# succinctlabs/snark-bn254-verifier

Hardware: AMD Instinct MI355X
Metric: Groth16 verifies/sec (2 pub-inputs) at batch=2^20, 1/2/4/8 MI355X (higher is better)
Workload: dtype int64

## Files before the change

### snark-bn254-verifier_amd/csrc/bn254_coop12.hip

```cpp
#include <hip/hip_runtime.h>
#include <mutex>
#include "bn254_vm.h"
#include "bn254_kernels.h"

namespace bn254 {

static_assert(COOP_T_ELEM == VE_S2, "COOP_T_ELEM must name a workspace slot that neither VE_T nor the result slot VE_S0 overlays");
#define C12_STRIDE 12
#define C12_SLOT(e) (((e) - VE_F) / 12)
#define C12_X 10
#define C12_I 11
#define C12_B 7
#define C12_R1 7
#define C12_R2 11
#define C12_R3 12
#define C12_SLOTS 13
#define C12_WAVE_DWORDS (C12_SLOTS * 64 * C12_STRIDE)
#define C12_PER_WAVE 5

typedef __attribute__((address_space(3))) int32_t c12_lds_i32;
typedef int c12_v4i __attribute__((ext_vector_type(4)));
typedef __attribute__((address_space(3))) c12_v4i c12_lds_i4;
struct Coop12 {
  c12_lds_i32* img;
  uint32_t lane, g0, c, h;
  __device__ __forceinline__ void put(int slot, const Fp& a) const {
    c12_lds_i4* q = (c12_lds_i4*)(img + ((size_t)slot * 64 + lane) * C12_STRIDE);
    q[0] = (c12_v4i){a.v[0], a.v[1], a.v[2], a.v[3]}; q[1] = (c12_v4i){a.v[4], a.v[5], a.v[6], a.v[7]}; q[2] = (c12_v4i){a.v[8], 0, 0, 0};
  }
  __device__ __forceinline__ Fp at(int slot, uint32_t ln) const {
    const c12_lds_i4* q = (const c12_lds_i4*)(img + ((size_t)slot * 64 + ln) * C12_STRIDE);
    const c12_v4i v0 = q[0], v1 = q[1], v2 = q[2];
    Fp a;
    a.v[0] = v0.x; a.v[1] = v0.y; a.v[2] = v0.z; a.v[3] = v0.w; a.v[4] = v1.x; a.v[5] = v1.y; a.v[6] = v1.z; a.v[7] = v1.w; a.v[8] = v2.x;
    return a;
  }
  __device__ __forceinline__ Fp own(int slot) const { return at(slot, lane); }
  __device__ __forceinline__ Fp half(int slot, uint32_t i) const { return at(slot, g0 + 2 * i + h); }
  __device__ __forceinline__ Fp2 coef(int slot, uint32_t i) const { Fp2 r; r.c0 = at(slot, g0 + 2 * i); r.c1 = at(slot, g0 + 2 * i + 1); return r; }
};

__device__ __forceinline__ Fp2 c12_scale(const Fp2& a, int32_t w) {
  Fp2 r;
#pragma unroll
  for (int i = 0; i < BN_NL; i++) { r.c0.v[i] = a.c0.v[i] * w; r.c1.v[i] = a.c1.v[i] * w; }
  return r;
}
struct C12H { Fp p, q; };
__device__ __forceinline__ C12H c12_halves(const Fp2& b, uint32_t h) { C12H r; r.p = fp_select(h != 0, b.c1, b.c0); r.q = fp_select(h != 0, b.c0, fp_neg(b.c1)); return r; }
__device__ __forceinline__ void c12_publish_xi(const Coop12& co, int slot) {
  const Fp o = co.own(slot), pt = co.at(slot, co.lane ^ 1);
  co.put(C12_X, fp_lincomb_reduce(9, o, co.h ? 1 : -1, pt));
}
__device__ __forceinline__ void c12_publish_i(const Coop12& co, int slot) {
  const Fp pt = co.at(slot, co.lane ^ 1);
  co.put(C12_I, fp_select(co.h != 0, pt, fp_neg(pt)));
}

__constant__ int8_t C12_SQ_Q[6][4] = {{0, 1, 2, 3}, {0, 2, 3, 0}, {0, 1, 3, 4}, {0, 1, 4, 0}, {0, 1, 2, 5}, {0, 1, 2, 0}};
__constant__ int8_t C12_SQ_P[6][4] = {{0, 5, 4, 3}, {1, 5, 4, 0}, {2, 1, 5, 4}, {3, 2, 5, 0}, {4, 3, 2, 5}, {5, 4, 3, 0}};
__constant__ int8_t C12_SQ_X[6][4] = {{0, 1, 1, 1}, {0, 1, 1, 0}, {0, 0, 1, 1}, {0, 0, 1, 0}, {0, 0, 0, 1}, {0, 0, 0, 0}};
__constant__ int8_t C12_SQ_W[6][4] = {{1, 2, 2, 1}, {2, 2, 2, 0}, {2, 1, 2, 1}, {2, 2, 2, 0}, {2, 2, 1, 1}, {2, 2, 2, 0}};
__device__ __forceinline__ void c12_sqr(const Coop12& co, int s) {
  c12_publish_xi(co, s);
  c12_publish_i(co, s);
  const uint32_t c = co.c;
  const Fp2 p0 = c12_scale(co.coef(s, C12_SQ_P[c][0]), C12_SQ_W[c][0]);
  const Fp2 p1 = c12_scale(co.coef(C12_SQ_X[c][1] ? C12_X : s, C12_SQ_P[c][1]), C12_SQ_W[c][1]);
  const Fp2 p2 = c12_scale(co.coef(C12_SQ_X[c][2] ? C12_X : s, C12_SQ_P[c][2]), C12_SQ_W[c][2]);
  const Fp2 p3 = c12_scale(co.coef(C12_SQ_X[c][3] ? C12_X : s, C12_SQ_P[c][3]), C12_SQ_W[c][3]);
  const Fp q0 = co.half(s, C12_SQ_Q[c][0]), q1 = co.half(s, C12_SQ_Q[c][1]), q2 = co.half(s, C12_SQ_Q[c][2]), q3 = co.half(s, C12_SQ_Q[c][3]);
  const Fp j0 = co.half(C12_I, C12_SQ_Q[c][0]), j1 = co.half(C12_I, C12_SQ_Q[c][1]), j2 = co.half(C12_I, C12_SQ_Q[c][2]), j3 = co.half(C12_I, C12_SQ_Q[c][3]);
  co.put(s, fp_dot(dplus(p0.c0, q0), dplus(p0.c1, j0), dplus(p1.c0, q1), dplus(p1.c1, j1), dplus(p2.c0, q2), dplus(p2.c1, j2), dplus(p3.c0, q3), dplus(p3.c1, j3)));
}
__device__ __forceinline__ void c12_mul_line_fp(const Coop12& co, int s, const Fp& d0, const C12H& d3, const C12H& d4, bool keep) {
  c12_publish_xi(co, s);
  const uint32_t c = co.c;
  const Fp k = co.own(s);
  const Fp2 k1 = co.coef(c >= 1 ? s : C12_X, (c + 5) % 6), k3 = co.coef(c >= 3 ? s : C12_X, (c + 3) % 6);
  const Fp r = fp_dot(dplus(k, d0), dplus(k1.c0, d3.p), dplus(k1.c1, d3.q), dplus(k3.c0, d4.p), dplus(k3.c1, d4.q));
  co.put(s, fp_select(keep, k, r));
}
__device__ __forceinline__ void c12_mul_line_fp2(const Coop12& co, int s, const C12H& d0, const C12H& d3, const C12H& d4) {
  c12_publish_xi(co, s);
  const uint32_t c = co.c;
  const Fp2 k0 = co.coef(s, c);
  const Fp2 k1 = co.coef(c >= 1 ? s : C12_X, (c + 5) % 6), k3 = co.coef(c >= 3 ? s : C12_X, (c + 3) % 6);
  co.put(s, fp_dot(dplus(k0.c0, d0.p), dplus(k0.c1, d0.q), dplus(k1.c0, d3.p), dplus(k1.c1, d3.q), dplus(k3.c0, d4.p), dplus(k3.c1, d4.q)));
}
__device__ __noinline__ void c12_mul(const Coop12 co, int d, int a, int b, bool conj_b) {
  const uint32_t c = co.c;
  c12_publish_xi(co, a);
  int bp = b;
  if (conj_b) {
    const Fp o = co.own(b);
    co.put(C12_B, (c & 1) ? fp_neg(o) : o);
    bp = C12_B;
  }
  c12_publish_i(co, bp);
  Fp acc;
  {
    const Fp2 a0 = co.coef(0 <= (int)c ? a : C12_X, 0), a1 = co.coef(1 <= c ? a : C12_X, 1), a2 = co.coef(2 <= c ? a : C12_X, 2);
    const uint32_t i0 = (c + 6 - 0) % 6, i1 = (c + 6 - 1) % 6, i2 = (c + 6 - 2) % 6;
    const Fp q0 = co.half(bp, i0), q1 = co.half(bp, i1), q2 = co.half(bp, i2), j0 = co.half(C12_I, i0), j1 = co.half(C12_I, i1), j2 = co.half(C12_I, i2);
    acc = fp_dot(dplus(a0.c0, q0), dplus(a0.c1, j0), dplus(a1.c0, q1), dplus(a1.c1, j1), dplus(a2.c0, q2), dplus(a2.c1, j2));
  }
  {
    const Fp2 a3 = co.coef(3 <= c ? a : C12_X, 3), a4 = co.coef(4 <= c ? a : C12_X, 4), a5 = co.coef(5 <= c ? a : C12_X, 5);
    const uint32_t i3 = (c + 6 - 3) % 6, i4 = (c + 6 - 4) % 6, i5 = (c + 6 - 5) % 6;
    const Fp q3 = co.half(bp, i3), q4 = co.half(bp, i4), q5 = co.half(bp, i5), j3 = co.half(C12_I, i3), j4 = co.half(C12_I, i4), j5 = co.half(C12_I, i5);
    acc = fp_add(acc, fp_dot(dplus(a3.c0, q3), dplus(a3.c1, j3), dplus(a4.c0, q4), dplus(a4.c1, j4), dplus(a5.c0, q5), dplus(a5.c1, j5)));
  }
  co.put(d, acc);
}
__constant__ int8_t C12_CY_A[6] = {0, 2, 1, 0, 2, 1};
__constant__ int8_t C12_CY_B[6] = {3, 5, 4, 3, 5, 4};
__device__ __noinline__ void c12_cyclo_sqr_n(const Coop12 co, int d, int s, int count) {
  const uint32_t c = co.c, h = co.h;
  const bool is_s = (c == 0) | (c == 2) | (c == 4);
  const int32_t lin = is_s ? -2 : 2;
  Fp k = co.own(s);
  for (int it = 0; it < count; it++) {
    const int src = it == 0 ? s : d;
    const Fp2 a = co.coef(src, C12_CY_A[c]), b = co.coef(src, C12_CY_B[c]);
    const Fp2 xb = fp2_mul_xi(b);
    const Fp2 u1 = fp2_select(is_s, xb, c12_scale(a, 2));
    const Fp2 v1 = fp2_select(is_s | (c == 1), is_s ? b : xb, b);
    const Fp2 u2 = c12_scale(a, is_s ? 1 : 0);
    const C12H h1 = c12_halves(v1, h), h2 = c12_halves(a, h);
    const Fp X = fp_dot(dplus(u1.c0, h1.p), dplus(u1.c1, h1.q), dplus(u2.c0, h2.p), dplus(u2.c1, h2.q));
    const Fp z = fp_lincomb_reduce(3, X, lin, k);
    co.put(d, z);
    k = z;
  }
}
__device__ __noinline__ void c12_conj(const Coop12 co, int d, int s) {
  const Fp k = co.own(s);
  co.put(d, (co.c & 1) ? fp_neg(k) : k);
}
__device__ __noinline__ void c12_frob(const Coop12 co, int d, int s, int j) {
  Fp2 k = co.coef(s, co.c);
  if (j & 1) k = fp2_conj(k);
  const int32_t(*t)[2][BN_NL] = j == 1 ? BN_FROB_G1 : j == 2 ? BN_FROB_G2 : BN_FROB_G3;
  Fp2 g;
#pragma unroll
  for (int l = 0; l < BN_NL; l++) { g.c0.v[l] = t[co.c][0][l]; g.c1.v[l] = t[co.c][1][l]; }
  const C12H gh = c12_halves(g, co.h);
  co.put(d, fp_dot(dplus(k.c0, gh.p), dplus(k.c1, gh.q)));
}
__device__ __noinline__ void c12_inv(const Coop12 co, int d, int s) {
  Fp12 f;
  K0(f) = co.coef(s, 0); K1(f) = co.coef(s, 1); K2(f) = co.coef(s, 2); K3(f) = co.coef(s, 3); K4(f) = co.coef(s, 4); K5(f) = co.coef(s, 5);
  Fp12 r = fp12_inv(f);
  const uint32_t c = co.c;
  const Fp2 o = fp2_select(c == 0, K0(r), fp2_select(c == 1, K1(r), fp2_select(c == 2, K2(r), fp2_select(c == 3, K3(r), fp2_select(c == 4, K4(r), K5(r))))));
  co.put(d, fp_select(co.h != 0, o.c1, o.c0));
}
struct Coop12Ops {
  const Coop12& co;
  __device__ __forceinline__ void f12_inv(int d, int a) { c12_inv(co, C12_SLOT(d), C12_SLOT(a)); }
  __device__ __forceinline__ void f12_conj(int d, int a) { c12_conj(co, C12_SLOT(d), C12_SLOT(a)); }
  __device__ __forceinline__ void f12_mul(int d, int a, int b, bool conj_b = false) { c12_mul(co, C12_SLOT(d), C12_SLOT(a), C12_SLOT(b), conj_b); }
  __device__ __forceinline__ void f12_frob(int d, int a, int j) { c12_frob(co, C12_SLOT(d), C12_SLOT(a), j); }
  __device__ __forceinline__ void f12_cyclo_sqr(int d, int a) { c12_cyclo_sqr_n(co, C12_SLOT(d), C12_SLOT(a), 1); }
  __device__ __forceinline__ void f12_cyclo_sqr_n(int d, int a, int count) { c12_cyclo_sqr_n(co, C12_SLOT(d), C12_SLOT(a), count); }
};

__device__ __forceinline__ Fp c12_ws_ld(const int32_t* ws, uint32_t n, uint32_t p, int e) {
  Fp r;
#pragma unroll
  for (int l = 0; l < BN_NL; l++) r.v[l] = ws[((size_t)e * BN_NL + l) * n + p];
  return r;
}
__device__ __forceinline__ void c12_ws_st(int32_t* ws, uint32_t n, uint32_t p, int e, const Fp& a) {
#pragma unroll
  for (int l = 0; l < BN_NL; l++) ws[((size_t)e * BN_NL + l) * n + p] = a.v[l];
}
__device__ __forceinline__ Fp2 c12_ws_ld2(const int32_t* ws, uint32_t n, uint32_t p, int e) { Fp2 r; r.c0 = c12_ws_ld(ws, n, p, e); r.c1 = c12_ws_ld(ws, n, p, e + 1); return r; }
__device__ __forceinline__ FixedLine c12_line_entry(const int32_t* entry) {
  FixedLine l;
#pragma unroll
  for (int i = 0; i < BN_NL; i++) {
    l.m.c0.v[i] = entry[i]; l.m.c1.v[i] = entry[BN_NL + i]; l.c.c0.v[i] = entry[2 * BN_NL + i]; l.c.c1.v[i] = entry[3 * BN_NL + i];
    l.xc.c0.v[i] = entry[4 * BN_NL + i]; l.xc.c1.v[i] = entry[5 * BN_NL + i];
  }
  return l;
}
__device__ __forceinline__ void c12_store_f12(const Coop12& co, int32_t* ws, uint32_t n, uint32_t p, int slot, int e, bool pending) {
  const Fp r = co.own(slot);
  if (pending) c12_ws_st(ws, n, p, e + 2 * (int)co.c + (int)co.h, r);
}

__device__ __forceinline__ bool c12_eq_const(const Coop12& co, int slot, const int32_t* __restrict__ target, uint32_t pl) {
  Fp t;
#pragma unroll
  for (int l = 0; l < BN_NL; l++) t.v[l] = target[(2 * (int)co.c + (int)co.h) * BN_NL + l];
  BN_SETB(t, 1.0, 0.5);
  const uint64_t m = __builtin_amdgcn_ballot_w64(fp_eq(co.own(slot), t));
  return ((m >> (pl * 12u)) & 0xfffull) == 0xfffull;
}

#define C12_PROLOGUE()                                                                                        \
  extern __shared__ __attribute__((aligned(16))) int32_t c12_lds[];                                           \
  const uint32_t lane = threadIdx.x & 63;                                                                     \
  const bool act = lane < 12 * C12_PER_WAVE;                                                                  \
  const uint32_t la = act ? lane : lane - 12;                          \
  const uint32_t pl = la / 12, c = (la - pl * 12) >> 1, h = la & 1;                                           \
  const uint32_t p = blockIdx.x * (uint32_t)C12_PER_WAVE + pl;                                                \
  const bool live = act && p < n;                                                                             \
  const uint32_t pc = p < n ? p : n - 1;                                                                      \
  const uint8_t st = status[pc];                                                                              \
  const bool pending = live && (st & BN254_ST_PENDING) != 0;                                                  \
  if (__builtin_amdgcn_ballot_w64(pending) == 0) return;                                                      \
  Coop12 co{(c12_lds_i32*)c12_lds, lane, pl * 12, c, h}

__global__ void __launch_bounds__(64) k_coop12_final_exp(int32_t* ws, uint32_t n, const uint8_t* __restrict__ status) {
  C12_PROLOGUE();
  co.put(C12_SLOT(VE_F), c12_ws_ld(ws, n, pc, VE_F + 2 * (int)c + (int)h));
  Coop12Ops ops{co};
  vm_final_exp_program(ops);
  c12_store_f12(co, ws, n, p, C12_SLOT(VE_S0), VE_S0, pending);
}

__global__ void __launch_bounds__(64)
k_coop12_miller_fixed(int32_t* ws, uint32_t n, uint8_t* status, const uint8_t* __restrict__ kinds, int n_pairs,
                      const int32_t* __restrict__ tab0, const int32_t* __restrict__ tab1, const int32_t* __restrict__ tab2,
                      int e_p0, int e_p1, int e_p2, int inf0, int inf1, int inf2, int fuse_final_exp, const int32_t* __restrict__ target, int reject_code) {
  C12_PROLOGUE();
  const int F = C12_SLOT(VE_F);
  co.put(F, (c == 0 && h == 0) ? fp_one() : fp_zero());
  const int np = __builtin_amdgcn_readfirstlane(n_pairs);
  const Fp px0 = c12_ws_ld(ws, n, pc, e_p0), py0 = c12_ws_ld(ws, n, pc, e_p0 + 1), px1 = c12_ws_ld(ws, n, pc, e_p1), py1 = c12_ws_ld(ws, n, pc, e_p1 + 1);
  const Fp px2 = c12_ws_ld(ws, n, pc, e_p2), py2 = c12_ws_ld(ws, n, pc, e_p2 + 1);
  const bool i0 = (st & inf0) != 0, i1 = (st & inf1) != 0, i2 = (st & inf2) != 0;
  for (int s = 0; s < BN_ATE_STEPS; s++) {
    const int kind = __builtin_amdgcn_readfirstlane((int)kinds[s]);
    if (kind == 0 && s != 0) c12_sqr(co, F);
    { const FixedLine l = c12_line_entry(tab0 + (size_t)s * FIXED_LINE_DWORDS); const C12H m = c12_halves(l.m, h);
      C12H d3; d3.p = fp_mul(m.p, px0); d3.q = fp_mul(m.q, px0); c12_mul_line_fp(co, F, py0, d3, c12_halves(l.c, h), i0); }
    if (np > 1) { const FixedLine l = c12_line_entry(tab1 + (size_t)s * FIXED_LINE_DWORDS); const C12H m = c12_halves(l.m, h);
      C12H d3; d3.p = fp_mul(m.p, px1); d3.q = fp_mul(m.q, px1); c12_mul_line_fp(co, F, py1, d3, c12_halves(l.c, h), i1); }
    if (np > 2) { const FixedLine l = c12_line_entry(tab2 + (size_t)s * FIXED_LINE_DWORDS); const C12H m = c12_halves(l.m, h);
      C12H d3; d3.p = fp_mul(m.p, px2); d3.q = fp_mul(m.q, px2); c12_mul_line_fp(co, F, py2, d3, c12_halves(l.c, h), i2); }
  }
  if (fuse_final_exp) {
    Coop12Ops ops{co};
    vm_final_exp_program(ops);
    if (target) {
      const bool acc = c12_eq_const(co, C12_SLOT(VE_S0), target, pl);
      if (pending && c == 0 && h == 0) status[p] = acc ? BN254_ST_ACCEPT : (uint8_t)reject_code;
    } else c12_store_f12(co, ws, n, p, C12_SLOT(VE_S0), VE_S0, pending);
  } else c12_store_f12(co, ws, n, p, F, VE_F, pending);
}

__device__ __forceinline__ Fp2 c12_sel6(uint32_t c, const Fp2& v0, const Fp2& v1, const Fp2& v2, const Fp2& v3, const Fp2& v4, const Fp2& v5) {
  return fp2_select(c == 0, v0, fp2_select(c == 1, v1, fp2_select(c == 2, v2, fp2_select(c == 3, v3, fp2_select(c == 4, v4, v5)))));
}
__device__ __forceinline__ Fp2 c12_fp_as_fp2(const Fp& a) { Fp2 r; r.c0 = a; r.c1 = fp_zero(); return r; }
__device__ __forceinline__ Fp c12_prod(const Coop12& co, const Fp2& u, const Fp2& v) {
  const C12H vh = c12_halves(v, co.h);
  return fp_dot(dplus(u.c0, vh.p), dplus(u.c1, vh.q));
}
struct C12Line { Fp2 d0, d3, d4, s1, s2, cz; };
__device__ __forceinline__ void c12_g2_double(const Coop12& co, G2Proj& t, const Fp& xa, const Fp& ya, const Fp2& m1, const Fp& xl, const Fp2& m2, const Fp& xc, const Fp2& c1,
                                              const Fp& zl, C12Line& out) {
  const uint32_t c = co.c;
  const Fp2 yz = fp2_add(t.y, t.z);
  co.put(C12_R1, c12_prod(co, c12_sel6(c, t.x, t.y, t.z, t.x, yz, m1), c12_sel6(c, t.y, t.y, t.z, t.x, yz, c12_fp_as_fp2(xl))));
  const Fp2 A = co.coef(C12_R1, 0), B = co.coef(C12_R1, 1), C = co.coef(C12_R1, 2), J = co.coef(C12_R1, 3), S = co.coef(C12_R1, 4);
  out.s1 = co.coef(C12_R1, 5);
  const Fp2 H = fp2_sub2(S, B, C);
  const Fp2 b3 = fp2_from_limbs(BN_TWIST_3B0, BN_TWIST_3B1);
  co.put(C12_R2, c12_prod(co, c12_sel6(c, B, B, b3, H, J, m2), c12_sel6(c, H, B, C, c12_fp_as_fp2(ya), c12_fp_as_fp2(xa), c12_fp_as_fp2(xc))));
  const Fp2 BH = co.coef(C12_R2, 0), E = co.coef(C12_R2, 2), Hy = co.coef(C12_R2, 3), Jx = co.coef(C12_R2, 4);
  out.s2 = co.coef(C12_R2, 5);
  const Fp2 F = fp2_mul_small(E, 3);
  const Fp2 BmF = fp2_sub(B, F), BF = fp2_add(B, F);
  co.put(C12_R3, c12_prod(co, c12_sel6(c, E, A, BF, c1, E, E), c12_sel6(c, E, BmF, BF, c12_fp_as_fp2(zl), E, E)));
  const Fp2 E2 = co.coef(C12_R3, 0), AX = co.coef(C12_R3, 1), BF2 = co.coef(C12_R3, 2);
  out.cz = co.coef(C12_R3, 3);
  t.x = fp2_dbl(AX);
  t.y = fp2_sub(BF2, fp2_mul_small(E2, 12));
  t.z = fp2_mul_small(BH, 4);
  out.d0 = fp2_neg(Hy);
  out.d3 = fp2_mul_small(Jx, 3);
  out.d4 = fp2_sub(E, B);
}
__device__ __forceinline__ void c12_g2_add(const Coop12& co, G2Proj& t, const Fp2& qx, const Fp2& qy, const Fp& xa, const Fp& ya, const Fp2& m1, const Fp& xl, const Fp2& m2,
                                           const Fp& xc, const Fp2& c1, const Fp& zl, C12Line& out) {
  const uint32_t c = co.c;
  co.put(C12_R1, c12_prod(co, c12_sel6(c, qy, qx, qx, qx, qx, m1), c12_sel6(c, t.z, t.z, t.z, t.z, t.z, c12_fp_as_fp2(xl))));
  const Fp2 O = fp2_sub(t.y, co.coef(C12_R1, 0)), L = fp2_sub(t.x, co.coef(C12_R1, 1));
  out.s1 = co.coef(C12_R1, 5);
  co.put(C12_R2, c12_prod(co, c12_sel6(c, O, L, qx, L, L, m2), c12_sel6(c, O, L, O, qy, c12_fp_as_fp2(ya), c12_fp_as_fp2(xc))));
  const Fp2 Cc = co.coef(C12_R2, 0), D = co.coef(C12_R2, 1), xqO = co.coef(C12_R2, 2), Lyq = co.coef(C12_R2, 3);
  out.d0 = co.coef(C12_R2, 4);
  out.s2 = co.coef(C12_R2, 5);
  co.put(C12_R3, c12_prod(co, c12_sel6(c, L, t.z, t.x, O, c1, O), c12_sel6(c, D, Cc, D, c12_fp_as_fp2(xa), c12_fp_as_fp2(zl), O)));
  const Fp2 E = co.coef(C12_R3, 0), Fz = co.coef(C12_R3, 1), G = co.coef(C12_R3, 2), Ox = co.coef(C12_R3, 3);
  out.cz = co.coef(C12_R3, 4);
  const Fp2 H = fp2_sub(fp2_add(E, Fz), fp2_dbl(G));
  const Fp2 GmH = fp2_sub(G, H);
  co.put(C12_R1, c12_prod(co, c12_sel6(c, L, GmH, t.y, E, E, E), c12_sel6(c, H, O, E, t.z, E, E)));
  t.x = co.coef(C12_R1, 0);
  t.y = fp2_sub(co.coef(C12_R1, 1), co.coef(C12_R1, 2));
  t.z = co.coef(C12_R1, 3);
  out.d3 = fp2_neg(Ox);
  out.d4 = fp2_sub(xqO, Lyq);
}
__device__ __forceinline__ G1Aff c12_msm_entry(const int32_t* __restrict__ msm_tab, size_t idx) {
  const int4* e = (const int4*)(msm_tab + idx * MSM_ENTRY_DWORDS);
  int4 v0 = e[0], v1 = e[1], v2 = e[2], v3 = e[3], v4 = e[4];
  G1Aff q;
  q.x.v[0] = v0.x; q.x.v[1] = v0.y; q.x.v[2] = v0.z; q.x.v[3] = v0.w; q.x.v[4] = v1.x; q.x.v[5] = v1.y; q.x.v[6] = v1.z; q.x.v[7] = v1.w;
  q.x.v[8] = v2.x; q.y.v[0] = v2.y; q.y.v[1] = v2.z; q.y.v[2] = v2.w; q.y.v[3] = v3.x; q.y.v[4] = v3.y; q.y.v[5] = v3.z; q.y.v[6] = v3.w;
  q.y.v[7] = v4.x; q.y.v[8] = v4.y;
  return q;
}
// ... 133 lines not shown
```

### snark-bn254-verifier_amd/csrc/bn254_devws.h

```cpp
#pragma once
#include <hip/hip_runtime.h>
#include "bn254_vm.h"
#include "bn254_kernels.h"

namespace bn254 {

struct DevWs {
  __amdgpu_buffer_rsrc_t rsrc;
  uint32_t row_bytes;
  uint32_t voff;
  int32_t* lds = nullptr;
  __device__ __forceinline__ void park(int slot, const Fp2& a) const {
#pragma unroll
    for (int l = 0; l < BN_NL; l++) { lds[(slot * 18 + l) * 256 + threadIdx.x] = a.c0.v[l]; lds[(slot * 18 + BN_NL + l) * 256 + threadIdx.x] = a.c1.v[l]; }
  }
  __device__ __forceinline__ Fp2 unpark(int slot) const {
    Fp2 r;
#pragma unroll
    for (int l = 0; l < BN_NL; l++) { r.c0.v[l] = lds[(slot * 18 + l) * 256 + threadIdx.x]; r.c1.v[l] = lds[(slot * 18 + BN_NL + l) * 256 + threadIdx.x]; }
    BN_SETB(r.c0, 3.0, 0.5); BN_SETB(r.c1, 3.0, 0.5);
    return r;
  }
  __device__ __forceinline__ DevWs(int32_t* base, uint32_t n, uint32_t lane) {
    uint64_t b = (uint64_t)base;
    uint32_t lo = __builtin_amdgcn_readfirstlane((uint32_t)b), hi = __builtin_amdgcn_readfirstlane((uint32_t)(b >> 32));
    uint32_t nn = __builtin_amdgcn_readfirstlane(n);
    rsrc = __builtin_amdgcn_make_buffer_rsrc((void*)(((uint64_t)hi << 32) | lo), 0, nn * (uint32_t)(G16_WS_ELEMS * 36), 0x00020000);
    row_bytes = nn * 4u;
    voff = lane * 4u;
  }
  __device__ __forceinline__ Fp ld(int e) const {
    Fp r;
    uint32_t eu = __builtin_amdgcn_readfirstlane((uint32_t)e);
#pragma unroll
    for (int l = 0; l < BN_NL; l++) r.v[l] = __builtin_amdgcn_raw_buffer_load_b32(rsrc, voff, (eu * (uint32_t)BN_NL + (uint32_t)l) * row_bytes, 0);
    return r;
  }
  __device__ __forceinline__ void st(int e, const Fp& a) const {
    uint32_t eu = __builtin_amdgcn_readfirstlane((uint32_t)e);
#pragma unroll
    for (int l = 0; l < BN_NL; l++) __builtin_amdgcn_raw_buffer_store_b32(a.v[l], rsrc, voff, (eu * (uint32_t)BN_NL + (uint32_t)l) * row_bytes, 0);
  }
};

#define DEAD_LANE (0xffffffffu / 4u)

__device__ __forceinline__ const int32_t* uni_ptr(const int32_t* p) {
  uint64_t b = (uint64_t)p;
  uint32_t lo = __builtin_amdgcn_readfirstlane((uint32_t)b), hi = __builtin_amdgcn_readfirstlane((uint32_t)(b >> 32));
  return (const int32_t*)(((uint64_t)hi << 32) | lo);
}
__device__ __forceinline__ Fp uni_ld(const int32_t* p) {
  Fp r;
#pragma unroll
  for (int l = 0; l < BN_NL; l++) r.v[l] = p[l];
  return r;
}
__device__ __forceinline__ Fp2 uni_ld2(const int32_t* p) { Fp2 r; r.c0 = uni_ld(p); r.c1 = uni_ld(p + BN_NL); return r; }

__device__ __forceinline__ G1Aff msm_entry(const int32_t* __restrict__ msm_tab, size_t idx) {
  const int4* e = (const int4*)(msm_tab + idx * MSM_ENTRY_DWORDS);
  int4 v0 = e[0], v1 = e[1], v2 = e[2], v3 = e[3], v4 = e[4];
  G1Aff q;
  q.x.v[0] = v0.x; q.x.v[1] = v0.y; q.x.v[2] = v0.z; q.x.v[3] = v0.w; q.x.v[4] = v1.x; q.x.v[5] = v1.y; q.x.v[6] = v1.z; q.x.v[7] = v1.w;
  q.x.v[8] = v2.x; q.y.v[0] = v2.y; q.y.v[1] = v2.z; q.y.v[2] = v2.w; q.y.v[3] = v3.x; q.y.v[4] = v3.y; q.y.v[5] = v3.z; q.y.v[6] = v3.w;
  q.y.v[7] = v4.x; q.y.v[8] = v4.y;
  BN_SETB(q.x, 1.0, 0.5); BN_SETB(q.y, 1.0, 0.5);
  return q;
}

struct KeyView { const int32_t *msm_tab, *k0, *gtab, *dtab, *target; int n_public, inputs_match; };
__device__ __forceinline__ const int32_t* keys_const_ptr(uint64_t bits) {
  const uint32_t lo = __builtin_amdgcn_readfirstlane((uint32_t)bits), hi = __builtin_amdgcn_readfirstlane((uint32_t)(bits >> 32));
  return (const int32_t*)(const __attribute__((address_space(4))) int32_t*)(((uint64_t)hi << 32) | lo);
}
__device__ __forceinline__ KeyView keys_view(const G16KeyDesc* __restrict__ desc, const uint32_t* __restrict__ granule_key, uint32_t wave_first, uint32_t n_keys) {
  static_assert(sizeof(G16KeyDesc) == 48, "five pointers and two words");
  uint32_t k = (uint32_t)__builtin_amdgcn_readfirstlane((int)granule_key[wave_first / G16_KEYS_GRANULE]);
  k = k < n_keys ? k : 0u;
  const uint64_t b = (uint64_t)(desc + k);
  const uint32_t lo = __builtin_amdgcn_readfirstlane((uint32_t)b), hi = __builtin_amdgcn_readfirstlane((uint32_t)(b >> 32));
  const __attribute__((address_space(4))) uint64_t* f = (const __attribute__((address_space(4))) uint64_t*)(((uint64_t)hi << 32) | lo);
  KeyView v;
  const uint64_t tab = f[0];
  v.msm_tab = (const int32_t*)(const __attribute__((address_space(1))) int32_t*)tab;
  v.k0 = keys_const_ptr(f[1]); v.gtab = keys_const_ptr(f[2]); v.dtab = keys_const_ptr(f[3]); v.target = keys_const_ptr(f[4]);
  const uint64_t w = f[5];
  v.n_public = __builtin_amdgcn_readfirstlane((int)(uint32_t)w); v.inputs_match = __builtin_amdgcn_readfirstlane((int)(uint32_t)(w >> 32));
  return v;
}

__device__ __forceinline__ void be_field_to_words(uint32_t w[8], const uint32_t* d) {
#pragma unroll
  for (int i = 0; i < 8; i++) w[i] = __builtin_bswap32(d[7 - i]);
}
__device__ __forceinline__ bool words_lt_p(const uint32_t w[8]) { return !words_ge(w, BN_P_WORDS); }

#define VM_KERNEL_PROLOGUE()                                                                     \
  const uint32_t i = blockIdx.x * 256u + threadIdx.x;                                           \
  const uint8_t st = status[i < n ? i : n - 1];                                                 \
  if (__builtin_amdgcn_ballot_w64((st & BN254_ST_PENDING) != 0) == 0) return;                   \
  DevWs w(ws, n, i < n ? i : DEAD_LANE)


}
```

### snark-bn254-verifier_amd/csrc/bn254_k_keys.hip

```cpp
#include <hip/hip_runtime.h>
#include "bn254_devws.h"
#include "bn254_keys.h"

namespace bn254 {

#define KEYS_LDS_COUNTERS 8192
__global__ void __launch_bounds__(256) k_keys_count(const uint32_t* __restrict__ key_index, uint32_t n, uint32_t n_keys, uint32_t* __restrict__ count) {
  __shared__ uint32_t lc[KEYS_LDS_COUNTERS];
  const bool priv = n_keys <= KEYS_LDS_COUNTERS;
  if (priv) { for (uint32_t k = threadIdx.x; k < n_keys; k += 256) lc[k] = 0; __syncthreads(); }
  for (uint32_t i = blockIdx.x * 256u + threadIdx.x; i < n; i += gridDim.x * 256u) {
    const uint32_t k = key_index[i];
    if (k >= n_keys) continue;
    if (priv) atomicAdd(&lc[k], 1u); else atomicAdd(&count[k], 1u);
  }
  if (priv) {
    __syncthreads();
    for (uint32_t k = threadIdx.x; k < n_keys; k += 256) { const uint32_t c = lc[k]; if (c) atomicAdd(&count[k], c); }
  }
}
__global__ void __launch_bounds__(1024) k_keys_scan(const uint32_t* __restrict__ count, uint32_t n_keys, uint32_t* __restrict__ base, uint32_t* __restrict__ cursor, uint32_t* __restrict__ n_slots) {
  __shared__ uint32_t tot[1024];
  const uint32_t t = threadIdx.x, per = (n_keys + 1023u) / 1024u;
  const uint32_t lo = t * per < n_keys ? t * per : n_keys, hi = lo + per < n_keys ? lo + per : n_keys;
// ... 25 lines not shown
    const uint32_t lead = (uint32_t)__builtin_ctzll(left);
    const uint32_t kk = (uint32_t)__builtin_amdgcn_readlane((int)k, (int)lead);
    const uint64_t same = __builtin_amdgcn_ballot_w64(todo && k == kk);
    uint32_t first = 0;
    if (lane == lead) first = atomicAdd(&cursor[kk], (uint32_t)__builtin_popcountll(same));
    first = (uint32_t)__builtin_amdgcn_readlane((int)first, (int)lead);
    if (todo && k == kk) {
      keys_place(slot_to_proof, granule_key, first + (uint32_t)__builtin_popcountll(same & ((1ull << lane) - 1ull)), i, k);
      todo = false;
    }
  }
}

#define PREPK_LDS_ROW 65
__global__ void __launch_bounds__(256, 2)
k_g16_prepare_keys(const uint8_t* __restrict__ proofs, size_t stride, const uint8_t* __restrict__ inputs, size_t input_stride, uint32_t n_proofs, uint32_t m, uint32_t slot0,
                   const uint32_t* __restrict__ n_slots, const uint32_t* __restrict__ slot_to_proof, const uint32_t* __restrict__ granule_key,
                   const G16KeyDesc* __restrict__ desc, uint32_t n_keys, int32_t* ws, uint8_t* __restrict__ slot_status) {
  __shared__ uint32_t lds[4 * 64 * PREPK_LDS_ROW];
  const int wave = threadIdx.x >> 6, lane = threadIdx.x & 63;
  const uint32_t first = blockIdx.x * 256u + (uint32_t)wave * 64u;
  const uint32_t total = (uint32_t)__builtin_amdgcn_readfirstlane((int)n_slots[0]);
  const uint32_t live_slots = total > slot0 ? (total - slot0 < m ? total - slot0 : m) : 0u;
  const bool wave_live = first < live_slots;
  const uint32_t i = first + lane;
  uint32_t pi = wave_live ? slot_to_proof[i] : G16_KEYS_NO_PROOF;
  const bool live = pi < n_proofs;
  uint32_t* wl = lds + wave * 64 * PREPK_LDS_ROW;
  const bool aligned = ((((uintptr_t)proofs) | stride) & 3) == 0;
  if (wave_live) {
    if (aligned) {
      for (int j0 = 0; j0 < 64; j0 += 16) {
        uint32_t v[16];
#pragma unroll
        for (int u = 0; u < 16; u++) { const uint32_t rec = (uint32_t)__builtin_amdgcn_readlane((int)pi, j0 + u); v[u] = rec < n_proofs ? *(const uint32_t*)(proofs + (size_t)rec * stride + (size_t)lane * 4) : 0u; }
#pragma unroll
        for (int u = 0; u < 16; u++) wl[(j0 + u) * PREPK_LDS_ROW + lane] = v[u];
      }
    } else {
      for (int j = 0; j < 64; j++) {
        const uint32_t rec = (uint32_t)__builtin_amdgcn_readlane((int)pi, j);
        uint32_t v = 0;
        if (rec < n_proofs) {
          const uint8_t* p = proofs + (size_t)rec * stride + (size_t)lane * 4;
          v = (uint32_t)p[0] | (uint32_t)p[1] << 8 | (uint32_t)p[2] << 16 | (uint32_t)p[3] << 24;
        }
        wl[j * PREPK_LDS_ROW + lane] = v;
      }
    }
  }
  __syncthreads();
  if (!wave_live) { if (i < m) slot_status[i] = 0; return; }
  const KeyView kv = keys_view(desc, granule_key, first, n_keys);
  DevWs w(ws, m, live ? i : DEAD_LANE);
  const uint32_t* my = wl + lane * PREPK_LDS_ROW;
  uint32_t d[8], wx[8], wy[8];
  int err = 0;
  int err_c = 0;

#pragma unroll
  for (int k = 0; k < 8; k++) d[k] = my[k];
  be_field_to_words(wx, d);
#pragma unroll
  for (int k = 0; k < 8; k++) d[k] = my[8 + k];
  be_field_to_words(wy, d);
  bool memb = words_lt_p(wx) & words_lt_p(wy);
  G1Aff A; A.x = fp_from_words(wx); A.y = fp_from_words(wy);
  if (!memb) err = BN254_ST_NOT_MEMBER; else if (!g1_on_curve(A)) err = BN254_ST_NOT_ON_CURVE;
  w.st(VE_AX, A.x); w.st(VE_AY, A.y);

  G2Aff B;
  bool membb = true;
#pragma unroll
  for (int k = 0; k < 8; k++) d[k] = my[16 + k];
  be_field_to_words(wx, d); membb &= words_lt_p(wx); B.x.c1 = fp_from_words(wx);
#pragma unroll
  for (int k = 0; k < 8; k++) d[k] = my[24 + k];
  be_field_to_words(wx, d); membb &= words_lt_p(wx); B.x.c0 = fp_from_words(wx);
#pragma unroll
  for (int k = 0; k < 8; k++) d[k] = my[32 + k];
  be_field_to_words(wx, d); membb &= words_lt_p(wx); B.y.c1 = fp_from_words(wx);
#pragma unroll
  for (int k = 0; k < 8; k++) d[k] = my[40 + k];
  be_field_to_words(wx, d); membb &= words_lt_p(wx); B.y.c0 = fp_from_words(wx);
  if (err == 0) { if (!membb) err = BN254_ST_NOT_MEMBER; else if (!g2_on_curve(B)) err = BN254_ST_NOT_ON_CURVE; }
  vst2(w, VE_B, B.x); vst2(w, VE_B + 2, B.y);

#pragma unroll
  for (int k = 0; k < 8; k++) d[k] = my[48 + k];
  be_field_to_words(wx, d);
#pragma unroll
  for (int k = 0; k < 8; k++) d[k] = my[56 + k];
  be_field_to_words(wy, d);
  memb = words_lt_p(wx) & words_lt_p(wy);
  G1Aff C; C.x = fp_from_words(wx); C.y = fp_from_words(wy);
  if (!memb) err_c = BN254_ST_NOT_MEMBER; else if (!g1_on_curve(C)) err_c = BN254_ST_NOT_ON_CURVE;
  w.st(VE_CX, C.x); w.st(VE_CY, C.y);

  const int32_t* k0 = kv.k0;
  const int32_t* msm_tab = kv.msm_tab;
  const int n_public = kv.inputs_match ? kv.n_public : 0;
  G1Aff K0; K0.x = uni_ld(k0); K0.y = uni_ld(k0 + BN_NL);
  G1Proj L = g1_from_affine(K0);
  for (int s = 0; s < n_public; s++) {
    uint32_t sw[8];
#pragma unroll
    for (int k = 0; k < 8; k++) sw[k] = 0u;
    if (live) {
      const uint8_t* sp = inputs + (size_t)pi * input_stride + (size_t)s * 32;
      if (((((uintptr_t)inputs) | input_stride) & 3) == 0) {
#pragma unroll
        for (int k = 0; k < 8; k++) sw[k] = ((const uint32_t*)sp)[k];
      } else {
#pragma unroll
        for (int k = 0; k < 8; k++) sw[k] = (uint32_t)sp[4 * k] | (uint32_t)sp[4 * k + 1] << 8 | (uint32_t)sp[4 * k + 2] << 16 | (uint32_t)sp[4 * k + 3] << 24;
      }
    }
    for (int j = 0; j < 32; j++) {
      const int wi = 31 - j;
      const uint32_t dig = sw[0] & 0xff;
#pragma unroll
      for (int k = 0; k < 7; k++) sw[k] = (sw[k] >> 8) | (sw[k + 1] << 24);
      sw[7] >>= 8;
      if (dig != 0) L = g1_add_mixed(L, msm_entry(msm_tab, (size_t)(s * 32 + wi) * 255 + (dig - 1)));
    }
  }
  bool l_inf = g1_is_identity(L);
  G1Aff La = g1_to_affine(L);
  La.y = fp_select(l_inf, fp_one(), La.y);
  w.st(VE_LX, La.x); w.st(VE_LY, La.y);
  slot_status[i] = !live ? (uint8_t)0 : err ? (uint8_t)err : (uint8_t)(BN254_ST_PENDING | (l_inf ? BN254_ST_LINF : 0) | err_c);
}

__global__ void __launch_bounds__(256, 2)
k_g16_check_scalars_keys(const uint8_t* __restrict__ inputs, size_t input_stride, uint32_t n_proofs, uint32_t m, const uint32_t* __restrict__ slot_to_proof,
                         const uint32_t* __restrict__ granule_key, const G16KeyDesc* __restrict__ desc, uint32_t n_keys, uint8_t* __restrict__ slot_status) {
  const uint32_t i = blockIdx.x * 256u + threadIdx.x;
  const uint32_t first = i & ~63u;
  if (first >= m) return;
  const uint8_t st = slot_status[i];
  if (__builtin_amdgcn_ballot_w64(st != 0) == 0) return;
  const int n_public = keys_view(desc, granule_key, first, n_keys).n_public;
  const uint32_t pi = slot_to_proof[i];
  if (st == 0 || pi >= n_proofs) return;
  bool bad = false;
  for (int s = 0; s < n_public; s++) {
    uint32_t w[8];
    words_from_be(w, inputs + (size_t)pi * input_stride + (size_t)s * 32);
    bad |= words_ge(w, BN_R_WORDS);
  }
  if (bad) slot_status[i] = BN254_ST_NOT_MEMBER;
}

#define VM_KEYS_PROLOGUE()                                                                       \
  const uint32_t i = blockIdx.x * 256u + threadIdx.x;                                           \
  if ((i & ~63u) >= n) return;                                                                   \
  const uint8_t st = status[i < n ? i : n - 1];                                                 \
  if (__builtin_amdgcn_ballot_w64((st & BN254_ST_PENDING) != 0) == 0) return;                   \
  DevWs w(ws, n, i < n ? i : DEAD_LANE)

__global__ void __launch_bounds__(256, 2)
k_g16_subgroup_keys(uint32_t n, int32_t* ws, uint8_t* __restrict__ status, const uint32_t* __restrict__ granule_key, const G16KeyDesc* __restrict__ desc, uint32_t n_keys, int e_t) {
  VM_KEYS_PROLOGUE();
  const int inputs_match_key = keys_view(desc, granule_key, i & ~63u, n_keys).inputs_match;
  bool ok = vm_g2_ate_check(w, e_t, VE_B);
  if (i < n && (st & BN254_ST_PENDING)) {
    uint8_t out;
    if (!ok) out = BN254_ST_NOT_IN_SUBGROUP;
    else if (st & 0x3f) out = st & 0x3f;
    else if (!inputs_match_key) out = BN254_ST_INPUT_LEN;
    else out = BN254_ST_PENDING | (st & BN254_ST_LINF);
    status[i] = out;
  }
}

__global__ void __launch_bounds__(256, 2)
k_g16_compare_keys(int32_t* ws, uint32_t n, const uint8_t* __restrict__ status, const uint32_t* __restrict__ slot_to_proof, const uint32_t* __restrict__ granule_key,
                   const G16KeyDesc* __restrict__ desc, uint32_t n_keys, uint32_t n_proofs, uint8_t* __restrict__ out_status) {
  const uint32_t i = blockIdx.x * 256u + threadIdx.x;
  if ((i & ~63u) >= n) return;
  const uint8_t st = status[i < n ? i : n - 1];
  if (__builtin_amdgcn_ballot_w64(st != 0) == 0) return;
  uint8_t out = st;
  if (__builtin_amdgcn_ballot_w64((st & BN254_ST_PENDING) != 0) != 0) {
    DevWs w(ws, n, i < n ? i : DEAD_LANE);
    const int32_t* target = keys_view(desc, granule_key, i & ~63u, n_keys).target;
    const bool acc = vm_f12_eq_const(w, VE_S0, target);
    if (st & BN254_ST_PENDING) out = acc ? BN254_ST_ACCEPT : BN254_ST_REJECT;
  }
  if (i < n && st != 0) { const uint32_t pi = slot_to_proof[i]; if (pi < n_proofs) out_status[pi] = out; }
}

}

using namespace bn254;
hipError_t bn254_launch_keys_group(const uint32_t* key_index, uint32_t n, uint32_t n_keys, uint32_t slot_cap, uint32_t* count, uint32_t* base, uint32_t* cursor,
                                   uint32_t* n_slots, uint32_t* slot_to_proof, uint32_t* granule_key, uint8_t* status, hipStream_t s) {
  hipError_t e;
  if ((e = hipMemsetAsync(count, 0, (size_t)n_keys * 4, s)) != hipSuccess) return e;
  if ((e = hipMemsetAsync(slot_to_proof, 0xff, (size_t)slot_cap * 4, s)) != hipSuccess) return e;
  if ((e = hipMemsetAsync(granule_key, 0, (size_t)(slot_cap / G16_KEYS_GRANULE + 1) * 4, s)) != hipSuccess) return e;
  const unsigned blocks = (n + 255) / 256;
  hipLaunchKernelGGL(k_keys_count, dim3(blocks < 1024 ? blocks : 1024), dim3(256), 0, s, key_index, n, n_keys, count);
  hipLaunchKernelGGL(k_keys_scan, dim3(1), dim3(1024), 0, s, (const uint32_t*)count, n_keys, base, cursor, n_slots);
  hipLaunchKernelGGL(k_keys_place, dim3(blocks), dim3(256), 0, s, key_index, n, n_keys, cursor, slot_to_proof, granule_key, status);
  return hipGetLastError();
}
void bn254_launch_g16_prepare_keys(const G16KeysLaunchArgs& a, unsigned grid, hipStream_t s) {
  hipLaunchKernelGGL(k_g16_prepare_keys, dim3(grid), dim3(256), 0, s, a.proofs, a.stride, a.inputs, a.input_stride, a.n_proofs, (uint32_t)a.m, a.slot0, a.n_slots, a.slot_to_proof,
                     a.granule_key, a.desc, a.n_keys, a.ws, a.slot_status);
  if (a.strict_scalars)
    hipLaunchKernelGGL(k_g16_check_scalars_keys, dim3(grid), dim3(256), 0, s, a.inputs, a.input_stride, a.n_proofs, (uint32_t)a.m, a.slot_to_proof, a.granule_key, a.desc, a.n_keys,
                       a.slot_status);
}
void bn254_launch_g16_subgroup_keys(const G16KeysLaunchArgs& a, unsigned grid, hipStream_t s, int e_t) {
  hipLaunchKernelGGL(k_g16_subgroup_keys, dim3(grid), dim3(256), 0, s, (uint32_t)a.m, a.ws, a.slot_status, a.granule_key, a.desc, a.n_keys, e_t);
}
void bn254_launch_g16_compare_keys(const G16KeysLaunchArgs& a, unsigned grid, hipStream_t s) {
  hipLaunchKernelGGL(k_g16_compare_keys, dim3(grid), dim3(256), 0, s, a.ws, (uint32_t)a.m, (const uint8_t*)a.slot_status, a.slot_to_proof, a.granule_key, a.desc, a.n_keys, a.n_proofs,
                     a.status);
}
```

### snark-bn254-verifier_amd/csrc/bn254_k_miller.hip

```cpp
#include <cstdlib>
#include "bn254_devws.h"

namespace bn254 {

template <bool DO_SQR>
__global__ void __launch_bounds__(256, 2) k_miller_step_dbl(int32_t* ws, uint32_t n, const uint8_t* __restrict__ status, int e_t, int e, int e_pa,
                                                            const int32_t* __restrict__ entry0, int e_p0, int inf_mask0,
                                                            const int32_t* __restrict__ entry1, int e_p1, int inf_mask1) {
  __shared__ int32_t park_lds[72 * 256];
  VM_KERNEL_PROLOGUE();
  w.lds = park_lds;
  FixedLine l0, l1;
  l0.m = uni_ld2(entry0); l0.c = uni_ld2(entry0 + 2 * BN_NL); l0.xc = uni_ld2(entry0 + 4 * BN_NL);
  l1.m = uni_ld2(entry1); l1.c = uni_ld2(entry1 + 2 * BN_NL); l1.xc = uni_ld2(entry1 + 4 * BN_NL);
  vm_miller_step<DO_SQR>(w, 0, e_t, 0, e, e_pa, l0, e_p0, (st & inf_mask0) != 0, l1, e_p1, (st & inf_mask1) != 0);
}
__global__ void __launch_bounds__(256, 2) k_miller_step_add(int32_t* ws, uint32_t n, const uint8_t* __restrict__ status, int kind, int e_t, int e_b, int e, int e_pa,
                                                            const int32_t* __restrict__ entry0, int e_p0, int inf_mask0,
                                                            const int32_t* __restrict__ entry1, int e_p1, int inf_mask1) {
  __shared__ int32_t park_lds[72 * 256];
  VM_KERNEL_PROLOGUE();
  w.lds = park_lds;
  FixedLine l0, l1;
  l0.m = uni_ld2(entry0); l0.c = uni_ld2(entry0 + 2 * BN_NL); l0.xc = uni_ld2(entry0 + 4 * BN_NL);
  l1.m = uni_ld2(entry1); l1.c = uni_ld2(entry1 + 2 * BN_NL); l1.xc = uni_ld2(entry1 + 4 * BN_NL);
  int k = __builtin_amdgcn_readfirstlane(kind);
  vm_miller_step<false>(w, k < 1 ? 1 : k, e_t, e_b, e, e_pa, l0, e_p0, (st & inf_mask0) != 0, l1, e_p1, (st & inf_mask1) != 0);
}

struct DevLines {
  const int32_t* tab0; const int32_t* tab1;
  __device__ __forceinline__ FixedLine get(int t, int s) const {
    const int32_t* e = (t == 0 ? tab0 : tab1) + (size_t)s * FIXED_LINE_DWORDS;
    FixedLine l; l.m = uni_ld2(e); l.c = uni_ld2(e + 2 * BN_NL); l.xc = uni_ld2(e + 4 * BN_NL);
    return l;
  }
};
struct DevKinds {
  MillerKinds k;
  __device__ __forceinline__ int get(int s) const { return __builtin_amdgcn_readfirstlane((k.nib[s >> 1] >> ((s & 1) * 4)) & 15); }
};
__global__ void __launch_bounds__(256, 2) k_miller_run(int32_t* ws, uint32_t n, const uint8_t* __restrict__ status, MillerKinds kinds, int s_begin, int s_end,
                                                       int e_t, int e_b, int e, int e_pa, const int32_t* __restrict__ tab0, int e_p0, int inf_mask0,
                                                       const int32_t* __restrict__ tab1, int e_p1, int inf_mask1) {
  __shared__ int32_t park_lds[72 * 256];
  VM_KERNEL_PROLOGUE();
  w.lds = park_lds;
  DevLines lines{uni_ptr(tab0), uni_ptr(tab1)};
  DevKinds dk{kinds};
  vm_miller_run(w, lines, dk, __builtin_amdgcn_readfirstlane(s_begin), __builtin_amdgcn_readfirstlane(s_end), e_t, e_b, e, e_pa, e_p0, (st & inf_mask0) != 0,
                e_p1, (st & inf_mask1) != 0);
}

__global__ void __launch_bounds__(256, 2) k_miller_run_keys(int32_t* ws, uint32_t n, const uint8_t* __restrict__ status, MillerKinds kinds, int s_begin, int s_end,
                                                            int e_t, int e_b, int e, int e_pa, const G16KeyDesc* __restrict__ desc, uint32_t n_keys,
                                                            const uint32_t* __restrict__ granule_key, int e_p0, int inf_mask0, int e_p1, int inf_mask1) {
  __shared__ int32_t park_lds[72 * 256];
  if (((blockIdx.x * 256u + threadIdx.x) & ~63u) >= n) return;
  VM_KERNEL_PROLOGUE();
  w.lds = park_lds;
  const KeyView kv = keys_view(desc, granule_key, i & ~63u, n_keys);
  DevLines lines{kv.gtab, kv.dtab};
  DevKinds dk{kinds};
  vm_miller_run(w, lines, dk, __builtin_amdgcn_readfirstlane(s_begin), __builtin_amdgcn_readfirstlane(s_end), e_t, e_b, e, e_pa, e_p0, (st & inf_mask0) != 0,
                e_p1, (st & inf_mask1) != 0);
}

__global__ void __launch_bounds__(256, 2) k_miller_run_fixed2(int32_t* ws, uint32_t n, const uint8_t* __restrict__ status, MillerKinds kinds, int s_begin, int s_end, int e,
                                                              const int32_t* __restrict__ tab0, int e_p0, int inf_mask0, const int32_t* __restrict__ tab1, int e_p1, int inf_mask1) {
  __shared__ int32_t park_lds[72 * 256];
  VM_KERNEL_PROLOGUE();
  w.lds = park_lds;
  DevLines lines{uni_ptr(tab0), uni_ptr(tab1)};
  DevKinds dk{kinds};
  vm_miller_run_fixed2(w, lines, dk, __builtin_amdgcn_readfirstlane(s_begin), __builtin_amdgcn_readfirstlane(s_end), e, e_p0, (st & inf_mask0) != 0, e_p1, (st & inf_mask1) != 0);
}

}

using namespace bn254;
void bn254_launch_miller_run_fixed2(const MillerKinds& kinds, int s_begin, int s_end, int32_t* ws, uint32_t n, const uint8_t* status, unsigned grid, hipStream_t s, int e,
                                    const int32_t* tab0, int ep0, int inf0, const int32_t* tab1, int ep1, int inf1) {
  hipLaunchKernelGGL(k_miller_run_fixed2, dim3(grid), dim3(256), 0, s, ws, n, status, kinds, s_begin, s_end, e, tab0, ep0, inf0, tab1, ep1, inf1);
}
void bn254_launch_miller_run(const MillerKinds& kinds, int s_begin, int s_end, int32_t* ws, uint32_t n, const uint8_t* status, unsigned grid, hipStream_t s, int et, int eb,
                             int e, int epa, const int32_t* tab0, int ep0, int inf0, const int32_t* tab1, int ep1, int inf1) {
  hipLaunchKernelGGL(k_miller_run, dim3(grid), dim3(256), 0, s, ws, n, status, kinds, s_begin, s_end, et, eb, e, epa, tab0, ep0, inf0, tab1, ep1, inf1);
}
void bn254_launch_miller_run_keys(const MillerKinds& kinds, int s_begin, int s_end, int32_t* ws, uint32_t n, const uint8_t* status, unsigned grid, hipStream_t s, int et, int eb,
                                  int e, int epa, const G16KeyDesc* desc, uint32_t n_keys, const uint32_t* granule_key, int ep0, int inf0, int ep1, int inf1) {
  hipLaunchKernelGGL(k_miller_run_keys, dim3(grid), dim3(256), 0, s, ws, n, status, kinds, s_begin, s_end, et, eb, e, epa, desc, n_keys, granule_key, ep0, inf0, ep1, inf1);
}
void bn254_launch_miller_step(bool do_sqr, int kind, int32_t* ws, uint32_t n, const uint8_t* status, unsigned grid, hipStream_t s, int et, int eb, int e, int epa,
                              const int32_t* t0, int ep0, int inf0, const int32_t* t1, int ep1, int inf1) {
  if (kind == 0 && do_sqr) hipLaunchKernelGGL(k_miller_step_dbl<true>, dim3(grid), dim3(256), 0, s, ws, n, status, et, e, epa, t0, ep0, inf0, t1, ep1, inf1);
  else if (kind == 0) hipLaunchKernelGGL(k_miller_step_dbl<false>, dim3(grid), dim3(256), 0, s, ws, n, status, et, e, epa, t0, ep0, inf0, t1, ep1, inf1);
  else hipLaunchKernelGGL(k_miller_step_add, dim3(grid), dim3(256), 0, s, ws, n, status, kind, et, eb, e, epa, t0, ep0, inf0, t1, ep1, inf1);
}
```

### snark-bn254-verifier_amd/csrc/bn254_kernels.h

```cpp
#pragma once
#include <hip/hip_runtime.h>
#include <stddef.h>
#include <stdint.h>

#define BN254_ST_REJECT 0
#define BN254_ST_ACCEPT 1
#define BN254_ST_NOT_MEMBER 2
#define BN254_ST_NOT_ON_CURVE 3
#define BN254_ST_NOT_IN_SUBGROUP 4
#define BN254_ST_INPUT_LEN 5
#define BN254_ST_MALFORMED 6
#define BN254_ST_PENDING 0x80
#define BN254_ST_LINF 0x40
#define BN254_ST_LINF2 0x20
#define BN254_ST_LINF3 0x10

#define MSM_ENTRY_DWORDS 20
#include "bn254_fw.h"
#define FIXED_LINE_DWORDS 54
#define G16_WS_ELEMS 130
#define G16_WS_BYTES_PER_PROOF (G16_WS_ELEMS * 36)
#define G16_MAX_BATCH 1048576
#define G16_MAX_LAUNCH 786432

static_assert((unsigned long long)G16_MAX_LAUNCH * G16_WS_BYTES_PER_PROOF < 0xfffffffcull, "workspace of one launch exceeds 32-bit buffer offsets");
#define VE_LX_ELEM 8
#define VE_CX_ELEM 6
struct G16LaunchArgs {
  const uint8_t* proofs; size_t stride;
  const uint8_t* inputs; int n_public;
  size_t n;
  int32_t* ws;
  uint8_t* status;
  const int32_t* msm_tab;
  const int32_t* k0;
  const int32_t* gtab;
  const int32_t* dtab;
  const int32_t* target;
  int inputs_match_key;
  int strict_scalars = 0;
  int msm_comb = 0;
  uint16_t* msm_digits = nullptr;
  int part_of_larger = 0;
  int32_t* msm_part;
  hipStream_t split_streams[2] = {nullptr, nullptr};
  hipEvent_t split_ev[3] = {nullptr, nullptr, nullptr};
};
#define G16_SPLIT_MAX_PROOFS 16384
#define G16_WIDE_MSM_MIN_INPUTS 16
#define G16_WIDE_MSM_INPUTS_PER_LANE 16
#define G16_COMB_TEETH 13
#define G16_COMB_COLS 20
static inline __host__ __device__ uint32_t g16_comb_digit(const uint32_t w[8], int col) {
  uint32_t idx = 0;
#pragma unroll
  for (int t = 0; t < G16_COMB_TEETH; t++) {
    const int base = G16_COMB_COLS * t;
    const int wi = base >> 5, sh = base & 31;
    const uint64_t two = ((uint64_t)(wi + 1 < 8 ? w[wi + 1 < 8 ? wi + 1 : 7] : 0u) << 32) | w[wi < 8 ? wi : 7];
    const uint32_t bit = wi < 8 ? (uint32_t)((two >> (sh + col)) & 1u) : 0u;
    idx |= bit << t;
  }
  return idx;
}
#define G16_WIDE_MSM_MAX_PROOFS 65536
enum {
  KID_PREPARE, KID_SUBGROUP, KID_VM_INIT, KID_F12_SQR, KID_MUL_LINE_FIXED, KID_F12_MUL,
  KID_CYCLO_SQR, KID_F12_CONJ, KID_F12_FROB, KID_F12_INV, KID_COMPARE, KID_F12_COPY, KID_CYCLO_SQR_N, KID_MILLER_DBL_VAR, KID_MILLER_ADD_VAR, KID_MSM_PARTIAL, KID_MSM_REDUCE, KID_MUL_LINE_FIXED2, KID_MILLER_SQR_DBL_VAR, KID_MILLER_STEP_DBL, KID_MILLER_STEP_ADD, KID_COOP_G16, KID_MILLER_RUN, KID_COUNT
};
extern const char* const bn254_kernel_kind_names[KID_COUNT];
struct G16Prof {
  uint32_t mask;
  hipEvent_t* ev;
  uint8_t* kid;
  int cap, used;
};
hipError_t bn254_launch_g16(const G16LaunchArgs& a, hipStream_t s, hipEvent_t* ev, G16Prof* prof);
void bn254_launch_miller_step(bool do_sqr, int kind, int32_t* ws, uint32_t n, const uint8_t* status, unsigned grid, hipStream_t s, int et, int eb, int e, int epa,
                              const int32_t* t0, int ep0, int inf0, const int32_t* t1, int ep1, int inf1);
struct MillerKinds { uint8_t nib[44]; };
void bn254_launch_miller_run(const MillerKinds& kinds, int s_begin, int s_end, int32_t* ws, uint32_t n, const uint8_t* status, unsigned grid, hipStream_t s, int et, int eb,
                             int e, int epa, const int32_t* tab0, int ep0, int inf0, const int32_t* tab1, int ep1, int inf1);
void bn254_launch_miller_run_fixed2(const MillerKinds& kinds, int s_begin, int s_end, int32_t* ws, uint32_t n, const uint8_t* status, unsigned grid, hipStream_t s, int e,
                                    const int32_t* tab0, int ep0, int inf0, const int32_t* tab1, int ep1, int inf1);
#include "bn254_keys.h"
struct G16KeysLaunchArgs {
  const uint8_t* proofs; size_t stride;
  const uint8_t* inputs; size_t input_stride;
  uint32_t n_proofs;
  size_t m;
  uint32_t slot0;
  const uint32_t* n_slots;
  const uint32_t* slot_to_proof;
  const uint32_t* granule_key;
  const bn254::G16KeyDesc* desc; uint32_t n_keys;
  int32_t* ws;
  uint8_t* slot_status;
  uint8_t* status;
  int strict_scalars = 0;
  int part_of_larger = 0;
};
hipError_t bn254_launch_keys_group(const uint32_t* key_index, uint32_t n, uint32_t n_keys, uint32_t slot_cap, uint32_t* count, uint32_t* base, uint32_t* cursor,
                                   uint32_t* n_slots, uint32_t* slot_to_proof, uint32_t* granule_key, uint8_t* status, hipStream_t s);
void bn254_launch_g16_prepare_keys(const G16KeysLaunchArgs& a, unsigned grid, hipStream_t s);
void bn254_launch_g16_subgroup_keys(const G16KeysLaunchArgs& a, unsigned grid, hipStream_t s, int e_t);
void bn254_launch_g16_compare_keys(const G16KeysLaunchArgs& a, unsigned grid, hipStream_t s);
void bn254_launch_miller_run_keys(const MillerKinds& kinds, int s_begin, int s_end, int32_t* ws, uint32_t n, const uint8_t* status, unsigned grid, hipStream_t s, int et, int eb,
                                  int e, int epa, const bn254::G16KeyDesc* desc, uint32_t n_keys, const uint32_t* granule_key, int ep0, int inf0, int ep1, int inf1);
hipError_t bn254_launch_g16_keys(const G16KeysLaunchArgs& a, hipStream_t s);
size_t bn254_tab_build_teeth(int form);
size_t bn254_tab_build_entries(int form);
size_t bn254_tab_build_out_entries(int form);
hipError_t bn254_launch_tab_build(int form, const int32_t* pts, uint32_t points, int32_t* table, int32_t* teeth_plane, int32_t* teeth_aff, int32_t* plane, hipStream_t s);
#include "bn254_rlc_plan.h"
struct RlcLaunchArgs {
  uint32_t key[11];
  uint32_t counter_base;
  bn254::RlcPlan plan;
  uint8_t* grp_status;
  const int32_t* btab;
  const int32_t* rlc_tab;
  const int32_t* one;
  uint8_t* grp_rows = nullptr;
  uint16_t* grp_digits = nullptr;
  int32_t* grp_part = nullptr;
  int msm_form = 2;
};
hipError_t bn254_launch_g16_rlc(const G16LaunchArgs& a, const RlcLaunchArgs& r, hipStream_t s);
hipError_t bn254_launch_gather_rows(uint8_t* dst, const uint8_t* src, size_t src_stride, uint32_t row_bytes, const uint32_t* idx, uint32_t m, hipStream_t s);
hipError_t bn254_launch_scatter_status(uint8_t* status, const uint8_t* fb_status, const uint32_t* idx, uint32_t m, hipStream_t s);
hipError_t bn254_launch_g16_decompress(const uint8_t* src, size_t stride, uint32_t n, uint8_t* raw, uint8_t* pre, hipStream_t s);
hipError_t bn254_launch_g16_status_merge(uint8_t* status, const uint8_t* pre, uint32_t n, hipStream_t s);
hipError_t bn254_launch_sp1_public_inputs(const uint8_t* vkh, size_t vkh_stride, const uint8_t* pv, uint64_t pv_bytes, uint64_t pv_base, const uint64_t* off, uint32_t n,
                                          uint8_t* rows, uint8_t* pre, hipStream_t s);
#define G1_GLV_TAB_BYTES_PER_LANE (16 * 28 * 4)
namespace bn254 { struct MsmPlan; }
size_t bn254_g1_msm_scratch_lanes(const bn254::MsmPlan& plan, size_t n);
hipError_t bn254_launch_g1_msm_rows(const bn254::MsmPlan& plan, const int32_t* terms, const uint8_t* flags, size_t n, int n_terms, int32_t* part, int32_t* glv_tab,
                                    const int32_t* tabs, hipStream_t s);
hipError_t bn254_launch_g1_sum_rows(const bn254::MsmPlan& plan, const int32_t* part, size_t n, uint32_t* out_words, uint8_t* out_inf, int32_t* ws, uint8_t* status, int e_x, int inf_bit,
                                    int e_x_b, int inf_bit_b, hipStream_t s);
hipError_t bn254_launch_pairing2_fixed(int32_t* ws, uint8_t* status, size_t n, const int32_t* tab0, const int32_t* tab1, const int32_t* target_one,
                                       int reject_code, hipStream_t s, hipStream_t aux, hipEvent_t ev_fork, hipEvent_t ev_join);
#define COOP_T_ELEM 46
#define COOP12_MAX_PROOFS 30720
#define COOP12_MAX_PROOFS_FIXED 40960
hipError_t bn254_coop12_miller_g16(int32_t* ws, uint8_t* status, size_t n, const int32_t* tab0, const int32_t* tab1, const uint8_t* inputs, int n_public,
                                   int inputs_match_key, const int32_t* msm_tab, const int32_t* k0, int l_from_ws, int fuse_final_exp, const int32_t* target, hipStream_t s);
hipError_t bn254_coop12_final_exp(int32_t* ws, uint8_t* status, size_t n, hipStream_t s);
hipError_t bn254_coop12_miller_fixed(int32_t* ws, uint8_t* status, size_t n, int n_pairs, const int32_t* tab0, const int32_t* tab1, const int32_t* tab2,
                                     int e_p0, int e_p1, int e_p2, int inf0, int inf1, int inf2, int fuse_final_exp, const int32_t* target, int reject_code, hipStream_t s);
static inline size_t bn254_coop_max_proofs() { return COOP12_MAX_PROOFS; }
static inline size_t bn254_coop_max_proofs_fixed() { return COOP12_MAX_PROOFS_FIXED; }
double bn254_measure_valu_sustained(double ms_target);
double bn254_measure_valu_peak(int reps);
hipError_t bn254_launch_dbg_fp_mul(const uint8_t* a, const uint8_t* b, uint8_t* o, size_t n, hipStream_t s);
hipError_t bn254_launch_dbg_fp12_op(int op, const uint8_t* a, const uint8_t* b, uint8_t* o, size_t n, int32_t* ws, uint8_t* status, hipStream_t s);
hipError_t bn254_launch_dbg_pairing(const uint8_t* g1, const uint8_t* g2, uint8_t* o, size_t n, int32_t* ws, uint8_t* status, hipStream_t s);
hipError_t bn254_launch_dbg_g2_ate(const uint8_t* g1, const uint8_t* g2, uint8_t* o, size_t n, int32_t* ws, uint8_t* status, hipStream_t s);
hipError_t bn254_launch_dbg_g2_subgroup(const uint8_t* g2, uint8_t* o, size_t n, hipStream_t s);
```

### snark-bn254-verifier_amd/csrc/bn254_kernels.hip

```cpp
#include <hip/hip_runtime.h>
#include <cstdlib>
#include <cstring>
#include "bn254_devws.h"
#include "bn254_rlc.h"
#include "bn254_g16_plan.h"
#include "bn254_codec.h"
#include "bn254_sha256.h"

namespace bn254 {


__global__ void __launch_bounds__(256, 2) k_vm_init(int32_t* ws, uint32_t n, const uint8_t* __restrict__ status) {
  VM_KERNEL_PROLOGUE();
  w.st(VE_F, fp_one());
  for (int e = 1; e < 12; e++) w.st(VE_F + e, fp_zero());
  for (int e = 0; e < 4; e++) w.st(VE_T + e, w.ld(VE_B + e));
  w.st(VE_T + 4, fp_one()); w.st(VE_T + 5, fp_zero());
}
__global__ void __launch_bounds__(256, 2) k_f12_sqr(int32_t* ws, uint32_t n, const uint8_t* __restrict__ status, int e) { VM_KERNEL_PROLOGUE(); vm_f12_sqr(w, e); }
__global__ void __launch_bounds__(256, 2) k_f12_mul_line_fixed(int32_t* ws, uint32_t n, const uint8_t* __restrict__ status, int e, const int32_t* __restrict__ entry, int e_px, int inf_mask) {
  VM_KERNEL_PROLOGUE();
  FixedLine l; l.m = uni_ld2(entry); l.c = uni_ld2(entry + 2 * BN_NL); l.xc = uni_ld2(entry + 4 * BN_NL);
  vm_f12_mul_line_fixed(w, e, l, e_px, (st & inf_mask) != 0);
}
__global__ void __launch_bounds__(256, 2) k_f12_mul_line_fixed2(int32_t* ws, uint32_t n, const uint8_t* __restrict__ status, int e, const int32_t* __restrict__ entry0,
                                                                int e_px0, int inf_mask0, const int32_t* __restrict__ entry1, int e_px1, int inf_mask1) {
  __shared__ int32_t park_lds[72 * 256];
  VM_KERNEL_PROLOGUE();
  w.lds = park_lds;
  FixedLine l0, l1;
  l0.m = uni_ld2(entry0); l0.c = uni_ld2(entry0 + 2 * BN_NL); l0.xc = uni_ld2(entry0 + 4 * BN_NL);
  l1.m = uni_ld2(entry1); l1.c = uni_ld2(entry1 + 2 * BN_NL); l1.xc = uni_ld2(entry1 + 4 * BN_NL);
  vm_f12_mul_line_fixed2(w, e, l0, e_px0, (st & inf_mask0) != 0, l1, e_px1, (st & inf_mask1) != 0);
}
__global__ void __launch_bounds__(256, 2) k_miller_dbl_var(int32_t* ws, uint32_t n, const uint8_t* __restrict__ status, int e_t, int e, int e_px) {
  VM_KERNEL_PROLOGUE(); vm_miller_dbl_var(w, e_t, e, e_px);
}
__global__ void __launch_bounds__(256, 2) k_miller_sqr_dbl_var(int32_t* ws, uint32_t n, const uint8_t* __restrict__ status, int e_t, int e, int e_px) {
  __shared__ int32_t park_lds[72 * 256];
  VM_KERNEL_PROLOGUE();
  w.lds = park_lds;
  vm_miller_sqr_dbl_var(w, e_t, e, e_px);
}
__global__ void __launch_bounds__(256, 2) k_miller_add_var(int32_t* ws, uint32_t n, const uint8_t* __restrict__ status, int e_t, int e_b, int which, int e, int e_px) {
  VM_KERNEL_PROLOGUE(); vm_miller_add_var(w, e_t, e_b, which, e, e_px);
}
__global__ void __launch_bounds__(256, 2) k_f12_mul(int32_t* ws, uint32_t n, const uint8_t* __restrict__ status, int d, int a, int b, int conj_b) {
  __shared__ int32_t park_lds[72 * 256];
  VM_KERNEL_PROLOGUE();
  w.lds = park_lds;
  vm_f12_mul(w, d, a, b, conj_b != 0);
}
__global__ void __launch_bounds__(256, 2) k_f12_copy(int32_t* ws, uint32_t n, const uint8_t* __restrict__ status, int d, int a) { VM_KERNEL_PROLOGUE(); vm_f12_copy(w, d, a); }
__global__ void __launch_bounds__(256, 2) k_f12_cyclo_sqr(int32_t* ws, uint32_t n, const uint8_t* __restrict__ status, int d, int a) { VM_KERNEL_PROLOGUE(); vm_f12_cyclo_sqr(w, d, a); }
__global__ void __launch_bounds__(256, 2) k_f12_cyclo_sqr_n(int32_t* ws, uint32_t n, const uint8_t* __restrict__ status, int d, int a, int count) {
  VM_KERNEL_PROLOGUE(); vm_f12_cyclo_sqr_n(w, d, a, __builtin_amdgcn_readfirstlane(count));
}
__global__ void __launch_bounds__(256, 2) k_f12_conj(int32_t* ws, uint32_t n, const uint8_t* __restrict__ status, int d, int a) { VM_KERNEL_PROLOGUE(); vm_f12_conj(w, d, a); }
__global__ void __launch_bounds__(256, 2) k_f12_frob(int32_t* ws, uint32_t n, const uint8_t* __restrict__ status, int d, int a, int j) { VM_KERNEL_PROLOGUE(); vm_f12_frob(w, d, a, j); }
__global__ void __launch_bounds__(256, 2) k_f12_inv(int32_t* ws, uint32_t n, const uint8_t* __restrict__ status, int d, int a) { VM_KERNEL_PROLOGUE(); vm_f12_inv(w, d, a); }
__global__ void __launch_bounds__(256, 2) k_g16_compare(int32_t* ws, uint32_t n, uint8_t* __restrict__ status, const int32_t* __restrict__ target, int reject_code) {
  VM_KERNEL_PROLOGUE();
  bool acc = vm_f12_eq_const(w, VE_S0, target);
  if (i < n && (st & BN254_ST_PENDING)) status[i] = acc ? BN254_ST_ACCEPT : (uint8_t)reject_code;
}


#define PREP_LDS_ROW 65
__global__ void __launch_bounds__(256, 2)
k_g16_prepare(const uint8_t* __restrict__ proofs, size_t stride, const uint8_t* __restrict__ inputs, int n_public, uint32_t n,
              int32_t* ws, uint8_t* __restrict__ status, const int32_t* __restrict__ msm_tab, const int32_t* __restrict__ k0,
              int inputs_match_key, int wide_msm) {
  __shared__ uint32_t lds[4 * 64 * PREP_LDS_ROW];
  const int wave = threadIdx.x >> 6, lane = threadIdx.x & 63;
  const uint32_t first = blockIdx.x * 256u + (uint32_t)wave * 64u;
  uint32_t* wl = lds + wave * 64 * PREP_LDS_ROW;
  const bool aligned = ((((uintptr_t)proofs) | stride) & 3) == 0;
  if (aligned) {
    for (int j0 = 0; j0 < 64; j0 += 16) {
      uint32_t v[16];
#pragma unroll
      for (int u = 0; u < 16; u++) { const uint32_t rec = first + (uint32_t)(j0 + u); v[u] = rec < n ? *(const uint32_t*)(proofs + (size_t)rec * stride + (size_t)lane * 4) : 0u; }
#pragma unroll
      for (int u = 0; u < 16; u++) wl[(j0 + u) * PREP_LDS_ROW + lane] = v[u];
    }
  } else {
    for (int j = 0; j < 64; j++) {
      uint32_t rec = first + j;
      uint32_t v = 0;
      if (rec < n) {
        const uint8_t* p = proofs + (size_t)rec * stride + (size_t)lane * 4;
        v = (uint32_t)p[0] | (uint32_t)p[1] << 8 | (uint32_t)p[2] << 16 | (uint32_t)p[3] << 24;
      }
      wl[j * PREP_LDS_ROW + lane] = v;
    }
  }
  __syncthreads();
  const uint32_t i = first + lane;
  const bool live = i < n;
  const uint32_t ii = live ? i : n - 1;
  DevWs w(ws, n, live ? i : DEAD_LANE);
  const uint32_t* my = wl + lane * PREP_LDS_ROW;
  uint32_t d[8], wx[8], wy[8];
  int err = 0;
  int err_c = 0;

#pragma unroll
  for (int k = 0; k < 8; k++) d[k] = my[k];
  be_field_to_words(wx, d);
#pragma unroll
  for (int k = 0; k < 8; k++) d[k] = my[8 + k];
  be_field_to_words(wy, d);
  bool memb = words_lt_p(wx) & words_lt_p(wy);
  G1Aff A; A.x = fp_from_words(wx); A.y = fp_from_words(wy);
  if (!memb) err = BN254_ST_NOT_MEMBER; else if (!g1_on_curve(A)) err = BN254_ST_NOT_ON_CURVE;
  w.st(VE_AX, A.x); w.st(VE_AY, A.y);

  G2Aff B;
  bool membb = true;
#pragma unroll
  for (int k = 0; k < 8; k++) d[k] = my[16 + k];
  be_field_to_words(wx, d); membb &= words_lt_p(wx); B.x.c1 = fp_from_words(wx);
#pragma unroll
  for (int k = 0; k < 8; k++) d[k] = my[24 + k];
  be_field_to_words(wx, d); membb &= words_lt_p(wx); B.x.c0 = fp_from_words(wx);
#pragma unroll
  for (int k = 0; k < 8; k++) d[k] = my[32 + k];
  be_field_to_words(wx, d); membb &= words_lt_p(wx); B.y.c1 = fp_from_words(wx);
#pragma unroll
  for (int k = 0; k < 8; k++) d[k] = my[40 + k];
  be_field_to_words(wx, d); membb &= words_lt_p(wx); B.y.c0 = fp_from_words(wx);
  if (err == 0) { if (!membb) err = BN254_ST_NOT_MEMBER; else if (!g2_on_curve(B)) err = BN254_ST_NOT_ON_CURVE; }
  vst2(w, VE_B, B.x); vst2(w, VE_B + 2, B.y);

#pragma unroll
  for (int k = 0; k < 8; k++) d[k] = my[48 + k];
  be_field_to_words(wx, d);
#pragma unroll
  for (int k = 0; k < 8; k++) d[k] = my[56 + k];
  be_field_to_words(wy, d);
  memb = words_lt_p(wx) & words_lt_p(wy);
  G1Aff C; C.x = fp_from_words(wx); C.y = fp_from_words(wy);
  if (!memb) err_c = BN254_ST_NOT_MEMBER; else if (!g1_on_curve(C)) err_c = BN254_ST_NOT_ON_CURVE;
  w.st(VE_CX, C.x); w.st(VE_CY, C.y);

  if (wide_msm) {
    if (live) status[i] = err ? (uint8_t)err : (uint8_t)(BN254_ST_PENDING | err_c);
    return;
  }
  G1Aff K0; K0.x = uni_ld(k0); K0.y = uni_ld(k0 + BN_NL);
  G1Proj L = g1_from_affine(K0);
  if (inputs_match_key) {
    for (int s = 0; s < n_public; s++) {
      const uint8_t* sp = inputs + ((size_t)ii * (size_t)n_public + s) * 32;
      uint32_t sw[8];
      if ((((uintptr_t)inputs) & 3) == 0) {
#pragma unroll
        for (int k = 0; k < 8; k++) sw[k] = ((const uint32_t*)sp)[k];
      } else {
#pragma unroll
        for (int k = 0; k < 8; k++) sw[k] = (uint32_t)sp[4 * k] | (uint32_t)sp[4 * k + 1] << 8 | (uint32_t)sp[4 * k + 2] << 16 | (uint32_t)sp[4 * k + 3] << 24;
      }
      uint32_t kw[8];
#pragma unroll
      for (int k = 0; k < 8; k++) kw[k] = __builtin_bswap32(sw[7 - k]);
      auto next_digit = [&]() -> uint32_t {
        const uint32_t dg = kw[0] & MSM_FW_ENTRIES;
#pragma unroll
        for (int k = 0; k < 7; k++) kw[k] = (kw[k] >> MSM_FW_BITS) | (kw[k + 1] << (32 - MSM_FW_BITS));
        kw[7] >>= MSM_FW_BITS;
        return dg;
      };
      uint32_t dig = next_digit();
      G1Aff q = msm_entry(msm_tab, (size_t)(s * MSM_FW_WINDOWS) * MSM_FW_ENTRIES + (dig ? dig - 1 : 0));
      for (int j = 0; j < MSM_FW_WINDOWS; j++) {
        uint32_t dn = 0; G1Aff qn = q;
        if (j + 1 < MSM_FW_WINDOWS) { dn = next_digit(); qn = msm_entry(msm_tab, (size_t)(s * MSM_FW_WINDOWS + j + 1) * MSM_FW_ENTRIES + (dn ? dn - 1 : 0)); }
        if (dig != 0) L = g1_add_mixed(L, q);
        dig = dn; q = qn;
      }
    }
  }
  bool l_inf = g1_is_identity(L);
  G1Aff La = g1_to_affine(L);
  La.y = fp_select(l_inf, fp_one(), La.y);
  w.st(VE_LX, La.x); w.st(VE_LY, La.y);
  if (live) status[i] = err ? (uint8_t)err : (uint8_t)(BN254_ST_PENDING | (l_inf ? BN254_ST_LINF : 0) | err_c);
}

__global__ void __launch_bounds__(256, 2)
k_g16_check_scalars(const uint8_t* __restrict__ inputs, int n_public, uint32_t n, uint8_t* __restrict__ status) {
  const uint32_t i = blockIdx.x * 256u + threadIdx.x;
  if (i >= n) return;
  bool bad = false;
  for (int s = 0; s < n_public; s++) {
    const uint8_t* sp = inputs + ((size_t)i * (size_t)n_public + s) * 32;
    uint32_t w[8];
    words_from_be(w, sp);
    bad |= words_ge(w, BN_R_WORDS);
  }
  if (bad) status[i] = BN254_ST_NOT_MEMBER;
}

__global__ void __launch_bounds__(256, 2)
k_g16_msm_partial(const uint8_t* __restrict__ inputs, int n_public, uint32_t n, int per, int chunks, const uint8_t* __restrict__ status,
                  const int32_t* __restrict__ msm_tab, int32_t* __restrict__ part) {
  const uint32_t g = blockIdx.x * 256u + threadIdx.x;
  if (g >= n * (uint32_t)chunks) return;
  const uint32_t c = g / n, i = g - c * n;
  G1Proj acc = g1_identity();
  if (status[i] & BN254_ST_PENDING) {
    const int s_end = (int)min((uint32_t)n_public, (c + 1) * (uint32_t)per);
    for (int s = (int)(c * per); s < s_end; s++) {
      const uint8_t* sp = inputs + ((size_t)i * (size_t)n_public + s) * 32;
      uint32_t sw[8];
      if ((((uintptr_t)inputs) & 3) == 0) {
#pragma unroll
        for (int k = 0; k < 8; k++) sw[k] = ((const uint32_t*)sp)[k];
      } else {
#pragma unroll
        for (int k = 0; k < 8; k++) sw[k] = (uint32_t)sp[4 * k] | (uint32_t)sp[4 * k + 1] << 8 | (uint32_t)sp[4 * k + 2] << 16 | (uint32_t)sp[4 * k + 3] << 24;
      }
      for (int j = 0; j < 32; j++) {
        const int wi = 31 - j;
        uint32_t dig = sw[0] & 0xff;
#pragma unroll
        for (int k = 0; k < 7; k++) sw[k] = (sw[k] >> 8) | (sw[k + 1] << 24);
        sw[7] >>= 8;
        if (dig != 0) acc = g1_add_mixed(acc, msm_entry(msm_tab, (size_t)(s * 32 + wi) * 255 + (dig - 1)));
      }
    }
  }
  int32_t* o = part + (size_t)c * 27 * n + i;
#pragma unroll
  for (int l = 0; l < BN_NL; l++) { o[(size_t)l * n] = acc.x.v[l]; o[(size_t)(9 + l) * n] = acc.y.v[l]; o[(size_t)(18 + l) * n] = acc.z.v[l]; }
}
__global__ void __launch_bounds__(256)
k_g16_comb_digits(const uint8_t* __restrict__ inputs, int n_public, uint32_t n, uint16_t* __restrict__ digits) {
  const size_t g = (size_t)blockIdx.x * 256u + threadIdx.x;
  if (g >= (size_t)n * (size_t)n_public) return;
  const uint32_t s = (uint32_t)(g / n), i = (uint32_t)(g - (size_t)s * n);
  const uint8_t* sp = inputs + ((size_t)i * (size_t)n_public + s) * 32;
  uint32_t w[8];
#pragma unroll
  for (int k = 0; k < 8; k++) { const uint8_t* q = sp + 28 - 4 * k; w[k] = (uint32_t)q[0] << 24 | (uint32_t)q[1] << 16 | (uint32_t)q[2] << 8 | (uint32_t)q[3]; }
  for (int col = 0; col < G16_COMB_COLS; col++) {
    const uint32_t idx = g16_comb_digit(w, col);
    digits[((size_t)col * (size_t)n_public + s) * n + i] = (uint16_t)idx;
  }
}
__global__ void __launch_bounds__(256, 2)
k_g16_msm_partial_comb(const uint16_t* __restrict__ digits, int n_public, uint32_t n, int per, int chunks, const uint8_t* __restrict__ status,
                       const int32_t* __restrict__ msm_tab, int32_t* __restrict__ part) {
  const uint32_t g = blockIdx.x * 256u + threadIdx.x;
  if (g >= n * (uint32_t)chunks) return;
  const uint32_t c = g / n, i = g - c * n;
  G1Proj acc = g1_identity();
  if (status[i] & BN254_ST_PENDING) {
    const int s_begin = (int)(c * per), s_end = (int)min((uint32_t)n_public, (c + 1) * (uint32_t)per);
    auto digit_at = [&](int col, int s) -> uint32_t { return digits[((size_t)col * (size_t)n_public + (size_t)s) * n + i]; };
    auto entry_at = [&](int s, uint32_t idx) -> G1Aff { return msm_entry(msm_tab, ((size_t)s << G16_COMB_TEETH) + idx); };
    auto advance = [&](int& col, int& s) { if (++s == s_end) { s = s_begin; col--; } };
    if (s_begin < s_end) {
      int col1 = G16_COMB_COLS - 1, s1 = s_begin;
      uint32_t d_cur = digit_at(col1, s1);
      G1Aff e_cur = entry_at(s1, d_cur);
      int col0 = col1, s0 = s1;
      advance(col1, s1);
      uint32_t d_nxt = col1 >= 0 ? digit_at(col1, s1) : 0u;
      int col2 = col1, s2 = s1;
      if (col2 >= 0) advance(col2, s2);
      while (col0 >= 0) {
        G1Aff e_nxt = e_cur;
        uint32_t d_nn = 0u;
        if (col1 >= 0) e_nxt = entry_at(s1, d_nxt);
        if (col2 >= 0) d_nn = digit_at(col2, s2);
        if (s0 == s_begin && col0 != G16_COMB_COLS - 1) acc = g1_dbl(acc);
        if (d_cur != 0) acc = g1_add_mixed(acc, e_cur);
        col0 = col1; s0 = s1; d_cur = d_nxt; e_cur = e_nxt;
        col1 = col2; s1 = s2; d_nxt = d_nn;
        if (col2 >= 0) advance(col2, s2);
      }
    }
  }
  int32_t* o = part + (size_t)c * 27 * n + i;
#pragma unroll
  for (int l = 0; l < BN_NL; l++) { o[(size_t)l * n] = acc.x.v[l]; o[(size_t)(9 + l) * n] = acc.y.v[l]; o[(size_t)(18 + l) * n] = acc.z.v[l]; }
}
__global__ void __launch_bounds__(256, 2)
k_g16_msm_reduce(const int32_t* __restrict__ part, int chunks, uint32_t n, int32_t* ws, uint8_t* __restrict__ status, const int32_t* __restrict__ k0) {
  VM_KERNEL_PROLOGUE();
  const uint32_t ii = i < n ? i : n - 1;
  G1Aff K0; K0.x = uni_ld(k0); K0.y = uni_ld(k0 + BN_NL);
  G1Proj L = g1_from_affine(K0);
  for (int c = 0; c < chunks; c++) {
    const int32_t* o = part + (size_t)c * 27 * n + ii;
    G1Proj q;
#pragma unroll
    for (int l = 0; l < BN_NL; l++) { q.x.v[l] = o[(size_t)l * n]; q.y.v[l] = o[(size_t)(9 + l) * n]; q.z.v[l] = o[(size_t)(18 + l) * n]; }
    BN_SETB(q.x, 3.0, 0.5); BN_SETB(q.y, 3.0, 0.5); BN_SETB(q.z, 3.0, 0.5);
    L = g1_add(L, q);
  }
  bool l_inf = g1_is_identity(L);
  G1Aff La = g1_to_affine(L);
  La.y = fp_select(l_inf, fp_one(), La.y);
  w.st(VE_LX, La.x); w.st(VE_LY, La.y);
  if (i < n && (st & BN254_ST_PENDING) && l_inf) status[i] = st | BN254_ST_LINF;
}

__global__ void __launch_bounds__(256, 2)
k_g16_msm_reduce8(const int32_t* __restrict__ part, int chunks, uint32_t n, int32_t* ws, uint8_t* __restrict__ status, const int32_t* __restrict__ k0) {
  __shared__ int32_t sums[32 * 8 * 27];
  const uint32_t p = blockIdx.x * 32u + (threadIdx.x >> 3), sub = threadIdx.x & 7u;
  const uint32_t pp = p < n ? p : n - 1;
  G1Proj L = g1_identity();
  for (int c = (int)sub; c < chunks; c += 8) {
    const int32_t* o = part + (size_t)c * 27 * n + pp;
    G1Proj q;
#pragma unroll
    for (int l = 0; l < BN_NL; l++) { q.x.v[l] = o[(size_t)l * n]; q.y.v[l] = o[(size_t)(9 + l) * n]; q.z.v[l] = o[(size_t)(18 + l) * n]; }
    BN_SETB(q.x, 3.0, 0.5); BN_SETB(q.y, 3.0, 0.5); BN_SETB(q.z, 3.0, 0.5);
    L = g1_add(L, q);
  }
  {
    int32_t* o = sums + threadIdx.x * 27;
    const Fp x = fp_reduce(L.x), y = fp_reduce(L.y), z = fp_reduce(L.z);
#pragma unroll
    for (int l = 0; l < BN_NL; l++) { o[l] = x.v[l]; o[9 + l] = y.v[l]; o[18 + l] = z.v[l]; }
  }
  __syncthreads();
  const bool lead = sub == 0 && p < n;
  const uint8_t st = status[pp];
  G1Aff K0; K0.x = uni_ld(k0); K0.y = uni_ld(k0 + BN_NL);
  G1Proj T = g1_from_affine(K0);
  for (int j = 0; j < 8; j++) {
    const int32_t* o = sums + ((threadIdx.x & ~7u) + j) * 27;
    G1Proj q;
#pragma unroll
    for (int l = 0; l < BN_NL; l++) { q.x.v[l] = o[l]; q.y.v[l] = o[9 + l]; q.z.v[l] = o[18 + l]; }
    BN_SETB(q.x, 1.01, 0.5); BN_SETB(q.y, 1.01, 0.5); BN_SETB(q.z, 1.01, 0.5);
    T = g1_add(T, q);
  }
  const bool l_inf = g1_is_identity(T);
  G1Aff La = g1_to_affine(T);
  La.y = fp_select(l_inf, fp_one(), La.y);
  DevWs w(ws, n, lead ? p : DEAD_LANE);
  w.st(VE_LX, La.x); w.st(VE_LY, La.y);
  if (lead && (st & BN254_ST_PENDING) && l_inf) status[p] = st | BN254_ST_LINF;
}

__global__ void __launch_bounds__(256, 2)
k_g16_subgroup(uint32_t n, int32_t* ws, uint8_t* __restrict__ status, int inputs_match_key, int e_t) {
  VM_KERNEL_PROLOGUE();
  bool ok = vm_g2_ate_check(w, e_t, VE_B);
  if (i < n && (st & BN254_ST_PENDING)) {
    uint8_t out;
    if (!ok) out = BN254_ST_NOT_IN_SUBGROUP;
    else if (st & 0x3f) out = st & 0x3f;
    else if (!inputs_match_key) out = BN254_ST_INPUT_LEN;
    else out = BN254_ST_PENDING | (st & BN254_ST_LINF);
    status[i] = out;
  }
}
__global__ void __launch_bounds__(256, 2) k_dbg_g2_ate(int32_t* ws, uint32_t n, const uint8_t* __restrict__ status, uint8_t* o) {
  VM_KERNEL_PROLOGUE();
  bool ok = vm_g2_ate_check(w, VE_T, VE_B);
  if (i < n) o[i] = ok ? 1 : 0;
}

struct DevWs2 {
  __amdgpu_buffer_rsrc_t rsrc;
  uint32_t row_bytes, voff_lo, voff_hi;
  int32_t* lds;
  __device__ __forceinline__ DevWs2(int32_t* base, uint32_t n, uint32_t lane_lo, uint32_t lane_hi, int32_t* lds_) : lds(lds_) {
    DevWs t(base, n, lane_lo);
    rsrc = t.rsrc; row_bytes = t.row_bytes; voff_lo = lane_lo * 4u; voff_hi = lane_hi * 4u;
  }
  __device__ __forceinline__ void park(int slot, const Fp2& a) const {
#pragma unroll
    for (int l = 0; l < BN_NL; l++) { lds[(slot * 18 + l) * 256 + threadIdx.x] = a.c0.v[l]; lds[(slot * 18 + BN_NL + l) * 256 + threadIdx.x] = a.c1.v[l]; }
  }
  __device__ __forceinline__ Fp2 unpark(int slot) const {
    Fp2 r;
#pragma unroll
    for (int l = 0; l < BN_NL; l++) { r.c0.v[l] = lds[(slot * 18 + l) * 256 + threadIdx.x]; r.c1.v[l] = lds[(slot * 18 + BN_NL + l) * 256 + threadIdx.x]; }
    return r;
  }
  __device__ __forceinline__ Fp ld(int e) const {
    Fp r;
    uint32_t eu = __builtin_amdgcn_readfirstlane((uint32_t)e);
    const bool hi = eu >= (uint32_t)RLC_HI;
    if (hi) eu -= (uint32_t)RLC_HI;
    const uint32_t vo = hi ? voff_hi : voff_lo;
#pragma unroll
    for (int l = 0; l < BN_NL; l++) r.v[l] = __builtin_amdgcn_raw_buffer_load_b32(rsrc, vo, (eu * (uint32_t)BN_NL + (uint32_t)l) * row_bytes, 0);
    return r;
  }
  __device__ __forceinline__ void st(int e, const Fp& a) const {
    uint32_t eu = __builtin_amdgcn_readfirstlane((uint32_t)e);
#pragma unroll
    for (int l = 0; l < BN_NL; l++) __builtin_amdgcn_raw_buffer_store_b32(a.v[l], rsrc, voff_lo, (eu * (uint32_t)BN_NL + (uint32_t)l) * row_bytes, 0);
  }
};
struct DevWsM {
  __amdgpu_buffer_rsrc_t rsrc;
  uint32_t row_bytes, voff0, lane, m, n, voff;
  int32_t* lds;
  __device__ __forceinline__ DevWsM(int32_t* base, uint32_t n_, uint32_t lane_, uint32_t m_, int32_t* lds_) : lane(lane_), m(m_), n(n_), lds(lds_) {
    DevWs t(base, n_, lane_);
    rsrc = t.rsrc; row_bytes = t.row_bytes; voff0 = lane_ < n_ ? lane_ * 4u : 0xfffffffcu; voff = voff0;
  }
  __device__ __forceinline__ void sel(int q) { const uint32_t i = lane + (uint32_t)q * m; voff = (lane < m && i < n) ? i * 4u : 0xfffffffcu; }
  __device__ __forceinline__ void park(int slot, const Fp2& a) const {
#pragma unroll
    for (int l = 0; l < BN_NL; l++) { lds[(slot * 18 + l) * 256 + threadIdx.x] = a.c0.v[l]; lds[(slot * 18 + BN_NL + l) * 256 + threadIdx.x] = a.c1.v[l]; }
  }
  __device__ __forceinline__ Fp2 unpark(int slot) const {
    Fp2 r;
#pragma unroll
    for (int l = 0; l < BN_NL; l++) { r.c0.v[l] = lds[(slot * 18 + l) * 256 + threadIdx.x]; r.c1.v[l] = lds[(slot * 18 + BN_NL + l) * 256 + threadIdx.x]; }
    return r;
  }
  __device__ __forceinline__ Fp ldv(int e, uint32_t vo) const {
    Fp r;
    uint32_t eu = __builtin_amdgcn_readfirstlane((uint32_t)e);
#pragma unroll
    for (int l = 0; l < BN_NL; l++) r.v[l] = __builtin_amdgcn_raw_buffer_load_b32(rsrc, vo, (eu * (uint32_t)BN_NL + (uint32_t)l) * row_bytes, 0);
    return r;
  }
  __device__ __forceinline__ void stv(int e, const Fp& a, uint32_t vo) const {
    uint32_t eu = __builtin_amdgcn_readfirstlane((uint32_t)e);
#pragma unroll
    for (int l = 0; l < BN_NL; l++) __builtin_amdgcn_raw_buffer_store_b32(a.v[l], rsrc, vo, (eu * (uint32_t)BN_NL + (uint32_t)l) * row_bytes, 0);
  }
  __device__ __forceinline__ Fp ld(int e) const { return ldv(e, voff); }
  __device__ __forceinline__ void st(int e, const Fp& a) const { stv(e, a, voff); }
  __device__ __forceinline__ Fp ld0(int e) const { return ldv(e, voff0); }
  __device__ __forceinline__ void st0(int e, const Fp& a) const { stv(e, a, voff0); }
};
template <bool DO_SQR>
__global__ void __launch_bounds__(256, 2)
k_rlc_miller_multi(int32_t* ws, uint32_t n, const uint8_t* __restrict__ status, int kind, int G, uint32_t m) {
  __shared__ int32_t park_lds[72 * 256];
  const uint32_t j = blockIdx.x * 256u + threadIdx.x;
  uint32_t deadmask = 0;
  const int g = __builtin_amdgcn_readfirstlane(G);
  for (int q = 0; q < g; q++) {
    const uint32_t i = j + (uint32_t)q * m;
    const bool live = j < m && i < n && (status[i < n ? i : n - 1] & BN254_ST_PENDING) != 0;
    if (!live) deadmask |= 1u << q;
  }
  if (__builtin_amdgcn_ballot_w64(j < m) == 0) return;
  DevWsM w(ws, n, j < m ? j : 0xffffffffu, m, park_lds);
  vm_miller_var_multi<DO_SQR>(w, __builtin_amdgcn_readfirstlane(kind), g, deadmask);
}
__global__ void __launch_bounds__(256, 2) k_rlc_init_f(int32_t* ws, uint32_t n, uint32_t m) {
  const uint32_t j = blockIdx.x * 256u + threadIdx.x;
  DevWs w(ws, n, j < m ? j : DEAD_LANE);
  w.st(VE_F, fp_one());
  for (int e = 1; e < 12; e++) w.st(VE_F + e, fp_zero());
}
__global__ void __launch_bounds__(256, 2)
k_rlc_scale(int32_t* ws, uint32_t n, const uint8_t* __restrict__ status, const uint8_t* __restrict__ inputs, int n_public, ChaChaKey key, uint32_t counter_base) {
  VM_KERNEL_PROLOGUE();
  const uint32_t ii = i < n ? i : n - 1;
  uint32_t r[4];
  chacha20_block4(r, key, counter_base + ii);
  const uint8_t* in = inputs + (size_t)ii * (size_t)n_public * 32;
  vm_rlc_scale(w, r, n_public, [&](int j, uint32_t* o) { words_from_be(o, in + 32 * j); });
}
__global__ void __launch_bounds__(256, 2)
k_rlc_neutral(int32_t* ws, uint32_t n, const uint8_t* __restrict__ status, int n_public, int with_f) {
  const uint32_t i = blockIdx.x * 256u + threadIdx.x;
  const bool dead = i < n && (status[i] & BN254_ST_PENDING) == 0;
  if (__builtin_amdgcn_ballot_w64(dead) == 0) return;
  DevWs w(ws, n, dead ? i : DEAD_LANE);
  vm_rlc_neutral(w, n_public, __builtin_amdgcn_readfirstlane(with_f) != 0);
}
__global__ void __launch_bounds__(256, 2)
k_rlc_fold(int32_t* ws, uint32_t n, uint32_t cur, uint32_t half, int n_public, int with_f) {
  __shared__ int32_t park_lds[72 * 256];
  const uint32_t j = blockIdx.x * 256u + threadIdx.x;
  const bool act = j + half < cur;
  if (__builtin_amdgcn_ballot_w64(act) == 0) return;
  DevWs2 w(ws, n, act ? j : DEAD_LANE, act ? j + half : DEAD_LANE, park_lds);
  vm_rlc_fold(w, n_public, __builtin_amdgcn_readfirstlane(with_f) != 0);
}
__global__ void __launch_bounds__(256, 2)
k_rlc_group_points(int32_t* ws, uint32_t n, uint8_t* __restrict__ grp_status, uint32_t groups, int n_public, const int32_t* __restrict__ rlc_tab,
                   const int32_t* __restrict__ msm_tab) {
  const uint32_t g = blockIdx.x * 256u + threadIdx.x;
  if (__builtin_amdgcn_ballot_w64(g < groups) == 0) return;
  DevWs w(ws, n, g < groups ? g : DEAD_LANE);
  const int fl = vm_rlc_group_points(w, n_public, [&](int b, int wi, int d) {
    return b < 2 ? msm_entry(rlc_tab, (size_t)(b * MSM_FW_WINDOWS + wi) * MSM_FW_ENTRIES + d) : msm_entry(msm_tab, (size_t)((b - 2) * MSM_FW_WINDOWS + wi) * MSM_FW_ENTRIES + d);
  });
  if (g < groups) grp_status[g] = (uint8_t)(BN254_ST_PENDING | ((fl & 1) ? BN254_ST_LINF : 0) | ((fl & 2) ? BN254_ST_LINF2 : 0) | ((fl & 4) ? BN254_ST_LINF3 : 0));
}
template <bool DO_SQR>
__global__ void __launch_bounds__(256, 2)
k_rlc_group_step(int32_t* ws, uint32_t n, const uint8_t* __restrict__ status, int e, const int32_t* __restrict__ entry0, const int32_t* __restrict__ entry1,
                 const int32_t* __restrict__ entry2) {
  __shared__ int32_t park_lds[72 * 256];
  VM_KERNEL_PROLOGUE();
  w.lds = park_lds;
  FixedLine l0, l1, l2;
  l0.m = uni_ld2(entry0); l0.c = uni_ld2(entry0 + 2 * BN_NL); l0.xc = uni_ld2(entry0 + 4 * BN_NL);
  l1.m = uni_ld2(entry1); l1.c = uni_ld2(entry1 + 2 * BN_NL); l1.xc = uni_ld2(entry1 + 4 * BN_NL);
  l2.m = uni_ld2(entry2); l2.c = uni_ld2(entry2 + 2 * BN_NL); l2.xc = uni_ld2(entry2 + 4 * BN_NL);
  vm_miller_step_fixed3<DO_SQR>(w, e, l0, VE_LX, (st & BN254_ST_LINF) != 0, l1, VE_CX, (st & BN254_ST_LINF2) != 0, l2, VE_AX, (st & BN254_ST_LINF3) != 0);
}
__global__ void __launch_bounds__(256, 2)
k_rlc_scale_wide(int32_t* ws, uint32_t n, const uint8_t* __restrict__ status, ChaChaKey key, uint32_t counter_base) {
  VM_KERNEL_PROLOGUE();
  const uint32_t ii = i < n ? i : n - 1;
// ... 62 lines not shown
__global__ void __launch_bounds__(256, 2)
k_rlc_scatter(uint8_t* __restrict__ status, uint32_t n, const uint8_t* __restrict__ grp_status, RlcPlan plan) {
  const uint32_t i = blockIdx.x * 256u + threadIdx.x;
  if (i >= n) return;
  const uint8_t st = status[i];
  if (!(st & BN254_ST_PENDING)) return;
  status[i] = grp_status[rlc_group_of(i, plan)] == BN254_ST_ACCEPT ? (uint8_t)BN254_ST_ACCEPT : (uint8_t)BN254_ST_PENDING;
}
__global__ void k_gather_rows(uint8_t* __restrict__ dst, const uint8_t* __restrict__ src, size_t src_stride, uint32_t row_bytes, const uint32_t* __restrict__ idx, uint32_t m) {
  const size_t t = (size_t)blockIdx.x * 256 + threadIdx.x;
  const uint32_t per = row_bytes / 4;
  if (t >= (size_t)m * per) return;
  const uint32_t k = (uint32_t)(t / per), c = (uint32_t)(t % per);
  const uint8_t* p = src + (size_t)idx[k] * src_stride + 4 * (size_t)c;
  uint32_t v;
  if ((((uintptr_t)src) | src_stride) & 3) v = (uint32_t)p[0] | (uint32_t)p[1] << 8 | (uint32_t)p[2] << 16 | (uint32_t)p[3] << 24;
  else v = *(const uint32_t*)p;
  ((uint32_t*)dst)[t] = v;
}
__global__ void k_scatter_status(uint8_t* __restrict__ status, const uint8_t* __restrict__ fb_status, const uint32_t* __restrict__ idx, uint32_t m) {
  const uint32_t k = blockIdx.x * 256u + threadIdx.x;
  if (k < m) status[idx[k]] = fb_status[k];
}
__global__ void __launch_bounds__(256, 2) k_g16_decompress(const uint8_t* __restrict__ src, size_t stride, uint32_t n, uint8_t* __restrict__ raw, uint8_t* __restrict__ pre) {
  const uint32_t i = blockIdx.x * 256u + threadIdx.x;
  if (i >= n) return;
  const uint8_t* p = src + (size_t)i * stride;
  uint32_t in[32], out[64];
  if (((((uintptr_t)src) | stride) & 15) == 0) {
#pragma unroll
    for (int k = 0; k < 8; k++) { const uint4 v = ((const uint4*)p)[k]; in[4 * k] = v.x; in[4 * k + 1] = v.y; in[4 * k + 2] = v.z; in[4 * k + 3] = v.w; }
  } else {
#pragma unroll
    for (int k = 0; k < 32; k++) in[k] = (uint32_t)p[4 * k] | (uint32_t)p[4 * k + 1] << 8 | (uint32_t)p[4 * k + 2] << 16 | (uint32_t)p[4 * k + 3] << 24;
  }
  const bool ok = g16_decompress_record(in, out);
  uint4* q = (uint4*)(raw + (size_t)i * 256);
#pragma unroll
  for (int k = 0; k < 16; k++) q[k] = make_uint4(out[4 * k], out[4 * k + 1], out[4 * k + 2], out[4 * k + 3]);
  pre[i] = ok ? 0 : 1;
}
__global__ void __launch_bounds__(256) k_g16_status_merge(uint8_t* __restrict__ status, const uint8_t* __restrict__ pre, uint32_t n) {
  const uint32_t i = blockIdx.x * 256u + threadIdx.x;
  if (i < n && pre[i]) status[i] = BN254_ST_MALFORMED;
}
__global__ void __launch_bounds__(256) k_sp1_public_inputs(const uint8_t* __restrict__ vkh, size_t vkh_stride, const uint8_t* __restrict__ pv, uint64_t pv_bytes,
                                                           uint64_t pv_base, const uint64_t* __restrict__ off, uint32_t n, uint8_t* __restrict__ rows,
                                                           uint8_t* __restrict__ pre) {
  const uint32_t i = blockIdx.x * 256u + threadIdx.x;
  const bool lane = i < n;
  uint64_t start = 0, len = 0;
  bool ok = false;
  if (lane) ok = sp1_range(off[i], off[i + 1], pv_base, pv_bytes, &start, &len);
  const uint64_t nb = lane ? sha256_blocks(len) : 0;
  uint32_t h[8];
  sha256_init(h);
  for (uint64_t b = 0; __ballot(b < nb) != 0; b++) sp1_sha256_block(h, pv, pv_bytes, start, len, b);
  if (!lane) return;
  uint32_t v[8], dg[8];
  sp1_load_vkey_hash(vkh + (size_t)i * vkh_stride, v);
  sp1_digest_words(h, dg);
  uint4* q = (uint4*)(rows + (size_t)i * 64);
  q[0] = make_uint4(v[0], v[1], v[2], v[3]); q[1] = make_uint4(v[4], v[5], v[6], v[7]);
  q[2] = make_uint4(dg[0], dg[1], dg[2], dg[3]); q[3] = make_uint4(dg[4], dg[5], dg[6], dg[7]);
  pre[i] = ok ? 0 : 1;
}

#define VALU_PEAK_ITERS 16384
__global__ void __launch_bounds__(256) k_valu_peak(uint32_t* out, uint32_t seed, int iters) {
  const uint32_t tid = threadIdx.x + blockIdx.x * blockDim.x;
  const uint32_t a = seed * 2654435761u + tid, b = (seed ^ 0x9e3779b9u) + tid * 7u;
  uint64_t acc[16];
#pragma unroll
  for (int i = 0; i < 16; i++) acc[i] = (uint64_t)(a + i) << 7 | (uint32_t)i;
  for (int it = 0; it < iters; it++) {
#pragma unroll
    for (int i = 0; i < 16; i++) asm volatile("v_mad_u64_u32 %0, vcc, %1, %2, %0" : "+v"(acc[i]) : "v"(a), "v"(b) : "vcc");
  }
  uint32_t x = 0;
#pragma unroll
  for (int i = 0; i < 16; i++) x ^= (uint32_t)acc[i] ^ (uint32_t)(acc[i] >> 32);
  out[tid] = x;
}

__device__ __forceinline__ Fp probe_ld_fp(const uint8_t* p) {
  uint32_t w[8];
  words_from_be(w, p);
  return fp_from_words(w);
}
__device__ __forceinline__ void probe_st_fp(uint8_t* p, const Fp& a) {
  uint32_t w[8];
  fp_to_words(w, a);
  words_to_be(p, w);
}
__global__ void __launch_bounds__(256, 2) k_dbg_fp_mul(const uint8_t* a, const uint8_t* b, uint8_t* o, size_t n) {
  size_t i = (size_t)blockIdx.x * 256 + threadIdx.x;
  if (i >= n) return;
  probe_st_fp(o + 32 * i, fp_mul(probe_ld_fp(a + 32 * i), probe_ld_fp(b + 32 * i)));
}
__global__ void __launch_bounds__(256, 2) k_dbg_load(int32_t* ws, uint32_t n, uint8_t* status, int e, const uint8_t* src, int kind) {
  const uint32_t i = blockIdx.x * 256u + threadIdx.x;
  if (i >= n) return;
  DevWs w(ws, n, i);
  if (kind == 0) {
    const int korder[6] = {0, 2, 4, 1, 3, 5};
    const uint8_t* p = src + 384 * (size_t)i;
    for (int t = 0; t < 6; t++) { w.st(e + 2 * korder[t], probe_ld_fp(p + 64 * t)); w.st(e + 2 * korder[t] + 1, probe_ld_fp(p + 64 * t + 32)); }
  } else if (kind == 1) {
    w.st(VE_AX, probe_ld_fp(src + 64 * (size_t)i)); w.st(VE_AY, probe_ld_fp(src + 64 * (size_t)i + 32));
  } else {
    const uint8_t* q = src + 128 * (size_t)i;
    w.st(VE_B + 1, probe_ld_fp(q)); w.st(VE_B, probe_ld_fp(q + 32)); w.st(VE_B + 3, probe_ld_fp(q + 64)); w.st(VE_B + 2, probe_ld_fp(q + 96));
  }
  status[i] = BN254_ST_PENDING;
}
__global__ void __launch_bounds__(256, 2) k_dbg_store(int32_t* ws, uint32_t n, int e, uint8_t* dst) {
  const uint32_t i = blockIdx.x * 256u + threadIdx.x;
  if (i >= n) return;
  DevWs w(ws, n, i);
  const int korder[6] = {0, 2, 4, 1, 3, 5};
  uint8_t* p = dst + 384 * (size_t)i;
  for (int t = 0; t < 6; t++) { probe_st_fp(p + 64 * t, w.ld(e + 2 * korder[t])); probe_st_fp(p + 64 * t + 32, w.ld(e + 2 * korder[t] + 1)); }
}
__global__ void __launch_bounds__(256, 2) k_dbg_g2_subgroup(const uint8_t* g2, uint8_t* o, size_t n) {
  size_t i = (size_t)blockIdx.x * 256 + threadIdx.x;
  if (i >= n) return;
  G2Aff q; q.x.c1 = probe_ld_fp(g2 + 128 * i); q.x.c0 = probe_ld_fp(g2 + 128 * i + 32);
  q.y.c1 = probe_ld_fp(g2 + 128 * i + 64); q.y.c0 = probe_ld_fp(g2 + 128 * i + 96);
  o[i] = (g2_on_curve(q) && g2_in_subgroup(q)) ? 1 : 0;
}

}

using namespace bn254;
static inline unsigned grid_for(size_t n) { return (unsigned)((n + 255) / 256); }

const char* const bn254_kernel_kind_names[KID_COUNT] = {
  "k_g16_prepare", "k_g16_subgroup", "k_vm_init", "k_f12_sqr", "k_f12_mul_line_fixed",
  "k_f12_mul", "k_f12_cyclo_sqr", "k_f12_conj", "k_f12_frob", "k_f12_inv", "k_g16_compare", "k_f12_copy", "k_f12_cyclo_sqr_n", "k_miller_dbl_var", "k_miller_add_var", "k_g16_msm_partial", "k_g16_msm_reduce", "k_f12_mul_line_fixed2", "k_miller_sqr_dbl_var", "k_miller_step_dbl", "k_miller_step_add", "k_coop12_miller_g16", "k_miller_run"};
struct ProfScope {
  G16Prof* p; hipStream_t s; int slot;
  ProfScope(G16Prof* p_, int kid, hipStream_t s_) : p(p_), s(s_), slot(-1) {
    if (p && ((p->mask >> kid) & 1u) && p->used < p->cap) { slot = p->used++; p->kid[slot] = (uint8_t)kid; (void)hipEventRecord(p->ev[2 * slot], s); }
  }
  ~ProfScope() { if (slot >= 0) (void)hipEventRecord(p->ev[2 * slot + 1], s); }
};
#define BN_LAUNCH(KID, KERNEL, ...) do { ProfScope ps_(prof, KID, s); hipLaunchKernelGGL(KERNEL, dim3(grid), dim3(256), 0, s, __VA_ARGS__); } while (0)
struct LaunchOps {
  int32_t* ws; uint32_t n; const uint8_t* status; unsigned grid; hipStream_t s;
  const int32_t* tab[3];
  G16Prof* prof;
  int inf_mask[3] = {BN254_ST_LINF, 0, 0};
  const G16KeyDesc* key_desc = nullptr; uint32_t n_keys = 0; const uint32_t* granule_key = nullptr;
  int uni(int x) { return x; }
  void f12_sqr(int e) { BN_LAUNCH(KID_F12_SQR, k_f12_sqr, ws, n, status, e); }
  void miller_dbl_var(int et, int e, int ep) { BN_LAUNCH(KID_MILLER_DBL_VAR, k_miller_dbl_var, ws, n, status, et, e, ep); }
  void miller_step(bool do_sqr, int kind, int st_, int et, int eb, int e, int epa, int ep0, int ep1) {
    const int32_t *t0 = tab[0] + (size_t)st_ * FIXED_LINE_DWORDS, *t1 = tab[1] + (size_t)st_ * FIXED_LINE_DWORDS;
    ProfScope ps_(prof, kind == 0 ? KID_MILLER_STEP_DBL : KID_MILLER_STEP_ADD, s);
    bn254_launch_miller_step(do_sqr, kind, ws, n, status, grid, s, et, eb, e, epa, t0, ep0, inf_mask[0], t1, ep1, inf_mask[1]);
  }
  void miller_run(int s_begin, int s_end, int et, int eb, int e, int epa, int ep0, int ep1) {
    static const MillerKinds kinds = [] { MillerKinds k; memset(&k, 0, sizeof k); for (int st_ = 0; st_ < BN_ATE_STEPS; st_++) k.nib[st_ >> 1] |= (uint8_t)(miller_step_kind(st_) << ((st_ & 1) * 4)); return k; }();
    ProfScope ps_(prof, KID_MILLER_RUN, s);
    if (key_desc) { bn254_launch_miller_run_keys(kinds, s_begin, s_end, ws, n, status, grid, s, et, eb, e, epa, key_desc, n_keys, granule_key, ep0, inf_mask[0], ep1, inf_mask[1]); return; }
    bn254_launch_miller_run(kinds, s_begin, s_end, ws, n, status, grid, s, et, eb, e, epa, tab[0], ep0, inf_mask[0], tab[1], ep1, inf_mask[1]);
  }
  void miller_run_fixed2(int s_begin, int s_end, int e, int ep0, int ep1) {
    static const MillerKinds kinds = [] { MillerKinds k; memset(&k, 0, sizeof k); for (int st_ = 0; st_ < BN_ATE_STEPS; st_++) k.nib[st_ >> 1] |= (uint8_t)(miller_step_kind(st_) << ((st_ & 1) * 4)); return k; }();
    ProfScope ps_(prof, KID_MILLER_RUN, s);
    bn254_launch_miller_run_fixed2(kinds, s_begin, s_end, ws, n, status, grid, s, e, tab[0], ep0, inf_mask[0], tab[1], ep1, inf_mask[1]);
  }
  void miller_sqr_dbl_var(int et, int e, int ep) { BN_LAUNCH(KID_MILLER_SQR_DBL_VAR, k_miller_sqr_dbl_var, ws, n, status, et, e, ep); }
  void miller_add_var(int et, int eb, int which, int e, int ep) { BN_LAUNCH(KID_MILLER_ADD_VAR, k_miller_add_var, ws, n, status, et, eb, which, e, ep); }
  void f12_mul_line_fixed(int e, int t, int st_, int ep) {
    BN_LAUNCH(KID_MUL_LINE_FIXED, k_f12_mul_line_fixed, ws, n, status, e, tab[t] + (size_t)st_ * FIXED_LINE_DWORDS, ep, inf_mask[t]);
  }
  void f12_mul_line_fixed2(int e, int st_, int ep0, int ep1) {
    BN_LAUNCH(KID_MUL_LINE_FIXED2, k_f12_mul_line_fixed2, ws, n, status, e, tab[0] + (size_t)st_ * FIXED_LINE_DWORDS, ep0, inf_mask[0],
              tab[1] + (size_t)st_ * FIXED_LINE_DWORDS, ep1, inf_mask[1]);
  }
  void f12_mul(int d, int a, int b, bool conj_b = false) { BN_LAUNCH(KID_F12_MUL, k_f12_mul, ws, n, status, d, a, b, conj_b ? 1 : 0); }
  void f12_copy(int d, int a) { BN_LAUNCH(KID_F12_COPY, k_f12_copy, ws, n, status, d, a); }
  void f12_cyclo_sqr(int d, int a) { BN_LAUNCH(KID_CYCLO_SQR, k_f12_cyclo_sqr, ws, n, status, d, a); }
  void f12_cyclo_sqr_n(int d, int a, int count) { BN_LAUNCH(KID_CYCLO_SQR_N, k_f12_cyclo_sqr_n, ws, n, status, d, a, count); }
  void f12_conj(int d, int a) { BN_LAUNCH(KID_F12_CONJ, k_f12_conj, ws, n, status, d, a); }
  void f12_frob(int d, int a, int j) { BN_LAUNCH(KID_F12_FROB, k_f12_frob, ws, n, status, d, a, j); }
  void f12_inv(int d, int a) { BN_LAUNCH(KID_F12_INV, k_f12_inv, ws, n, status, d, a); }
};
static uint8_t g_step_kinds[BN_ATE_STEPS];
static const uint8_t* step_kinds_host() {
  static bool init = false;
  if (!init) { for (int s_ = 0; s_ < BN_ATE_STEPS; s_++) g_step_kinds[s_] = (uint8_t)miller_step_kind(s_); init = true; }
  return g_step_kinds;
}

hipError_t bn254_launch_g16(const G16LaunchArgs& a, hipStream_t s, hipEvent_t* ev , G16Prof* prof) {
  unsigned grid = grid_for(a.n);
  uint32_t n = (uint32_t)a.n;
  if (ev) (void)hipEventRecord(ev[0], s);
  static const bool coop_on = [] { const char* e = getenv("BN254_COOP"); return !e || atoi(e) != 0; }();
  static const int run_steps_env = [] { const char* e = getenv("BN254_MILLER_RUN_STEPS"); int v = e ? atoi(e) : -1; return v < -1 ? -1 : v; }();
  const G16Form form = g16_launch_form(a.n, (size_t)a.n_public, a.inputs_match_key != 0, a.msm_part != nullptr, a.part_of_larger != 0,
                                       a.split_streams[0] && a.split_streams[1], coop_on, run_steps_env);
  const bool wide = form.wide, coop = form.form == G16_FORM_COOP;
  BN_LAUNCH(KID_PREPARE, k_g16_prepare, a.proofs, a.stride, a.inputs, a.n_public, n, a.ws, a.status, a.msm_tab, a.k0, a.inputs_match_key, (wide || coop) ? 1 : 0);
  if (a.strict_scalars && a.n_public > 0) hipLaunchKernelGGL(k_g16_check_scalars, dim3(grid), dim3(256), 0, s, a.inputs, a.n_public, n, a.status);
  if (wide) {
    static const int per_env = [] { const char* e = getenv("BN254_WIDE_PER"); int v = e ? atoi(e) : 0; return v >= G16_WIDE_MSM_INPUTS_PER_LANE && v <= 256 ? v : 0; }();
    const int per = per_env ? per_env : G16_WIDE_MSM_INPUTS_PER_LANE, chunks = (a.n_public + per - 1) / per;
    unsigned pg = (unsigned)(((size_t)n * chunks + 255) / 256);
    {
      ProfScope ps_(prof, KID_MSM_PARTIAL, s);
      if (a.msm_comb) {
        const size_t scalars = (size_t)n * (size_t)a.n_public;
        hipLaunchKernelGGL(k_g16_comb_digits, dim3((unsigned)((scalars + 255) / 256)), dim3(256), 0, s, a.inputs, a.n_public, n, a.msm_digits);
        hipLaunchKernelGGL(k_g16_msm_partial_comb, dim3(pg), dim3(256), 0, s, (const uint16_t*)a.msm_digits, a.n_public, n, per, chunks, (const uint8_t*)a.status, a.msm_tab, a.msm_part);
      }
      else hipLaunchKernelGGL(k_g16_msm_partial, dim3(pg), dim3(256), 0, s, a.inputs, a.n_public, n, per, chunks, (const uint8_t*)a.status, a.msm_tab, a.msm_part);
    }
    if (chunks >= 16 && a.n <= 65536) {
      ProfScope ps_(prof, KID_MSM_REDUCE, s);
      hipLaunchKernelGGL(k_g16_msm_reduce8, dim3((unsigned)((a.n + 31) / 32)), dim3(256), 0, s, (const int32_t*)a.msm_part, chunks, n, a.ws, a.status, a.k0);
    } else {
      BN_LAUNCH(KID_MSM_REDUCE, k_g16_msm_reduce, (const int32_t*)a.msm_part, chunks, n, a.ws, a.status, a.k0);
    }
  }
  if (ev) (void)hipEventRecord(ev[1], s);
  if (coop) {
    hipError_t e;
    { ProfScope ps_(prof, KID_COOP_G16, s); e = bn254_coop12_miller_g16(a.ws, a.status, a.n, a.gtab, a.dtab, a.inputs, a.n_public, a.inputs_match_key, a.msm_tab, a.k0, wide ? 1 : 0, 1, a.target, s); }
    if (e != hipSuccess) return e;
    if (ev) { (void)hipEventRecord(ev[2], s); (void)hipEventRecord(ev[3], s); (void)hipEventRecord(ev[4], s); }
    return hipGetLastError();
  }
  LaunchOps ops{a.ws, n, a.status, grid, s, {a.gtab, a.dtab, nullptr}, prof};
  BN_LAUNCH(KID_VM_INIT, k_vm_init, a.ws, n, (const uint8_t*)a.status);
  if (form.form == G16_FORM_LATENCY) {
    ops.f12_copy(VE_S1, VE_F); ops.f12_copy(VE_S2, VE_F);
    (void)hipEventRecord(a.split_ev[0], s);
    LaunchOps ob{a.ws, n, a.status, grid, a.split_streams[0], {a.gtab, a.dtab, nullptr}, nullptr};
    LaunchOps oc{a.ws, n, a.status, grid, a.split_streams[1], {a.gtab, a.dtab, nullptr}, nullptr};
    (void)hipStreamWaitEvent(ob.s, a.split_ev[0], 0); (void)hipStreamWaitEvent(oc.s, a.split_ev[0], 0);
    const uint8_t* kinds = step_kinds_host();
    for (int st_ = 0; st_ < BN_ATE_STEPS; st_++) {
      const int kind = kinds[st_];
      if (kind == 0) { if (st_ != 0) ops.miller_sqr_dbl_var(VE_T, VE_F, VE_AX); else ops.miller_dbl_var(VE_T, VE_F, VE_AX); }
      else ops.miller_add_var(VE_T, VE_B, kind - 1, VE_F, VE_AX);
      if (kind == 0 && st_ != 0) { ob.f12_sqr(VE_S1); oc.f12_sqr(VE_S2); }
      ob.f12_mul_line_fixed(VE_S1, 0, st_, VE_LX);
      oc.f12_mul_line_fixed(VE_S2, 1, st_, VE_CX);
    }
    (void)hipEventRecord(a.split_ev[1], ob.s); (void)hipEventRecord(a.split_ev[2], oc.s);
    (void)hipStreamWaitEvent(s, a.split_ev[1], 0); (void)hipStreamWaitEvent(s, a.split_ev[2], 0);
    ops.f12_mul(VE_F, VE_F, VE_S1); ops.f12_mul(VE_F, VE_F, VE_S2);
  } else {
    const int run_steps = form.run_steps;
    if (run_steps) vm_miller_program_runs(ops, run_steps);
    else vm_miller_program(ops, step_kinds_host(), true);
  }
  if (ev) (void)hipEventRecord(ev[2], s);
  BN_LAUNCH(KID_SUBGROUP, k_g16_subgroup, n, a.ws, a.status, a.inputs_match_key, (int)VE_T);
  if (ev) (void)hipEventRecord(ev[3], s);
  vm_final_exp_program(ops);
  BN_LAUNCH(KID_COMPARE, k_g16_compare, a.ws, n, a.status, a.target, BN254_ST_REJECT);
  if (ev) (void)hipEventRecord(ev[4], s);
  return hipGetLastError();
}

hipError_t bn254_launch_g16_keys(const G16KeysLaunchArgs& a, hipStream_t s) {
  unsigned grid = grid_for(a.m);
  const uint32_t n = (uint32_t)a.m;
  G16Prof* prof = nullptr;
  static const int run_steps_env = [] { const char* e = getenv("BN254_MILLER_RUN_STEPS"); int v = e ? atoi(e) : -1; return v < 1 ? -1 : v; }();
  bn254_launch_g16_prepare_keys(a, grid, s);
  LaunchOps ops{a.ws, n, a.slot_status, grid, s, {nullptr, nullptr, nullptr}, prof};
  ops.key_desc = a.desc; ops.n_keys = a.n_keys; ops.granule_key = a.granule_key;
  BN_LAUNCH(KID_VM_INIT, k_vm_init, a.ws, n, (const uint8_t*)a.slot_status);
  vm_miller_program_runs(ops, g16_launch_form(a.m, 0, true, false, a.part_of_larger != 0, false, false, run_steps_env).run_steps);
  bn254_launch_g16_subgroup_keys(a, grid, s, (int)VE_T);
  vm_final_exp_program(ops);
  bn254_launch_g16_compare_keys(a, grid, s);
  return hipGetLastError();
}

hipError_t bn254_launch_g16_rlc(const G16LaunchArgs& a, const RlcLaunchArgs& r, hipStream_t s) {
  unsigned grid = grid_for(a.n);
  uint32_t n = (uint32_t)a.n;
  G16Prof* prof = nullptr;
  ChaChaKey key;
  for (int i = 0; i < 8; i++) key.k[i] = r.key[i];
  for (int i = 0; i < 3; i++) key.nonce[i] = r.key[8 + i];
  BN_LAUNCH(KID_PREPARE, k_g16_prepare, a.proofs, a.stride, a.inputs, a.n_public, n, a.ws, a.status, a.msm_tab, a.k0, a.inputs_match_key, 1);
  if (a.strict_scalars && a.n_public > 0) hipLaunchKernelGGL(k_g16_check_scalars, dim3(grid), dim3(256), 0, s, a.inputs, a.n_public, n, a.status);
  LaunchOps ops{a.ws, n, a.status, grid, s, {nullptr, nullptr, nullptr}, nullptr};
  BN_LAUNCH(KID_VM_INIT, k_vm_init, a.ws, n, (const uint8_t*)a.status);
  const bool wide = r.grp_rows != nullptr;
  const int slots = wide ? 0 : a.n_public;
  if (wide) hipLaunchKernelGGL(k_rlc_scale_wide, dim3(grid), dim3(256), 0, s, a.ws, n, (const uint8_t*)a.status, key, r.counter_base);
  else hipLaunchKernelGGL(k_rlc_scale, dim3(grid), dim3(256), 0, s, a.ws, n, (const uint8_t*)a.status, a.inputs, a.n_public, key, r.counter_base);
  const uint8_t* kinds = step_kinds_host();
  const int share = 1 << r.plan.pre;
  if (share == 1) {
    vm_miller_program(ops, kinds, false);
  } else {
    const uint32_t m = r.plan.lanes;
    const unsigned mgrid = grid_for(m);
    hipLaunchKernelGGL(k_rlc_init_f, dim3(mgrid), dim3(256), 0, s, a.ws, n, m);
    for (int st_ = 0; st_ < BN_ATE_STEPS; st_++) {
      const int kind = kinds[st_];
      if (kind == 0 && st_ != 0) hipLaunchKernelGGL(k_rlc_miller_multi<true>, dim3(mgrid), dim3(256), 0, s, a.ws, n, (const uint8_t*)a.status, kind, share, m);
      else hipLaunchKernelGGL(k_rlc_miller_multi<false>, dim3(mgrid), dim3(256), 0, s, a.ws, n, (const uint8_t*)a.status, kind, share, m);
    }
  }
  BN_LAUNCH(KID_SUBGROUP, k_g16_subgroup, n, a.ws, a.status, a.inputs_match_key, (int)VE_T);
  hipLaunchKernelGGL(k_rlc_neutral, dim3(grid), dim3(256), 0, s, a.ws, n, (const uint8_t*)a.status, slots, share == 1 ? 1 : 0);
  uint32_t cur = n;
  for (int k = 0; k < r.plan.rounds; k++) {
    const uint32_t half = r.plan.half[k];
    hipLaunchKernelGGL(k_rlc_fold, dim3(grid_for(cur - half)), dim3(256), 0, s, a.ws, n, cur, half, slots, k >= r.plan.pre ? 1 : 0);
    cur = half;
  }
  const uint32_t groups = r.plan.groups;
  const unsigned ggrid = grid_for(groups);
  if (wide) {
    const size_t lanes = (size_t)groups * (size_t)a.n_public;
    hipLaunchKernelGGL(k_rlc_group_scalars, dim3((unsigned)((lanes + 255) / 256)), dim3(256), 0, s, (const int32_t*)a.ws, n, (const uint8_t*)a.status, a.inputs, a.n_public, r.plan, r.grp_rows);
    (void)hipMemsetAsync(r.grp_status, BN254_ST_PENDING, ((size_t)groups + 255) / 256 * 256, s);
    const int per = G16_WIDE_MSM_INPUTS_PER_LANE, chunks = r.msm_form == 2 ? 0 : (a.n_public + per - 1) / per;
    const unsigned pg = (unsigned)(((size_t)groups * chunks + 255) / 256);
    if (r.msm_form == 0) {
      hipLaunchKernelGGL(k_g16_comb_digits, dim3((unsigned)((lanes + 255) / 256)), dim3(256), 0, s, (const uint8_t*)r.grp_rows, a.n_public, groups, r.grp_digits);
      hipLaunchKernelGGL(k_g16_msm_partial_comb, dim3(pg), dim3(256), 0, s, (const uint16_t*)r.grp_digits, a.n_public, groups, per, chunks, (const uint8_t*)r.grp_status, a.msm_tab, r.grp_part);
    } else if (r.msm_form == 1) {
      hipLaunchKernelGGL(k_g16_msm_partial, dim3(pg), dim3(256), 0, s, (const uint8_t*)r.grp_rows, a.n_public, groups, per, chunks, (const uint8_t*)r.grp_status, a.msm_tab, r.grp_part);
    }
    hipLaunchKernelGGL(k_rlc_group_points_wide, dim3(ggrid), dim3(256), 0, s, a.ws, n, r.grp_status, groups, a.n_public, r.rlc_tab, a.msm_tab, (const uint8_t*)r.grp_rows,
                       (const int32_t*)r.grp_part, chunks, r.msm_form);
  } else {
    (void)hipMemsetAsync(r.grp_status, 0, ((size_t)groups + 255) / 256 * 256, s);
    hipLaunchKernelGGL(k_rlc_group_points, dim3(ggrid), dim3(256), 0, s, a.ws, n, r.grp_status, groups, a.n_public, r.rlc_tab, a.msm_tab);
  }
  LaunchOps gops{a.ws, n, r.grp_status, ggrid, s, {a.gtab, a.dtab, r.btab}, nullptr};
  gops.inf_mask[0] = BN254_ST_LINF; gops.inf_mask[1] = BN254_ST_LINF2; gops.inf_mask[2] = BN254_ST_LINF3;
  for (int st_ = 0; st_ < BN_ATE_STEPS; st_++) {
    const int32_t *t0 = a.gtab + (size_t)st_ * FIXED_LINE_DWORDS, *t1 = a.dtab + (size_t)st_ * FIXED_LINE_DWORDS, *t2 = r.btab + (size_t)st_ * FIXED_LINE_DWORDS;
    if (kinds[st_] == 0 && st_ != 0) hipLaunchKernelGGL(k_rlc_group_step<true>, dim3(ggrid), dim3(256), 0, s, a.ws, n, (const uint8_t*)r.grp_status, (int)RLC_ACC, t0, t1, t2);
    else hipLaunchKernelGGL(k_rlc_group_step<false>, dim3(ggrid), dim3(256), 0, s, a.ws, n, (const uint8_t*)r.grp_status, (int)RLC_ACC, t0, t1, t2);
  }
  gops.f12_mul(VE_F, VE_F, RLC_ACC);
  vm_final_exp_program(gops);
  { unsigned grid = ggrid; BN_LAUNCH(KID_COMPARE, k_g16_compare, a.ws, n, r.grp_status, r.one, BN254_ST_REJECT); }
  hipLaunchKernelGGL(k_rlc_scatter, dim3(grid), dim3(256), 0, s, a.status, n, (const uint8_t*)r.grp_status, r.plan);
  return hipGetLastError();
}
hipError_t bn254_launch_gather_rows(uint8_t* dst, const uint8_t* src, size_t src_stride, uint32_t row_bytes, const uint32_t* idx, uint32_t m, hipStream_t s) {
  const size_t threads = (size_t)m * (row_bytes / 4);
  if (threads) hipLaunchKernelGGL(k_gather_rows, dim3((unsigned)((threads + 255) / 256)), dim3(256), 0, s, dst, src, src_stride, row_bytes, idx, m);
  return hipGetLastError();
}
hipError_t bn254_launch_scatter_status(uint8_t* status, const uint8_t* fb_status, const uint32_t* idx, uint32_t m, hipStream_t s) {
  if (m) hipLaunchKernelGGL(k_scatter_status, dim3(grid_for(m)), dim3(256), 0, s, status, fb_status, idx, m);
  return hipGetLastError();
}
hipError_t bn254_launch_g16_decompress(const uint8_t* src, size_t stride, uint32_t n, uint8_t* raw, uint8_t* pre, hipStream_t s) {
  if (n) hipLaunchKernelGGL(k_g16_decompress, dim3(grid_for(n)), dim3(256), 0, s, src, stride, n, raw, pre);
  return hipGetLastError();
}
hipError_t bn254_launch_g16_status_merge(uint8_t* status, const uint8_t* pre, uint32_t n, hipStream_t s) {
  if (n) hipLaunchKernelGGL(k_g16_status_merge, dim3(grid_for(n)), dim3(256), 0, s, status, pre, n);
  return hipGetLastError();
}
hipError_t bn254_launch_sp1_public_inputs(const uint8_t* vkh, size_t vkh_stride, const uint8_t* pv, uint64_t pv_bytes, uint64_t pv_base, const uint64_t* off, uint32_t n,
                                          uint8_t* rows, uint8_t* pre, hipStream_t s) {
  if (n) hipLaunchKernelGGL(k_sp1_public_inputs, dim3(grid_for(n)), dim3(256), 0, s, vkh, vkh_stride, pv, pv_bytes, pv_base, off, n, rows, pre);
  return hipGetLastError();
}
double bn254_measure_valu_peak(int reps) {
  hipDeviceProp_t p;
  int dev = 0;
  if (hipGetDevice(&dev) != hipSuccess || hipGetDeviceProperties(&p, dev) != hipSuccess) return 0.0;
  const int grid = p.multiProcessorCount * 4;
  uint32_t* out = nullptr;
  if (hipMalloc((void**)&out, (size_t)grid * 256 * 4) != hipSuccess) return 0.0;
  hipEvent_t e0, e1;
  (void)hipEventCreate(&e0); (void)hipEventCreate(&e1);
  hipLaunchKernelGGL(k_valu_peak, dim3(grid), dim3(256), 0, nullptr, out, 1u, VALU_PEAK_ITERS);
  float best = 1e30f;
  int since_best = 0;
  for (int r = 0; r < 200 && since_best < reps; r++) {
    (void)hipEventRecord(e0, nullptr);
    hipLaunchKernelGGL(k_valu_peak, dim3(grid), dim3(256), 0, nullptr, out, (uint32_t)(r + 2), VALU_PEAK_ITERS);
    (void)hipEventRecord(e1, nullptr);
    if (hipEventSynchronize(e1) != hipSuccess) { best = 1e30f; break; }
    float ms = 0.f;
    since_best++;
    if (hipEventElapsedTime(&ms, e0, e1) == hipSuccess && ms > 0.f && ms < best * 0.998f) { best = ms; since_best = 0; }
  }
  (void)hipEventDestroy(e0); (void)hipEventDestroy(e1); (void)hipFree(out);
  if (best > 1e29f) return 0.0;
  return (double)grid * 256.0 * (double)VALU_PEAK_ITERS * 16.0 / ((double)best * 1e-3);
}
double bn254_measure_valu_sustained(double ms_target) {
  hipDeviceProp_t p;
  int dev = 0;
  if (hipGetDevice(&dev) != hipSuccess || hipGetDeviceProperties(&p, dev) != hipSuccess) return 0.0;
  const int grid = p.multiProcessorCount * 4;
  uint32_t* out = nullptr;
  if (hipMalloc((void**)&out, (size_t)grid * 256 * 4) != hipSuccess) return 0.0;
  int launches = (int)(ms_target / 2.0);
  if (launches < 4) launches = 4;
  if (launches > 1000) launches = 1000;
  hipEvent_t e0, e1;
  (void)hipEventCreate(&e0); (void)hipEventCreate(&e1);
  (void)hipEventRecord(e0, nullptr);
  for (int r = 0; r < launches; r++) hipLaunchKernelGGL(k_valu_peak, dim3(grid), dim3(256), 0, nullptr, out, (uint32_t)(r + 1), VALU_PEAK_ITERS);
  (void)hipEventRecord(e1, nullptr);
  float ms = 0.f;
  const bool ok = hipEventSynchronize(e1) == hipSuccess && hipEventElapsedTime(&ms, e0, e1) == hipSuccess && ms > 0.f;
  (void)hipEventDestroy(e0); (void)hipEventDestroy(e1); (void)hipFree(out);
  return ok ? (double)launches * grid * 256.0 * (double)VALU_PEAK_ITERS * 16.0 / ((double)ms * 1e-3) : 0.0;
}
hipError_t bn254_launch_dbg_fp_mul(const uint8_t* a, const uint8_t* b, uint8_t* o, size_t n, hipStream_t s) {
  hipLaunchKernelGGL(k_dbg_fp_mul, dim3(grid_for(n)), dim3(256), 0, s, a, b, o, n);
  return hipGetLastError();
}
hipError_t bn254_launch_dbg_fp12_op(int op, const uint8_t* a, const uint8_t* b, uint8_t* o, size_t n, int32_t* ws, uint8_t* status, hipStream_t s) {
  unsigned g = grid_for(n);
  uint32_t nn = (uint32_t)n;
  LaunchOps ops{ws, nn, status, g, s, {nullptr, nullptr, nullptr}, nullptr};
  hipLaunchKernelGGL(k_dbg_load, dim3(g), dim3(256), 0, s, ws, nn, status, (int)VE_F, a, 0);
  if (op == 0) { hipLaunchKernelGGL(k_dbg_load, dim3(g), dim3(256), 0, s, ws, nn, status, (int)VE_S1, b, 0); ops.f12_mul(VE_S0, VE_F, VE_S1); }
  else if (op == 1) { ops.f12_sqr(VE_F); ops.f12_conj(VE_S0, VE_F); ops.f12_conj(VE_S0, VE_S0); }
  else if (op == 2) ops.f12_inv(VE_S0, VE_F);
  else if (op == 3) {
// ... 77 lines not shown
```

### snark-bn254-verifier_amd/csrc/bn254_vm.h

```cpp
#pragma once
#include "bn254_pairing.h"

namespace bn254 {

enum {
  VE_AX = 0, VE_AY = 1, VE_B = 2 , VE_CX = 6, VE_CY = 7, VE_LX = 8, VE_LY = 9,
  VE_F = 10,
  VE_T = 22,
  VE_S0 = 22, VE_S1 = 34, VE_S2 = 46, VE_S3 = 58, VE_S4 = 70,
  VE_P3 = 82,
  VE_TMPA = 94, VE_TMPB = 100,
  VE_P5 = 106, VE_P7 = 118,
  VE_COUNT = 130
};

template <class W> BN_HD Fp2 vld2(W& w, int e) { Fp2 r; r.c0 = w.ld(e); r.c1 = w.ld(e + 1); return r; }
template <class W> BN_HD void vst2(W& w, int e, const Fp2& a) { w.st(e, a.c0); w.st(e + 1, a.c1); }
template <class W> BN_HD Fp6 vld6(W& w, int e) { Fp6 r; r.c0 = vld2(w, e); r.c1 = vld2(w, e + 2); r.c2 = vld2(w, e + 4); return r; }
template <class W> BN_HD void vst6(W& w, int e, const Fp6& a) { vst2(w, e, a.c0); vst2(w, e + 2, a.c1); vst2(w, e + 4, a.c2); }

template <class W>
BN_HD void vm_f12_sqr(W& w, int e) {
  Fp2 k0 = vld2(w, e), k1 = vld2(w, e + 2), k2 = vld2(w, e + 4), k3 = vld2(w, e + 6), k4 = vld2(w, e + 8), k5 = vld2(w, e + 10);
  Fp2 x3 = fp2_mul_xi(k3), x4 = fp2_mul_xi(k4), x5 = fp2_mul_xi(k5);
  vst2(w, e, fp2_dotp(pp(k0, k0), pp2(k1, x5), pp2(k2, x4), pp(k3, x3)));
  vst2(w, e + 2, fp2_dotp(pp2(k0, k1), pp2(k2, x5), pp2(k3, x4)));
  vst2(w, e + 4, fp2_dotp(pp2(k0, k2), pp(k1, k1), pp2(k3, x5), pp(k4, x4)));
  vst2(w, e + 6, fp2_dotp(pp2(k0, k3), pp2(k1, k2), pp2(k4, x5)));
  vst2(w, e + 8, fp2_dotp(pp2(k0, k4), pp2(k1, k3), pp(k2, k2), pp(k5, x5)));
  vst2(w, e + 10, fp2_dotp(pp2(k0, k5), pp2(k1, k4), pp2(k2, k3)));
}
template <class W>
BN_HD void vm_f12_mul_line_fixed(W& w, int e, const FixedLine& l, int e_px, bool inf) {
  Fp px = w.ld(e_px), d0 = w.ld(e_px + 1);
  Fp2 d3 = fp2_mul_fp(l.m, px);
  Fp2 x3 = fp2_mul_xi(d3);
  const Fp2 &d4 = l.c, &x4 = l.xc;
  Fp2 k0 = vld2(w, e), k1 = vld2(w, e + 2), k2 = vld2(w, e + 4), k3 = vld2(w, e + 6), k4 = vld2(w, e + 8), k5 = vld2(w, e + 10);
  vst2(w, e, fp2_select(inf, k0, fp2_dotk(kfp(k0, d0), kp(x3, k5), kp(x4, k3))));
  vst2(w, e + 2, fp2_select(inf, k1, fp2_dotk(kfp(k1, d0), kp(d3, k0), kp(x4, k4))));
  vst2(w, e + 4, fp2_select(inf, k2, fp2_dotk(kfp(k2, d0), kp(d3, k1), kp(x4, k5))));
  vst2(w, e + 6, fp2_select(inf, k3, fp2_dotk(kfp(k3, d0), kp(d3, k2), kp(d4, k0))));
  vst2(w, e + 8, fp2_select(inf, k4, fp2_dotk(kfp(k4, d0), kp(d3, k3), kp(d4, k1))));
  vst2(w, e + 10, fp2_select(inf, k5, fp2_dotk(kfp(k5, d0), kp(d3, k4), kp(d4, k2))));
}
template <class W>
BN_HD void vm_f12_mul_line_fixed2(W& w, int e, const FixedLine& l1, int e_px1, bool inf1, const FixedLine& l2, int e_px2, bool inf2) {
  Fp2 r4, r5;
  {
    Fp px = w.ld(e_px1), d0 = w.ld(e_px1 + 1);
    Fp2 d3 = fp2_mul_fp(l1.m, px);
    Fp2 x3 = fp2_mul_xi(d3);
    const Fp2 &d4 = l1.c, &x4 = l1.xc;
    Fp2 k0 = vld2(w, e), k1 = vld2(w, e + 2), k2 = vld2(w, e + 4), k3 = vld2(w, e + 6), k4 = vld2(w, e + 8), k5 = vld2(w, e + 10);
    w.park(0, fp2_select(inf1, k0, fp2_dot_line(d0, k0, x3, k5, x4, k3)));
    w.park(1, fp2_select(inf1, k1, fp2_dot_line(d0, k1, d3, k0, x4, k4)));
    w.park(2, fp2_select(inf1, k2, fp2_dot_line(d0, k2, d3, k1, x4, k5)));
    w.park(3, fp2_select(inf1, k3, fp2_dot_line(d0, k3, d3, k2, d4, k0)));
    r4 = fp2_select(inf1, k4, fp2_dot_line(d0, k4, d3, k3, d4, k1));
    r5 = fp2_select(inf1, k5, fp2_dot_line(d0, k5, d3, k4, d4, k2));
  }
  {
    Fp px = w.ld(e_px2), d0 = w.ld(e_px2 + 1);
    Fp2 d3 = fp2_mul_fp(l2.m, px);
    Fp2 x3 = fp2_mul_xi(d3);
    const Fp2 &d4 = l2.c, &x4 = l2.xc;
    Fp2 k0 = w.unpark(0), k1 = w.unpark(1), k2 = w.unpark(2), k3 = w.unpark(3);
    const Fp2 &k4 = r4, &k5 = r5;
    vst2(w, e, fp2_select(inf2, k0, fp2_dotk(kfp(k0, d0), kp(x3, k5), kp(x4, k3))));
    vst2(w, e + 2, fp2_select(inf2, k1, fp2_dotk(kfp(k1, d0), kp(d3, k0), kp(x4, k4))));
    vst2(w, e + 4, fp2_select(inf2, k2, fp2_dotk(kfp(k2, d0), kp(d3, k1), kp(x4, k5))));
    vst2(w, e + 6, fp2_select(inf2, k3, fp2_dotk(kfp(k3, d0), kp(d3, k2), kp(d4, k0))));
    vst2(w, e + 8, fp2_select(inf2, k4, fp2_dotk(kfp(k4, d0), kp(d3, k3), kp(d4, k1))));
    vst2(w, e + 10, fp2_select(inf2, k5, fp2_dotk(kfp(k5, d0), kp(d3, k4), kp(d4, k2))));
  }
}
template <class W>
BN_HD void vm_f12_mul_line_regs(W& w, int e, const G2Line& l, int e_px) {
  Fp px = w.ld(e_px), py = w.ld(e_px + 1);
  Fp2 d0 = fp2_mul_fp(l.r0, py), d3 = fp2_mul_fp(l.r1, px), d4 = l.r2;
  Fp2 x3 = fp2_mul_xi(d3), x4 = fp2_mul_xi(d4);
  Fp2 k0 = vld2(w, e), k1 = vld2(w, e + 2), k2 = vld2(w, e + 4), k3 = vld2(w, e + 6), k4 = vld2(w, e + 8), k5 = vld2(w, e + 10);
  vst2(w, e, fp2_dotp(pp(d0, k0), pp(x3, k5), pp(x4, k3)));
  vst2(w, e + 2, fp2_dotp(pp(d0, k1), pp(d3, k0), pp(x4, k4)));
  vst2(w, e + 4, fp2_dotp(pp(d0, k2), pp(d3, k1), pp(x4, k5)));
  vst2(w, e + 6, fp2_dotp(pp(d0, k3), pp(d3, k2), pp(d4, k0)));
  vst2(w, e + 8, fp2_dotp(pp(d0, k4), pp(d3, k3), pp(d4, k1)));
  vst2(w, e + 10, fp2_dotp(pp(d0, k5), pp(d3, k4), pp(d4, k2)));
}
template <class W>
BN_HD void vm_miller_dbl_var(W& w, int e_t, int e, int e_px) {
  G2Proj t; t.x = vld2(w, e_t); t.y = vld2(w, e_t + 2); t.z = vld2(w, e_t + 4);
  G2Line l = g2_double_step(t);
  vst2(w, e_t, t.x); vst2(w, e_t + 2, t.y); vst2(w, e_t + 4, t.z);
  vm_f12_mul_line_regs(w, e, l, e_px);
}
template <class W>
BN_HD void vm_miller_add_var(W& w, int e_t, int e_b, int which, int e, int e_px) {
  G2Aff q; q.x = vld2(w, e_b); q.y = vld2(w, e_b + 2);
  if (which == 1) q = g2_neg(q);
  else if (which == 2) q = g2_psi_affine(q);
  else if (which == 3) q = g2_neg(g2_psi2_affine(q));
  G2Proj t; t.x = vld2(w, e_t); t.y = vld2(w, e_t + 2); t.z = vld2(w, e_t + 4);
  G2Line l = g2_add_step(t, q);
  vst2(w, e_t, t.x); vst2(w, e_t + 2, t.y); vst2(w, e_t + 4, t.z);
  vm_f12_mul_line_regs(w, e, l, e_px);
}

template <class W>
BN_HD void vm_miller_sqr_dbl_var(W& w, int e_t, int e, int e_px) {
  Fp2 r4, r5;
  {
    Fp2 k0 = vld2(w, e), k1 = vld2(w, e + 2), k2 = vld2(w, e + 4), k3 = vld2(w, e + 6), k4 = vld2(w, e + 8), k5 = vld2(w, e + 10);
    Fp2 x3 = fp2_mul_xi(k3), x4 = fp2_mul_xi(k4), x5 = fp2_mul_xi(k5);
    w.park(0, fp2_dotp(pp(k0, k0), pp2(k1, x5), pp2(k2, x4), pp(k3, x3)));
    w.park(1, fp2_dotp(pp2(k0, k1), pp2(k2, x5), pp2(k3, x4)));
    w.park(2, fp2_dotp(pp2(k0, k2), pp(k1, k1), pp2(k3, x5), pp(k4, x4)));
    w.park(3, fp2_dotp(pp2(k0, k3), pp2(k1, k2), pp2(k4, x5)));
    r4 = fp2_dotp(pp2(k0, k4), pp2(k1, k3), pp(k2, k2), pp(k5, x5));
    r5 = fp2_dotp(pp2(k0, k5), pp2(k1, k4), pp2(k2, k3));
  }
  G2Line l;
  {
    G2Proj t; t.x = vld2(w, e_t); t.y = vld2(w, e_t + 2); t.z = vld2(w, e_t + 4);
    l = g2_double_step(t);
    vst2(w, e_t, t.x); vst2(w, e_t + 2, t.y); vst2(w, e_t + 4, t.z);
  }
  BN_SCHED_FENCE();
  Fp px = w.ld(e_px), py = w.ld(e_px + 1);
  Fp2 d0 = fp2_mul_fp(l.r0, py), d3 = fp2_mul_fp(l.r1, px), d4 = l.r2;
  Fp2 x3 = fp2_mul_xi(d3), x4 = fp2_mul_xi(d4);
  BN_SCHED_FENCE();
  Fp2 k0 = w.unpark(0), k1 = w.unpark(1), k2 = w.unpark(2), k3 = w.unpark(3);
  const Fp2 &k4 = r4, &k5 = r5;
  vst2(w, e, fp2_dotp(pp(d0, k0), pp(x3, k5), pp(x4, k3)));
  vst2(w, e + 2, fp2_dotp(pp(d0, k1), pp(d3, k0), pp(x4, k4)));
  vst2(w, e + 4, fp2_dotp(pp(d0, k2), pp(d3, k1), pp(x4, k5)));
  vst2(w, e + 6, fp2_dotp(pp(d0, k3), pp(d3, k2), pp(d4, k0)));
  vst2(w, e + 8, fp2_dotp(pp(d0, k4), pp(d3, k3), pp(d4, k1)));
  vst2(w, e + 10, fp2_dotp(pp(d0, k5), pp(d3, k4), pp(d4, k2)));
}

template <bool DO_SQR, class W>
BN_HD void vm_miller_step(W& w, int kind, int e_t, int e_b, int e, int e_pa, const FixedLine& l0, int e_p0, bool inf0,
                          const FixedLine& l1, int e_p1, bool inf1) {
  Fp2 f4, f5;
  if constexpr (DO_SQR) {
    Fp2 k0 = vld2(w, e), k1 = vld2(w, e + 2), k2 = vld2(w, e + 4), k3 = vld2(w, e + 6), k4 = vld2(w, e + 8), k5 = vld2(w, e + 10);
    Fp2 x3 = fp2_mul_xi(k3), x4 = fp2_mul_xi(k4), x5 = fp2_mul_xi(k5);
    w.park(0, fp2_dotp(pp(k0, k0), pp2(k1, x5), pp2(k2, x4), pp(k3, x3)));
    w.park(1, fp2_dotp(pp2(k0, k1), pp2(k2, x5), pp2(k3, x4)));
    w.park(2, fp2_dotp(pp2(k0, k2), pp(k1, k1), pp2(k3, x5), pp(k4, x4)));
    w.park(3, fp2_dotp(pp2(k0, k3), pp2(k1, k2), pp2(k4, x5)));
    f4 = fp2_dotp(pp2(k0, k4), pp2(k1, k3), pp(k2, k2), pp(k5, x5));
    f5 = fp2_dotp(pp2(k0, k5), pp2(k1, k4), pp2(k2, k3));
  }
  G2Line l;
  {
    G2Proj t; t.x = vld2(w, e_t); t.y = vld2(w, e_t + 2); t.z = vld2(w, e_t + 4);
    if (kind == 0) {
      l = g2_double_step(t);
    } else {
      G2Aff q; q.x = vld2(w, e_b); q.y = vld2(w, e_b + 2);
      if (kind == 2) q = g2_neg(q);
      else if (kind == 3) q = g2_psi_affine(q);
      else if (kind == 4) q = g2_neg(g2_psi2_affine(q));
      l = g2_add_step(t, q);
    }
    vst2(w, e_t, t.x); vst2(w, e_t + 2, t.y); vst2(w, e_t + 4, t.z);
  }
  {
    Fp px = w.ld(e_pa), py = w.ld(e_pa + 1);
    Fp2 d0 = fp2_mul_fp(l.r0, py), d3 = fp2_mul_fp(l.r1, px), d4 = l.r2;
    Fp2 x3 = fp2_mul_xi(d3), x4 = fp2_mul_xi(d4);
    Fp2 k0, k1, k2, k3, k4, k5;
    if constexpr (DO_SQR) { k0 = w.unpark(0); k1 = w.unpark(1); k2 = w.unpark(2); k3 = w.unpark(3); k4 = f4; k5 = f5; }
    else { k0 = vld2(w, e); k1 = vld2(w, e + 2); k2 = vld2(w, e + 4); k3 = vld2(w, e + 6); k4 = vld2(w, e + 8); k5 = vld2(w, e + 10); }
    w.park(0, fp2_dotp(pp(d0, k0), pp(x3, k5), pp(x4, k3)));
    w.park(1, fp2_dotp(pp(d0, k1), pp(d3, k0), pp(x4, k4)));
    w.park(2, fp2_dotp(pp(d0, k2), pp(d3, k1), pp(x4, k5)));
    w.park(3, fp2_dotp(pp(d0, k3), pp(d3, k2), pp(d4, k0)));
    Fp2 n4 = fp2_dotp(pp(d0, k4), pp(d3, k3), pp(d4, k1));
    f5 = fp2_dotp(pp(d0, k5), pp(d3, k4), pp(d4, k2));
    f4 = n4;
  }
  {
    Fp px = w.ld(e_p0), d0 = w.ld(e_p0 + 1);
    Fp2 d3 = fp2_mul_fp(l0.m, px);
    Fp2 x3 = fp2_mul_xi(d3);
    const Fp2 &d4 = l0.c, &x4 = l0.xc;
    Fp2 k0 = w.unpark(0), k1 = w.unpark(1), k2 = w.unpark(2), k3 = w.unpark(3), k4 = f4, k5 = f5;
    w.park(0, fp2_select(inf0, k0, fp2_dot_line(d0, k0, x3, k5, x4, k3)));
    w.park(1, fp2_select(inf0, k1, fp2_dot_line(d0, k1, d3, k0, x4, k4)));
    w.park(2, fp2_select(inf0, k2, fp2_dot_line(d0, k2, d3, k1, x4, k5)));
    w.park(3, fp2_select(inf0, k3, fp2_dot_line(d0, k3, d3, k2, d4, k0)));
    f4 = fp2_select(inf0, k4, fp2_dot_line(d0, k4, d3, k3, d4, k1));
    f5 = fp2_select(inf0, k5, fp2_dot_line(d0, k5, d3, k4, d4, k2));
  }
  {
    Fp px = w.ld(e_p1), d0 = w.ld(e_p1 + 1);
    Fp2 d3 = fp2_mul_fp(l1.m, px);
    Fp2 x3 = fp2_mul_xi(d3);
    const Fp2 &d4 = l1.c, &x4 = l1.xc;
    Fp2 k0 = w.unpark(0), k1 = w.unpark(1), k2 = w.unpark(2), k3 = w.unpark(3);
    const Fp2 &k4 = f4, &k5 = f5;
    vst2(w, e, fp2_select(inf1, k0, fp2_dotk(kfp(k0, d0), kp(x3, k5), kp(x4, k3))));
    vst2(w, e + 2, fp2_select(inf1, k1, fp2_dotk(kfp(k1, d0), kp(d3, k0), kp(x4, k4))));
    vst2(w, e + 4, fp2_select(inf1, k2, fp2_dotk(kfp(k2, d0), kp(d3, k1), kp(x4, k5))));
    vst2(w, e + 6, fp2_select(inf1, k3, fp2_dotk(kfp(k3, d0), kp(d3, k2), kp(d4, k0))));
    vst2(w, e + 8, fp2_select(inf1, k4, fp2_dotk(kfp(k4, d0), kp(d3, k3), kp(d4, k1))));
    vst2(w, e + 10, fp2_select(inf1, k5, fp2_dotk(kfp(k5, d0), kp(d3, k4), kp(d4, k2))));
  }
}

template <class W> BN_HD void mf_load(W& w, int e, Fp2& f4, Fp2& f5) {
  w.park(0, vld2(w, e)); w.park(1, vld2(w, e + 2)); w.park(2, vld2(w, e + 4)); w.park(3, vld2(w, e + 6));
  f4 = vld2(w, e + 8); f5 = vld2(w, e + 10);
}
template <class W> BN_HD void mf_store(W& w, int e, const Fp2& f4, const Fp2& f5) {
  vst2(w, e, w.unpark(0)); vst2(w, e + 2, w.unpark(1)); vst2(w, e + 4, w.unpark(2)); vst2(w, e + 6, w.unpark(3));
  vst2(w, e + 8, f4); vst2(w, e + 10, f5);
}
template <class W> BN_HD void mf_sqr(W& w, Fp2& f4, Fp2& f5) {
  Fp2 k0 = w.unpark(0), k1 = w.unpark(1), k2 = w.unpark(2), k3 = w.unpark(3), k4 = f4, k5 = f5;
  Fp2 x3 = fp2_mul_xi(k3), x4 = fp2_mul_xi(k4), x5 = fp2_mul_xi(k5);
  w.park(0, fp2_dotp(pp(k0, k0), pp2(k1, x5), pp2(k2, x4), pp(k3, x3)));
  w.park(1, fp2_dotp(pp2(k0, k1), pp2(k2, x5), pp2(k3, x4)));
  w.park(2, fp2_dotp(pp2(k0, k2), pp(k1, k1), pp2(k3, x5), pp(k4, x4)));
  w.park(3, fp2_dotp(pp2(k0, k3), pp2(k1, k2), pp2(k4, x5)));
  Fp2 n4 = fp2_dotp(pp2(k0, k4), pp2(k1, k3), pp(k2, k2), pp(k5, x5));
  f5 = fp2_dotp(pp2(k0, k5), pp2(k1, k4), pp2(k2, k3));
  f4 = n4;
}
template <class W> BN_HD G2Line mf_g2(W& w, int kind, int e_t, int e_b) {
  G2Line l;
  G2Proj t; t.x = vld2(w, e_t); t.y = vld2(w, e_t + 2); t.z = vld2(w, e_t + 4);
  if (kind == 0) {
    l = g2_double_step(t);
  } else {
    G2Aff q; q.x = vld2(w, e_b); q.y = vld2(w, e_b + 2);
    if (kind == 2) q = g2_neg(q);
    else if (kind == 3) q = g2_psi_affine(q);
    else if (kind == 4) q = g2_neg(g2_psi2_affine(q));
    l = g2_add_step(t, q);
  }
  vst2(w, e_t, t.x); vst2(w, e_t + 2, t.y); vst2(w, e_t + 4, t.z);
  return l;
}
template <class W> BN_HD void mf_line_var(W& w, const G2Line& l, int e_pa, Fp2& f4, Fp2& f5) {
  Fp px = w.ld(e_pa), py = w.ld(e_pa + 1);
  Fp2 d0 = fp2_mul_fp(l.r0, py), d3 = fp2_mul_fp(l.r1, px), d4 = l.r2;
  Fp2 x3 = fp2_mul_xi(d3), x4 = fp2_mul_xi(d4);
  Fp2 k0 = w.unpark(0), k1 = w.unpark(1), k2 = w.unpark(2), k3 = w.unpark(3), k4 = f4, k5 = f5;
  w.park(0, fp2_dotp(pp(d0, k0), pp(x3, k5), pp(x4, k3)));
  w.park(1, fp2_dotp(pp(d0, k1), pp(d3, k0), pp(x4, k4)));
  w.park(2, fp2_dotp(pp(d0, k2), pp(d3, k1), pp(x4, k5)));
  w.park(3, fp2_dotp(pp(d0, k3), pp(d3, k2), pp(d4, k0)));
  Fp2 n4 = fp2_dotp(pp(d0, k4), pp(d3, k3), pp(d4, k1));
  f5 = fp2_dotp(pp(d0, k5), pp(d3, k4), pp(d4, k2));
  f4 = n4;
}
template <class W> BN_HD void mf_line_fixed(W& w, const FixedLine& l0, int e_p0, bool inf0, Fp2& f4, Fp2& f5) {
  Fp px = w.ld(e_p0), d0 = w.ld(e_p0 + 1);
  Fp2 d3 = fp2_mul_fp(l0.m, px);
  Fp2 x3 = fp2_mul_xi(d3);
  const Fp2 &d4 = l0.c, &x4 = l0.xc;
  Fp2 k0 = w.unpark(0), k1 = w.unpark(1), k2 = w.unpark(2), k3 = w.unpark(3), k4 = f4, k5 = f5;
  w.park(0, fp2_select(inf0, k0, fp2_dot_line(d0, k0, x3, k5, x4, k3)));
  w.park(1, fp2_select(inf0, k1, fp2_dot_line(d0, k1, d3, k0, x4, k4)));
  w.park(2, fp2_select(inf0, k2, fp2_dot_line(d0, k2, d3, k1, x4, k5)));
  w.park(3, fp2_select(inf0, k3, fp2_dot_line(d0, k3, d3, k2, d4, k0)));
  f4 = fp2_select(inf0, k4, fp2_dot_line(d0, k4, d3, k3, d4, k1));
  f5 = fp2_select(inf0, k5, fp2_dot_line(d0, k5, d3, k4, d4, k2));
}
template <class W> BN_HD void mf_line_fixed_k(W& w, const FixedLine& l1, int e_p1, bool inf1, Fp2& f4, Fp2& f5) {
  Fp px = w.ld(e_p1), d0 = w.ld(e_p1 + 1);
  Fp2 d3 = fp2_mul_fp(l1.m, px);
  Fp2 x3 = fp2_mul_xi(d3);
  const Fp2 &d4 = l1.c, &x4 = l1.xc;
  Fp2 k0 = w.unpark(0), k1 = w.unpark(1), k2 = w.unpark(2), k3 = w.unpark(3);
  const Fp2 k4 = f4, k5 = f5;
  w.park(0, fp2_select(inf1, k0, fp2_dotk(kfp(k0, d0), kp(x3, k5), kp(x4, k3))));
  w.park(1, fp2_select(inf1, k1, fp2_dotk(kfp(k1, d0), kp(d3, k0), kp(x4, k4))));
  w.park(2, fp2_select(inf1, k2, fp2_dotk(kfp(k2, d0), kp(d3, k1), kp(x4, k5))));
  w.park(3, fp2_select(inf1, k3, fp2_dotk(kfp(k3, d0), kp(d3, k2), kp(d4, k0))));
  f4 = fp2_select(inf1, k4, fp2_dotk(kfp(k4, d0), kp(d3, k3), kp(d4, k1)));
  f5 = fp2_select(inf1, k5, fp2_dotk(kfp(k5, d0), kp(d3, k4), kp(d4, k2)));
}
template <class W, class LINES, class KINDS>
BN_HD void vm_miller_run(W& w, const LINES& lines, const KINDS& kinds, int s_begin, int s_end, int e_t, int e_b, int e, int e_pa, int e_p0, bool inf0, int e_p1, bool inf1) {
  Fp2 f4, f5;
  mf_load(w, e, f4, f5);
  for (int s = s_begin; s < s_end; s++) {
    const int kind = kinds.get(s);
    if (kind == 0) {
      if (s != 0) mf_sqr(w, f4, f5);
      BN_SCHED_FENCE();
      G2Line l = mf_g2(w, 0, e_t, e_b);
      mf_line_var(w, l, e_pa, f4, f5);
    } else {
      G2Line l = mf_g2(w, kind, e_t, e_b);
      mf_line_var(w, l, e_pa, f4, f5);
    }
    BN_SCHED_FENCE();
    mf_line_fixed(w, lines.get(0, s), e_p0, inf0, f4, f5);
    mf_line_fixed_k(w, lines.get(1, s), e_p1, inf1, f4, f5);
  }
  mf_store(w, e, f4, f5);
}

template <class W, class LINES, class KINDS>
BN_HD void vm_miller_run_fixed2(W& w, const LINES& lines, const KINDS& kinds, int s_begin, int s_end, int e, int e_p0, bool inf0, int e_p1, bool inf1) {
  Fp2 f4, f5;
  mf_load(w, e, f4, f5);
  for (int s = s_begin; s < s_end; s++) {
    if (kinds.get(s) == 0 && s != 0) mf_sqr(w, f4, f5);
    BN_SCHED_FENCE();
    mf_line_fixed(w, lines.get(0, s), e_p0, inf0, f4, f5);
    mf_line_fixed_k(w, lines.get(1, s), e_p1, inf1, f4, f5);
  }
  mf_store(w, e, f4, f5);
}

template <class W>
BN_HD bool vm_g2_ate_check(W& w, int e_t, int e_b) {
  G2Aff b; b.x = vld2(w, e_b); b.y = vld2(w, e_b + 2);
  Fp2 sx = fp2_mul(fp2_conj(b.x), frob_coeff(3, 2));
  Fp2 sy = fp2_neg(fp2_mul(fp2_conj(b.y), frob_coeff(3, 3)));
  Fp2 X = vld2(w, e_t), Y = vld2(w, e_t + 2), Z = vld2(w, e_t + 4);
  return !fp2_is_zero(Z) & fp2_eq(X, fp2_mul(sx, Z)) & fp2_eq(Y, fp2_mul(sy, Z));
}

template <class W> BN_HD Fp6 vld_half(W& w, int e, int h) { Fp6 r; r.c0 = vld2(w, e + 2 * h); r.c1 = vld2(w, e + 4 + 2 * h); r.c2 = vld2(w, e + 8 + 2 * h); return r; }
template <class W> BN_HD void vst_half(W& w, int e, int h, const Fp6& a) { vst2(w, e + 2 * h, a.c0); vst2(w, e + 4 + 2 * h, a.c1); vst2(w, e + 8 + 2 * h, a.c2); }
template <class W>
BN_HD void vm_f12_mul(W& w, int e_dst, int e_a, int e_b, bool conj_b = false) {
  { Fp6 v0 = fp6_mul(vld_half(w, e_a, 0), vld_half(w, e_b, 0)); w.park(0, v0.c0); w.park(1, v0.c1); w.park(2, v0.c2); }
  BN_SCHED_FENCE();
  Fp6 a1 = vld_half(w, e_a, 1), b1 = vld_half(w, e_b, 1);
  if (conj_b) b1 = fp6_neg(b1);
  Fp6 c0;
  {
    const Fp6 v1 = fp6_mul(a1, b1);
    BN_SCHED_FENCE();
    { const Fp2 x = w.unpark(0); c0.c0 = fp2_add(x, fp2_mul_xi(v1.c2)); w.park(0, fp2_add(x, v1.c0)); }
    { const Fp2 x = w.unpark(1); c0.c1 = fp2_add(x, v1.c0); w.park(1, fp2_add(x, v1.c1)); }
    { const Fp2 x = w.unpark(2); c0.c2 = fp2_add(x, v1.c1); w.park(2, fp2_add(x, v1.c2)); }
  }
  BN_SCHED_FENCE();
  a1 = fp6_add(vld_half(w, e_a, 0), a1);
  b1 = fp6_add(vld_half(w, e_b, 0), b1);
  vst_half(w, e_dst, 0, c0);
  BN_SCHED_FENCE();
  const Fp6 s = fp6_mul(a1, b1);
  BN_SCHED_FENCE();
  Fp6 c1;
  c1.c0 = fp2_sub(s.c0, w.unpark(0)); c1.c1 = fp2_sub(s.c1, w.unpark(1)); c1.c2 = fp2_sub(s.c2, w.unpark(2));
  vst_half(w, e_dst, 1, c1);
}
template <class W>
BN_HD void vm_f12_cyclo_sqr(W& w, int e_dst, int e_src) {
  {
    Fp2 k0 = vld2(w, e_src), k3 = vld2(w, e_src + 6);
    Fp2 za, zb;
    gs_pair(za, zb, k0, k3, k0, k3, false);
    vst2(w, e_dst, za); vst2(w, e_dst + 6, zb);
  }
  {
    Fp2 k1 = vld2(w, e_src + 2), k2 = vld2(w, e_src + 4), k4 = vld2(w, e_src + 8), k5 = vld2(w, e_src + 10);
    Fp2 z2, z5, z4, z1;
    gs_pair(z2, z5, k1, k4, k2, k5, false);
    gs_pair(z4, z1, k2, k5, k4, k1, true);
    vst2(w, e_dst + 4, z2); vst2(w, e_dst + 10, z5); vst2(w, e_dst + 8, z4); vst2(w, e_dst + 2, z1);
  }
}
template <class W>
BN_HD void vm_f12_cyclo_sqr_n(W& w, int e_dst, int e_src, int count) {
  Fp2 k0 = vld2(w, e_src), k1 = vld2(w, e_src + 2), k2 = vld2(w, e_src + 4), k3 = vld2(w, e_src + 6), k4 = vld2(w, e_src + 8), k5 = vld2(w, e_src + 10);
  for (int it = 0; it < count; it++) {
    Fp2 n0, n3, n2, n5, n4, n1;
    gs_pair(n0, n3, k0, k3, k0, k3, false);
    k0 = n0; k3 = n3;
    gs_pair(n2, n5, k1, k4, k2, k5, false);
    gs_pair(n4, n1, k2, k5, k4, k1, true);
    k1 = n1; k2 = n2; k4 = n4; k5 = n5;
  }
  vst2(w, e_dst, k0); vst2(w, e_dst + 2, k1); vst2(w, e_dst + 4, k2); vst2(w, e_dst + 6, k3); vst2(w, e_dst + 8, k4); vst2(w, e_dst + 10, k5);
}
template <class W>
BN_HD void vm_f12_copy(W& w, int e_dst, int e_src) { for (int k = 0; k < 12; k++) w.st(e_dst + k, w.ld(e_src + k)); }
template <class W>
BN_HD void vm_f12_conj(W& w, int e_dst, int e_src) {
  for (int k = 0; k < 6; k++) { Fp2 x = vld2(w, e_src + 2 * k); vst2(w, e_dst + 2 * k, (k & 1) ? fp2_neg(x) : x); }
}
template <class W>
BN_HD void vm_f12_frob(W& w, int e_dst, int e_src, int j) {
  const bool odd = (j & 1) != 0;
  for (int k = 0; k < 6; k++) {
    Fp2 x = vld2(w, e_src + 2 * k);
    if (odd) x = fp2_conj(x);
    if (k > 0) { Fp2 c = frob_coeff(j, k); x = (j == 2) ? fp2_mul_fp(x, c.c0) : fp2_mul(x, c); }
    vst2(w, e_dst + 2 * k, x);
  }
}
template <class W>
BN_HD void vm_f12_inv(W& w, int e_dst, int e_src) {
  Fp6 d;
  {
    Fp6 s0 = fp6_sqr(vld_half(w, e_src, 0));
    Fp6 s1 = fp6_mul_v(fp6_sqr(vld_half(w, e_src, 1)));
    d = fp6_sub(s0, s1);
  }
  Fp6 di = fp6_inv(d);
  { Fp6 r0 = fp6_mul_plain(vld_half(w, e_src, 0), di); Fp6 r1 = fp6_neg(fp6_mul_plain(vld_half(w, e_src, 1), di)); vst_half(w, e_dst, 0, r0); vst_half(w, e_dst, 1, r1); }
}
template <class W>
BN_HD bool vm_f12_eq_const(W& w, int e, const int32_t* target ) {
  bool ok = true;
  for (int k = 0; k < 12; k++) {
    Fp t;
#pragma unroll
    for (int l = 0; l < BN_NL; l++) t.v[l] = target[k * BN_NL + l];
    BN_SETB(t, 1.0, 0.5);
    ok &= fp_eq(w.ld(e + k), t);
  }
  return ok;
}

BN_HD int miller_step_kind(int s) {
  int idx = 0;
  for (int it = 1; it < BN_ATE_NAF_LEN; it++) {
    if (idx == s) return 0;
    idx++;
    int d = BN_ATE_NAF[it];
    if (d != 0) { if (idx == s) return d > 0 ? 1 : 2; idx++; }
  }
  return s == idx ? 3 : 4;
}

template <class OPS>
BN_HD void vm_miller_program(OPS& ops, const uint8_t* step_kinds , bool with_fixed_pairs = true) {
  for (int s = 0; s < BN_ATE_STEPS; s++) {
    int kind = ops.uni(step_kinds[s]);
    if (with_fixed_pairs) {
      ops.miller_step(kind == 0 && s != 0, kind, s, VE_T, VE_B, VE_F, VE_AX, VE_LX, VE_CX);
      continue;
    }
    if (kind == 0) { if (s != 0) ops.miller_sqr_dbl_var(VE_T, VE_F, VE_AX); else ops.miller_dbl_var(VE_T, VE_F, VE_AX); }
    else ops.miller_add_var(VE_T, VE_B, kind - 1, VE_F, VE_AX);
  }
}
template <class OPS>
BN_HD void vm_miller_program_runs(OPS& ops, int per_run) {
  if (per_run < 1) per_run = 1;
  for (int s = 0; s < BN_ATE_STEPS; s += per_run)
    ops.miller_run(s, s + per_run < BN_ATE_STEPS ? s + per_run : BN_ATE_STEPS, VE_T, VE_B, VE_F, VE_AX, VE_LX, VE_CX);
}
template <class OPS>
BN_HD void vm_exp_u(OPS& ops, int e_dst, int e_src) {
  ops.f12_cyclo_sqr(e_dst, e_src);
  ops.f12_mul(VE_P3, e_dst, e_src, false);
  ops.f12_mul(VE_P5, VE_P3, e_dst, false);
  ops.f12_mul(VE_P7, VE_P5, e_dst, false);
  int run = 0, first = 1;
  for (int i = 1; i < BN_U_W4_LEN; i++) {
    run++;
    int d = BN_U_W4[i];
    if (d != 0) {
      ops.f12_cyclo_sqr_n(e_dst, first ? e_src : e_dst, run);
      run = 0; first = 0;
      int a = d < 0 ? -d : d;
      ops.f12_mul(e_dst, e_dst, a == 1 ? e_src : a == 3 ? VE_P3 : a == 5 ? VE_P5 : VE_P7, d < 0);
    }
  }
}
template <class OPS>
BN_HD void vm_final_exp_program(OPS& ops) {
  ops.f12_inv(VE_S0, VE_F);
  ops.f12_conj(VE_S1, VE_F);
  ops.f12_mul(VE_S0, VE_S1, VE_S0, false);
  ops.f12_frob(VE_S1, VE_S0, 2);
  ops.f12_mul(VE_F, VE_S1, VE_S0);
  vm_exp_u(ops, VE_S0, VE_F); ops.f12_conj(VE_S0, VE_S0);
  ops.f12_cyclo_sqr(VE_S0, VE_S0);
  ops.f12_cyclo_sqr(VE_S1, VE_S0);
  ops.f12_mul(VE_S1, VE_S0, VE_S1);
  vm_exp_u(ops, VE_S2, VE_S1); ops.f12_conj(VE_S2, VE_S2);
  ops.f12_conj(VE_S3, VE_S1);
  ops.f12_mul(VE_S1, VE_S2, VE_S3);
  ops.f12_cyclo_sqr(VE_S3, VE_S2);
  vm_exp_u(ops, VE_S4, VE_S3);
  ops.f12_mul(VE_S4, VE_S1, VE_S4);
  ops.f12_mul(VE_S3, VE_S0, VE_S4);
  ops.f12_mul(VE_S0, VE_S2, VE_S4);
  ops.f12_mul(VE_S0, VE_F, VE_S0);
  ops.f12_frob(VE_S2, VE_S3, 1); ops.f12_mul(VE_S0, VE_S2, VE_S0);
  ops.f12_frob(VE_S2, VE_S4, 2); ops.f12_mul(VE_S0, VE_S2, VE_S0);
  ops.f12_conj(VE_S2, VE_F); ops.f12_mul(VE_S2, VE_S2, VE_S3);
  ops.f12_frob(VE_S2, VE_S2, 3);
  ops.f12_mul(VE_S0, VE_S2, VE_S0);
}

}
```

Measured before the change: 5.928 million.

## Fold conjugations into mul/sqr operands and fuse subgroup check and final compare into kernels

Conjugation of an Fp12 operand is now carried as a flag bit on the element index and applied inside f12_mul and cyclotomic squaring, which removes separate conj passes and workspace round-trips in the final exponentiation. The G2 subgroup ate check is folded into the last Miller-run launch, and the final Fp12 multiply is merged with the equality-against-target verdict into one kernel. The two fixed-line helpers are unified into one. Together these cut kernel launches and global memory traffic, at the cost of more branching in hot kernels and added register and LDS pressure in the fused kernels.

```diff
diff --git a/snark-bn254-verifier_amd/csrc/bn254_coop12.hip b/snark-bn254-verifier_amd/csrc/bn254_coop12.hip
--- a/snark-bn254-verifier_amd/csrc/bn254_coop12.hip
+++ b/snark-bn254-verifier_amd/csrc/bn254_coop12.hip
@@ -160,10 +160,16 @@
   const Coop12& co;
   __device__ __forceinline__ void f12_inv(int d, int a) { c12_inv(co, C12_SLOT(d), C12_SLOT(a)); }
   __device__ __forceinline__ void f12_conj(int d, int a) { c12_conj(co, C12_SLOT(d), C12_SLOT(a)); }
-  __device__ __forceinline__ void f12_mul(int d, int a, int b, bool conj_b = false) { c12_mul(co, C12_SLOT(d), C12_SLOT(a), C12_SLOT(b), conj_b); }
+  __device__ __forceinline__ void f12_mul(int d, int a, int b, bool conj_b = false) {
+    c12_mul(co, C12_SLOT(d), C12_SLOT(ve_elem(a)), C12_SLOT(b), conj_b != ve_conj(a));
+    if (ve_conj(a)) c12_conj(co, C12_SLOT(d), C12_SLOT(d));
+  }
   __device__ __forceinline__ void f12_frob(int d, int a, int j) { c12_frob(co, C12_SLOT(d), C12_SLOT(a), j); }
-  __device__ __forceinline__ void f12_cyclo_sqr(int d, int a) { c12_cyclo_sqr_n(co, C12_SLOT(d), C12_SLOT(a), 1); }
-  __device__ __forceinline__ void f12_cyclo_sqr_n(int d, int a, int count) { c12_cyclo_sqr_n(co, C12_SLOT(d), C12_SLOT(a), count); }
+  __device__ __forceinline__ void f12_cyclo_sqr(int d, int a) { f12_cyclo_sqr_n(d, a, 1); }
+  __device__ __forceinline__ void f12_cyclo_sqr_n(int d, int a, int count) {
+    c12_cyclo_sqr_n(co, C12_SLOT(d), C12_SLOT(ve_elem(a)), count);
+    if (ve_conj(a)) c12_conj(co, C12_SLOT(d), C12_SLOT(d));
+  }
 };
 
 __device__ __forceinline__ Fp c12_ws_ld(const int32_t* ws, uint32_t n, uint32_t p, int e) {
diff --git a/snark-bn254-verifier_amd/csrc/bn254_devws.h b/snark-bn254-verifier_amd/csrc/bn254_devws.h
--- a/snark-bn254-verifier_amd/csrc/bn254_devws.h
+++ b/snark-bn254-verifier_amd/csrc/bn254_devws.h
@@ -102,5 +102,11 @@
   if (__builtin_amdgcn_ballot_w64((st & BN254_ST_PENDING) != 0) == 0) return;                   \
   DevWs w(ws, n, i < n ? i : DEAD_LANE)
 
+__device__ __forceinline__ uint8_t g16_subgroup_status(uint8_t st, bool in_g2, int inputs_match_key) {
+  if (!in_g2) return BN254_ST_NOT_IN_SUBGROUP;
+  if (st & 0x3f) return st & 0x3f;
+  if (!inputs_match_key) return BN254_ST_INPUT_LEN;
+  return BN254_ST_PENDING | (st & BN254_ST_LINF);
+}
 
 }
diff --git a/snark-bn254-verifier_amd/csrc/bn254_k_keys.hip b/snark-bn254-verifier_amd/csrc/bn254_k_keys.hip
--- a/snark-bn254-verifier_amd/csrc/bn254_k_keys.hip
+++ b/snark-bn254-verifier_amd/csrc/bn254_k_keys.hip
@@ -201,31 +201,10 @@
   if (bad) slot_status[i] = BN254_ST_NOT_MEMBER;
 }
 
-#define VM_KEYS_PROLOGUE()                                                                       \
-  const uint32_t i = blockIdx.x * 256u + threadIdx.x;                                           \
-  if ((i & ~63u) >= n) return;                                                                   \
-  const uint8_t st = status[i < n ? i : n - 1];                                                 \
-  if (__builtin_amdgcn_ballot_w64((st & BN254_ST_PENDING) != 0) == 0) return;                   \
-  DevWs w(ws, n, i < n ? i : DEAD_LANE)
-
 __global__ void __launch_bounds__(256, 2)
-k_g16_subgroup_keys(uint32_t n, int32_t* ws, uint8_t* __restrict__ status, const uint32_t* __restrict__ granule_key, const G16KeyDesc* __restrict__ desc, uint32_t n_keys, int e_t) {
-  VM_KEYS_PROLOGUE();
-  const int inputs_match_key = keys_view(desc, granule_key, i & ~63u, n_keys).inputs_match;
-  bool ok = vm_g2_ate_check(w, e_t, VE_B);
-  if (i < n && (st & BN254_ST_PENDING)) {
-    uint8_t out;
-    if (!ok) out = BN254_ST_NOT_IN_SUBGROUP;
-    else if (st & 0x3f) out = st & 0x3f;
-    else if (!inputs_match_key) out = BN254_ST_INPUT_LEN;
-    else out = BN254_ST_PENDING | (st & BN254_ST_LINF);
-    status[i] = out;
-  }
-}
-
-__global__ void __launch_bounds__(256, 2)
-k_g16_compare_keys(int32_t* ws, uint32_t n, const uint8_t* __restrict__ status, const uint32_t* __restrict__ slot_to_proof, const uint32_t* __restrict__ granule_key,
-                   const G16KeyDesc* __restrict__ desc, uint32_t n_keys, uint32_t n_proofs, uint8_t* __restrict__ out_status) {
+k_f12_mul_verdict_keys(int32_t* ws, uint32_t n, const uint8_t* __restrict__ status, const uint32_t* __restrict__ slot_to_proof, const uint32_t* __restrict__ granule_key,
+                       const G16KeyDesc* __restrict__ desc, uint32_t n_keys, uint32_t n_proofs, uint8_t* __restrict__ out_status, int e_dst, int e_a, int e_b) {
+  __shared__ int32_t park_lds[72 * 256];
   const uint32_t i = blockIdx.x * 256u + threadIdx.x;
   if ((i & ~63u) >= n) return;
   const uint8_t st = status[i < n ? i : n - 1];
@@ -233,8 +212,9 @@
   uint8_t out = st;
   if (__builtin_amdgcn_ballot_w64((st & BN254_ST_PENDING) != 0) != 0) {
     DevWs w(ws, n, i < n ? i : DEAD_LANE);
+    w.lds = park_lds;
     const int32_t* target = keys_view(desc, granule_key, i & ~63u, n_keys).target;
-    const bool acc = vm_f12_eq_const(w, VE_S0, target);
+    const bool acc = vm_f12_mul_eq_const(w, e_dst, e_a, e_b, target);
     if (st & BN254_ST_PENDING) out = acc ? BN254_ST_ACCEPT : BN254_ST_REJECT;
   }
   if (i < n && st != 0) { const uint32_t pi = slot_to_proof[i]; if (pi < n_proofs) out_status[pi] = out; }
@@ -262,10 +242,7 @@
     hipLaunchKernelGGL(k_g16_check_scalars_keys, dim3(grid), dim3(256), 0, s, a.inputs, a.input_stride, a.n_proofs, (uint32_t)a.m, a.slot_to_proof, a.granule_key, a.desc, a.n_keys,
                        a.slot_status);
 }
-void bn254_launch_g16_subgroup_keys(const G16KeysLaunchArgs& a, unsigned grid, hipStream_t s, int e_t) {
-  hipLaunchKernelGGL(k_g16_subgroup_keys, dim3(grid), dim3(256), 0, s, (uint32_t)a.m, a.ws, a.slot_status, a.granule_key, a.desc, a.n_keys, e_t);
-}
-void bn254_launch_g16_compare_keys(const G16KeysLaunchArgs& a, unsigned grid, hipStream_t s) {
-  hipLaunchKernelGGL(k_g16_compare_keys, dim3(grid), dim3(256), 0, s, a.ws, (uint32_t)a.m, (const uint8_t*)a.slot_status, a.slot_to_proof, a.granule_key, a.desc, a.n_keys, a.n_proofs,
-                     a.status);
-}
+void bn254_launch_f12_mul_verdict_keys(const G16KeysLaunchArgs& a, unsigned grid, hipStream_t s, int e_dst, int e_a, int e_b) {
+  hipLaunchKernelGGL(k_f12_mul_verdict_keys, dim3(grid), dim3(256), 0, s, a.ws, (uint32_t)a.m, (const uint8_t*)a.slot_status, a.slot_to_proof, a.granule_key, a.desc, a.n_keys,
+                     a.n_proofs, a.status, e_dst, e_a, e_b);
+}
diff --git a/snark-bn254-verifier_amd/csrc/bn254_k_miller.hip b/snark-bn254-verifier_amd/csrc/bn254_k_miller.hip
--- a/snark-bn254-verifier_amd/csrc/bn254_k_miller.hip
+++ b/snark-bn254-verifier_amd/csrc/bn254_k_miller.hip
@@ -40,21 +40,23 @@
   MillerKinds k;
   __device__ __forceinline__ int get(int s) const { return __builtin_amdgcn_readfirstlane((k.nib[s >> 1] >> ((s & 1) * 4)) & 15); }
 };
-__global__ void __launch_bounds__(256, 2) k_miller_run(int32_t* ws, uint32_t n, const uint8_t* __restrict__ status, MillerKinds kinds, int s_begin, int s_end,
+__global__ void __launch_bounds__(256, 2) k_miller_run(int32_t* ws, uint32_t n, uint8_t* status, MillerKinds kinds, int s_begin, int s_end,
                                                        int e_t, int e_b, int e, int e_pa, const int32_t* __restrict__ tab0, int e_p0, int inf_mask0,
-                                                       const int32_t* __restrict__ tab1, int e_p1, int inf_mask1) {
+                                                       const int32_t* __restrict__ tab1, int e_p1, int inf_mask1, int fold, int inputs_match_key) {
   __shared__ int32_t park_lds[72 * 256];
   VM_KERNEL_PROLOGUE();
   w.lds = park_lds;
   DevLines lines{uni_ptr(tab0), uni_ptr(tab1)};
   DevKinds dk{kinds};
-  vm_miller_run(w, lines, dk, __builtin_amdgcn_readfirstlane(s_begin), __builtin_amdgcn_readfirstlane(s_end), e_t, e_b, e, e_pa, e_p0, (st & inf_mask0) != 0,
-                e_p1, (st & inf_mask1) != 0);
+  const int s_last = __builtin_amdgcn_readfirstlane(s_end), fl = __builtin_amdgcn_readfirstlane(fold);
+  const bool in_g2 = vm_miller_run(w, lines, dk, __builtin_amdgcn_readfirstlane(s_begin), s_last, e_t, e_b, e, e_pa, e_p0, (st & inf_mask0) != 0,
+                                   e_p1, (st & inf_mask1) != 0, fl);
+  if ((fl & MR_FOLD_ATE) && s_last == BN_ATE_STEPS && i < n && (st & BN254_ST_PENDING)) status[i] = g16_subgroup_status(st, in_g2, inputs_match_key);
 }
 
-__global__ void __launch_bounds__(256, 2) k_miller_run_keys(int32_t* ws, uint32_t n, const uint8_t* __restrict__ status, MillerKinds kinds, int s_begin, int s_end,
+__global__ void __launch_bounds__(256, 2) k_miller_run_keys(int32_t* ws, uint32_t n, uint8_t* status, MillerKinds kinds, int s_begin, int s_end,
                                                             int e_t, int e_b, int e, int e_pa, const G16KeyDesc* __restrict__ desc, uint32_t n_keys,
-                                                            const uint32_t* __restrict__ granule_key, int e_p0, int inf_mask0, int e_p1, int inf_mask1) {
+                                                            const uint32_t* __restrict__ granule_key, int e_p0, int inf_mask0, int e_p1, int inf_mask1, int fold) {
   __shared__ int32_t park_lds[72 * 256];
   if (((blockIdx.x * 256u + threadIdx.x) & ~63u) >= n) return;
   VM_KERNEL_PROLOGUE();
@@ -62,8 +64,10 @@
   const KeyView kv = keys_view(desc, granule_key, i & ~63u, n_keys);
   DevLines lines{kv.gtab, kv.dtab};
   DevKinds dk{kinds};
-  vm_miller_run(w, lines, dk, __builtin_amdgcn_readfirstlane(s_begin), __builtin_amdgcn_readfirstlane(s_end), e_t, e_b, e, e_pa, e_p0, (st & inf_mask0) != 0,
-                e_p1, (st & inf_mask1) != 0);
+  const int s_last = __builtin_amdgcn_readfirstlane(s_end), fl = __builtin_amdgcn_readfirstlane(fold);
+  const bool in_g2 = vm_miller_run(w, lines, dk, __builtin_amdgcn_readfirstlane(s_begin), s_last, e_t, e_b, e, e_pa, e_p0, (st & inf_mask0) != 0,
+                                   e_p1, (st & inf_mask1) != 0, fl);
+  if ((fl & MR_FOLD_ATE) && s_last == BN_ATE_STEPS && i < n && (st & BN254_ST_PENDING)) status[i] = g16_subgroup_status(st, in_g2, kv.inputs_match);
 }
 
 __global__ void __launch_bounds__(256, 2) k_miller_run_fixed2(int32_t* ws, uint32_t n, const uint8_t* __restrict__ status, MillerKinds kinds, int s_begin, int s_end, int e,
@@ -83,13 +87,13 @@
                                     const int32_t* tab0, int ep0, int inf0, const int32_t* tab1, int ep1, int inf1) {
   hipLaunchKernelGGL(k_miller_run_fixed2, dim3(grid), dim3(256), 0, s, ws, n, status, kinds, s_begin, s_end, e, tab0, ep0, inf0, tab1, ep1, inf1);
 }
-void bn254_launch_miller_run(const MillerKinds& kinds, int s_begin, int s_end, int32_t* ws, uint32_t n, const uint8_t* status, unsigned grid, hipStream_t s, int et, int eb,
-                             int e, int epa, const int32_t* tab0, int ep0, int inf0, const int32_t* tab1, int ep1, int inf1) {
-  hipLaunchKernelGGL(k_miller_run, dim3(grid), dim3(256), 0, s, ws, n, status, kinds, s_begin, s_end, et, eb, e, epa, tab0, ep0, inf0, tab1, ep1, inf1);
+void bn254_launch_miller_run(const MillerKinds& kinds, int s_begin, int s_end, int32_t* ws, uint32_t n, uint8_t* status, unsigned grid, hipStream_t s, int et, int eb,
+                             int e, int epa, const int32_t* tab0, int ep0, int inf0, const int32_t* tab1, int ep1, int inf1, int fold, int inputs_match_key) {
+  hipLaunchKernelGGL(k_miller_run, dim3(grid), dim3(256), 0, s, ws, n, status, kinds, s_begin, s_end, et, eb, e, epa, tab0, ep0, inf0, tab1, ep1, inf1, fold, inputs_match_key);
 }
-void bn254_launch_miller_run_keys(const MillerKinds& kinds, int s_begin, int s_end, int32_t* ws, uint32_t n, const uint8_t* status, unsigned grid, hipStream_t s, int et, int eb,
-                                  int e, int epa, const G16KeyDesc* desc, uint32_t n_keys, const uint32_t* granule_key, int ep0, int inf0, int ep1, int inf1) {
-  hipLaunchKernelGGL(k_miller_run_keys, dim3(grid), dim3(256), 0, s, ws, n, status, kinds, s_begin, s_end, et, eb, e, epa, desc, n_keys, granule_key, ep0, inf0, ep1, inf1);
+void bn254_launch_miller_run_keys(const MillerKinds& kinds, int s_begin, int s_end, int32_t* ws, uint32_t n, uint8_t* status, unsigned grid, hipStream_t s, int et, int eb,
+                                  int e, int epa, const G16KeyDesc* desc, uint32_t n_keys, const uint32_t* granule_key, int ep0, int inf0, int ep1, int inf1, int fold) {
+  hipLaunchKernelGGL(k_miller_run_keys, dim3(grid), dim3(256), 0, s, ws, n, status, kinds, s_begin, s_end, et, eb, e, epa, desc, n_keys, granule_key, ep0, inf0, ep1, inf1, fold);
 }
 void bn254_launch_miller_step(bool do_sqr, int kind, int32_t* ws, uint32_t n, const uint8_t* status, unsigned grid, hipStream_t s, int et, int eb, int e, int epa,
                               const int32_t* t0, int ep0, int inf0, const int32_t* t1, int ep1, int inf1) {
diff --git a/snark-bn254-verifier_amd/csrc/bn254_kernels.h b/snark-bn254-verifier_amd/csrc/bn254_kernels.h
--- a/snark-bn254-verifier_amd/csrc/bn254_kernels.h
+++ b/snark-bn254-verifier_amd/csrc/bn254_kernels.h
@@ -79,8 +79,8 @@
 void bn254_launch_miller_step(bool do_sqr, int kind, int32_t* ws, uint32_t n, const uint8_t* status, unsigned grid, hipStream_t s, int et, int eb, int e, int epa,
                               const int32_t* t0, int ep0, int inf0, const int32_t* t1, int ep1, int inf1);
 struct MillerKinds { uint8_t nib[44]; };
-void bn254_launch_miller_run(const MillerKinds& kinds, int s_begin, int s_end, int32_t* ws, uint32_t n, const uint8_t* status, unsigned grid, hipStream_t s, int et, int eb,
-                             int e, int epa, const int32_t* tab0, int ep0, int inf0, const int32_t* tab1, int ep1, int inf1);
+void bn254_launch_miller_run(const MillerKinds& kinds, int s_begin, int s_end, int32_t* ws, uint32_t n, uint8_t* status, unsigned grid, hipStream_t s, int et, int eb,
+                             int e, int epa, const int32_t* tab0, int ep0, int inf0, const int32_t* tab1, int ep1, int inf1, int fold, int inputs_match_key);
 void bn254_launch_miller_run_fixed2(const MillerKinds& kinds, int s_begin, int s_end, int32_t* ws, uint32_t n, const uint8_t* status, unsigned grid, hipStream_t s, int e,
                                     const int32_t* tab0, int ep0, int inf0, const int32_t* tab1, int ep1, int inf1);
 #include "bn254_keys.h"
@@ -103,10 +103,9 @@
 hipError_t bn254_launch_keys_group(const uint32_t* key_index, uint32_t n, uint32_t n_keys, uint32_t slot_cap, uint32_t* count, uint32_t* base, uint32_t* cursor,
                                    uint32_t* n_slots, uint32_t* slot_to_proof, uint32_t* granule_key, uint8_t* status, hipStream_t s);
 void bn254_launch_g16_prepare_keys(const G16KeysLaunchArgs& a, unsigned grid, hipStream_t s);
-void bn254_launch_g16_subgroup_keys(const G16KeysLaunchArgs& a, unsigned grid, hipStream_t s, int e_t);
-void bn254_launch_g16_compare_keys(const G16KeysLaunchArgs& a, unsigned grid, hipStream_t s);
-void bn254_launch_miller_run_keys(const MillerKinds& kinds, int s_begin, int s_end, int32_t* ws, uint32_t n, const uint8_t* status, unsigned grid, hipStream_t s, int et, int eb,
-                                  int e, int epa, const bn254::G16KeyDesc* desc, uint32_t n_keys, const uint32_t* granule_key, int ep0, int inf0, int ep1, int inf1);
+void bn254_launch_miller_run_keys(const MillerKinds& kinds, int s_begin, int s_end, int32_t* ws, uint32_t n, uint8_t* status, unsigned grid, hipStream_t s, int et, int eb,
+                                  int e, int epa, const bn254::G16KeyDesc* desc, uint32_t n_keys, const uint32_t* granule_key, int ep0, int inf0, int ep1, int inf1, int fold);
+void bn254_launch_f12_mul_verdict_keys(const G16KeysLaunchArgs& a, unsigned grid, hipStream_t s, int e_dst, int e_a, int e_b);
 hipError_t bn254_launch_g16_keys(const G16KeysLaunchArgs& a, hipStream_t s);
 size_t bn254_tab_build_teeth(int form);
 size_t bn254_tab_build_entries(int form);
diff --git a/snark-bn254-verifier_amd/csrc/bn254_kernels.hip b/snark-bn254-verifier_amd/csrc/bn254_kernels.hip
--- a/snark-bn254-verifier_amd/csrc/bn254_kernels.hip
+++ b/snark-bn254-verifier_amd/csrc/bn254_kernels.hip
@@ -50,6 +50,13 @@
   VM_KERNEL_PROLOGUE();
   w.lds = park_lds;
   vm_f12_mul(w, d, a, b, conj_b != 0);
+}
+__global__ void __launch_bounds__(256, 2) k_f12_mul_verdict(int32_t* ws, uint32_t n, uint8_t* status, int d, int a, int b, const int32_t* __restrict__ target, int reject_code) {
+  __shared__ int32_t park_lds[72 * 256];
+  VM_KERNEL_PROLOGUE();
+  w.lds = park_lds;
+  const bool acc = vm_f12_mul_eq_const(w, d, a, b, target);
+  if (i < n && (st & BN254_ST_PENDING)) status[i] = acc ? BN254_ST_ACCEPT : (uint8_t)reject_code;
 }
 __global__ void __launch_bounds__(256, 2) k_f12_copy(int32_t* ws, uint32_t n, const uint8_t* __restrict__ status, int d, int a) { VM_KERNEL_PROLOGUE(); vm_f12_copy(w, d, a); }
 __global__ void __launch_bounds__(256, 2) k_f12_cyclo_sqr(int32_t* ws, uint32_t n, const uint8_t* __restrict__ status, int d, int a) { VM_KERNEL_PROLOGUE(); vm_f12_cyclo_sqr(w, d, a); }
@@ -353,14 +360,7 @@
 k_g16_subgroup(uint32_t n, int32_t* ws, uint8_t* __restrict__ status, int inputs_match_key, int e_t) {
   VM_KERNEL_PROLOGUE();
   bool ok = vm_g2_ate_check(w, e_t, VE_B);
-  if (i < n && (st & BN254_ST_PENDING)) {
-    uint8_t out;
-    if (!ok) out = BN254_ST_NOT_IN_SUBGROUP;
-    else if (st & 0x3f) out = st & 0x3f;
-    else if (!inputs_match_key) out = BN254_ST_INPUT_LEN;
-    else out = BN254_ST_PENDING | (st & BN254_ST_LINF);
-    status[i] = out;
-  }
+  if (i < n && (st & BN254_ST_PENDING)) status[i] = g16_subgroup_status(st, ok, inputs_match_key);
 }
 __global__ void __launch_bounds__(256, 2) k_dbg_g2_ate(int32_t* ws, uint32_t n, const uint8_t* __restrict__ status, uint8_t* o) {
   VM_KERNEL_PROLOGUE();
@@ -729,6 +729,7 @@
   G16Prof* prof;
   int inf_mask[3] = {BN254_ST_LINF, 0, 0};
   const G16KeyDesc* key_desc = nullptr; uint32_t n_keys = 0; const uint32_t* granule_key = nullptr;
+  int run_fold = 0, inputs_match_key = 0;
   int uni(int x) { return x; }
   void f12_sqr(int e) { BN_LAUNCH(KID_F12_SQR, k_f12_sqr, ws, n, status, e); }
   void miller_dbl_var(int et, int e, int ep) { BN_LAUNCH(KID_MILLER_DBL_VAR, k_miller_dbl_var, ws, n, status, et, e, ep); }
@@ -740,8 +741,8 @@
   void miller_run(int s_begin, int s_end, int et, int eb, int e, int epa, int ep0, int ep1) {
     static const MillerKinds kinds = [] { MillerKinds k; memset(&k, 0, sizeof k); for (int st_ = 0; st_ < BN_ATE_STEPS; st_++) k.nib[st_ >> 1] |= (uint8_t)(miller_step_kind(st_) << ((st_ & 1) * 4)); return k; }();
     ProfScope ps_(prof, KID_MILLER_RUN, s);
-    if (key_desc) { bn254_launch_miller_run_keys(kinds, s_begin, s_end, ws, n, status, grid, s, et, eb, e, epa, key_desc, n_keys, granule_key, ep0, inf_mask[0], ep1, inf_mask[1]); return; }
-    bn254_launch_miller_run(kinds, s_begin, s_end, ws, n, status, grid, s, et, eb, e, epa, tab[0], ep0, inf_mask[0], tab[1], ep1, inf_mask[1]);
+    if (key_desc) { bn254_launch_miller_run_keys(kinds, s_begin, s_end, ws, n, (uint8_t*)status, grid, s, et, eb, e, epa, key_desc, n_keys, granule_key, ep0, inf_mask[0], ep1, inf_mask[1], run_fold); return; }
+    bn254_launch_miller_run(kinds, s_begin, s_end, ws, n, (uint8_t*)status, grid, s, et, eb, e, epa, tab[0], ep0, inf_mask[0], tab[1], ep1, inf_mask[1], run_fold, inputs_match_key);
   }
   void miller_run_fixed2(int s_begin, int s_end, int e, int ep0, int ep1) {
     static const MillerKinds kinds = [] { MillerKinds k; memset(&k, 0, sizeof k); for (int st_ = 0; st_ < BN_ATE_STEPS; st_++) k.nib[st_ >> 1] |= (uint8_t)(miller_step_kind(st_) << ((st_ & 1) * 4)); return k; }();
@@ -812,7 +813,9 @@
     return hipGetLastError();
   }
   LaunchOps ops{a.ws, n, a.status, grid, s, {a.gtab, a.dtab, nullptr}, prof};
-  BN_LAUNCH(KID_VM_INIT, k_vm_init, a.ws, n, (const uint8_t*)a.status);
+  const bool folded = form.form == G16_FORM_LANES && form.run_steps > 0;
+  if (folded) { ops.run_fold = MR_FOLD_INIT | MR_FOLD_ATE; ops.inputs_match_key = a.inputs_match_key; }
+  else BN_LAUNCH(KID_VM_INIT, k_vm_init, a.ws, n, (const uint8_t*)a.status);
   if (form.form == G16_FORM_LATENCY) {
     ops.f12_copy(VE_S1, VE_F); ops.f12_copy(VE_S2, VE_F);
     (void)hipEventRecord(a.split_ev[0], s);
@@ -837,10 +840,15 @@
     else vm_miller_program(ops, step_kinds_host(), true);
   }
   if (ev) (void)hipEventRecord(ev[2], s);
-  BN_LAUNCH(KID_SUBGROUP, k_g16_subgroup, n, a.ws, a.status, a.inputs_match_key, (int)VE_T);
+  if (!folded) BN_LAUNCH(KID_SUBGROUP, k_g16_subgroup, n, a.ws, a.status, a.inputs_match_key, (int)VE_T);
   if (ev) (void)hipEventRecord(ev[3], s);
-  vm_final_exp_program(ops);
-  BN_LAUNCH(KID_COMPARE, k_g16_compare, a.ws, n, a.status, a.target, BN254_ST_REJECT);
+  if (folded) {
+    vm_final_exp_program_head(ops);
+    BN_LAUNCH(KID_F12_MUL, k_f12_mul_verdict, a.ws, n, a.status, (int)VE_S0, (int)VE_S2, (int)VE_S0, a.target, BN254_ST_REJECT);
+  } else {
+    vm_final_exp_program(ops);
+    BN_LAUNCH(KID_COMPARE, k_g16_compare, a.ws, n, a.status, a.target, BN254_ST_REJECT);
+  }
   if (ev) (void)hipEventRecord(ev[4], s);
   return hipGetLastError();
 }
@@ -853,11 +861,10 @@
   bn254_launch_g16_prepare_keys(a, grid, s);
   LaunchOps ops{a.ws, n, a.slot_status, grid, s, {nullptr, nullptr, nullptr}, prof};
   ops.key_desc = a.desc; ops.n_keys = a.n_keys; ops.granule_key = a.granule_key;
-  BN_LAUNCH(KID_VM_INIT, k_vm_init, a.ws, n, (const uint8_t*)a.slot_status);
+  ops.run_fold = MR_FOLD_INIT | MR_FOLD_ATE;
   vm_miller_program_runs(ops, g16_launch_form(a.m, 0, true, false, a.part_of_larger != 0, false, false, run_steps_env).run_steps);
-  bn254_launch_g16_subgroup_keys(a, grid, s, (int)VE_T);
-  vm_final_exp_program(ops);
-  bn254_launch_g16_compare_keys(a, grid, s);
+  vm_final_exp_program_head(ops);
+  bn254_launch_f12_mul_verdict_keys(a, grid, s, (int)VE_S0, (int)VE_S2, (int)VE_S0);
   return hipGetLastError();
 }
 
diff --git a/snark-bn254-verifier_amd/csrc/bn254_vm.h b/snark-bn254-verifier_amd/csrc/bn254_vm.h
--- a/snark-bn254-verifier_amd/csrc/bn254_vm.h
+++ b/snark-bn254-verifier_amd/csrc/bn254_vm.h
@@ -11,8 +11,11 @@
   VE_P3 = 82,
   VE_TMPA = 94, VE_TMPB = 100,
   VE_P5 = 106, VE_P7 = 118,
-  VE_COUNT = 130
+  VE_COUNT = 130,
+  VE_CONJ = 0x100
 };
+BN_HD bool ve_conj(int e) { return (e & VE_CONJ) != 0; }
+BN_HD int ve_elem(int e) { return e & ~VE_CONJ; }
 
 template <class W> BN_HD Fp2 vld2(W& w, int e) { Fp2 r; r.c0 = w.ld(e); r.c1 = w.ld(e + 1); return r; }
 template <class W> BN_HD void vst2(W& w, int e, const Fp2& a) { w.st(e, a.c0); w.st(e + 1, a.c1); }
@@ -260,37 +263,33 @@
   f5 = fp2_dotp(pp(d0, k5), pp(d3, k4), pp(d4, k2));
   f4 = n4;
 }
-template <class W> BN_HD void mf_line_fixed(W& w, const FixedLine& l0, int e_p0, bool inf0, Fp2& f4, Fp2& f5) {
-  Fp px = w.ld(e_p0), d0 = w.ld(e_p0 + 1);
-  Fp2 d3 = fp2_mul_fp(l0.m, px);
+template <class W> BN_HD void mf_line_fixed(W& w, const FixedLine& l, int e_p, bool inf, Fp2& f4, Fp2& f5) {
+  Fp px = w.ld(e_p), d0 = w.ld(e_p + 1);
+  Fp2 d3 = fp2_mul_fp(l.m, px);
   Fp2 x3 = fp2_mul_xi(d3);
-  const Fp2 &d4 = l0.c, &x4 = l0.xc;
-  Fp2 k0 = w.unpark(0), k1 = w.unpark(1), k2 = w.unpark(2), k3 = w.unpark(3), k4 = f4, k5 = f5;
-  w.park(0, fp2_select(inf0, k0, fp2_dot_line(d0, k0, x3, k5, x4, k3)));
-  w.park(1, fp2_select(inf0, k1, fp2_dot_line(d0, k1, d3, k0, x4, k4)));
-  w.park(2, fp2_select(inf0, k2, fp2_dot_line(d0, k2, d3, k1, x4, k5)));
-  w.park(3, fp2_select(inf0, k3, fp2_dot_line(d0, k3, d3, k2, d4, k0)));
-  f4 = fp2_select(inf0, k4, fp2_dot_line(d0, k4, d3, k3, d4, k1));
-  f5 = fp2_select(inf0, k5, fp2_dot_line(d0, k5, d3, k4, d4, k2));
-}
-template <class W> BN_HD void mf_line_fixed_k(W& w, const FixedLine& l1, int e_p1, bool inf1, Fp2& f4, Fp2& f5) {
-  Fp px = w.ld(e_p1), d0 = w.ld(e_p1 + 1);
-  Fp2 d3 = fp2_mul_fp(l1.m, px);
-  Fp2 x3 = fp2_mul_xi(d3);
-  const Fp2 &d4 = l1.c, &x4 = l1.xc;
+  const Fp2 &d4 = l.c, &x4 = l.xc;
   Fp2 k0 = w.unpark(0), k1 = w.unpark(1), k2 = w.unpark(2), k3 = w.unpark(3);
   const Fp2 k4 = f4, k5 = f5;
-  w.park(0, fp2_select(inf1, k0, fp2_dotk(kfp(k0, d0), kp(x3, k5), kp(x4, k3))));
-  w.park(1, fp2_select(inf1, k1, fp2_dotk(kfp(k1, d0), kp(d3, k0), kp(x4, k4))));
-  w.park(2, fp2_select(inf1, k2, fp2_dotk(kfp(k2, d0), kp(d3, k1), kp(x4, k5))));
-  w.park(3, fp2_select(inf1, k3, fp2_dotk(kfp(k3, d0), kp(d3, k2), kp(d4, k0))));
-  f4 = fp2_select(inf1, k4, fp2_dotk(kfp(k4, d0), kp(d3, k3), kp(d4, k1)));
-  f5 = fp2_select(inf1, k5, fp2_dotk(kfp(k5, d0), kp(d3, k4), kp(d4, k2)));
-}
+  w.park(0, fp2_select(inf, k0, fp2_dotk(kfp(k0, d0), kp(x3, k5), kp(x4, k3))));
+  w.park(1, fp2_select(inf, k1, fp2_dotk(kfp(k1, d0), kp(d3, k0), kp(x4, k4))));
+  w.park(2, fp2_select(inf, k2, fp2_dotk(kfp(k2, d0), kp(d3, k1), kp(x4, k5))));
+  w.park(3, fp2_select(inf, k3, fp2_dotk(kfp(k3, d0), kp(d3, k2), kp(d4, k0))));
+  f4 = fp2_select(inf, k4, fp2_dotk(kfp(k4, d0), kp(d3, k3), kp(d4, k1)));
+  f5 = fp2_select(inf, k5, fp2_dotk(kfp(k5, d0), kp(d3, k4), kp(d4, k2)));
+}
+template <class W> BN_HD void mf_init(W& w, int e_t, int e_b, Fp2& f4, Fp2& f5) {
+  w.park(0, fp2_one()); w.park(1, fp2_zero()); w.park(2, fp2_zero()); w.park(3, fp2_zero());
+  f4 = fp2_zero(); f5 = fp2_zero();
+  vst2(w, e_t, vld2(w, e_b)); vst2(w, e_t + 2, vld2(w, e_b + 2)); vst2(w, e_t + 4, fp2_one());
+}
+enum { MR_FOLD_INIT = 1, MR_FOLD_ATE = 2 };
+template <class W> BN_HD bool vm_g2_ate_check(W& w, int e_t, int e_b);
 template <class W, class LINES, class KINDS>
-BN_HD void vm_miller_run(W& w, const LINES& lines, const KINDS& kinds, int s_begin, int s_end, int e_t, int e_b, int e, int e_pa, int e_p0, bool inf0, int e_p1, bool inf1) {
+BN_HD bool vm_miller_run(W& w, const LINES& lines, const KINDS& kinds, int s_begin, int s_end, int e_t, int e_b, int e, int e_pa, int e_p0, bool inf0, int e_p1, bool inf1,
+                         int fold = 0) {
   Fp2 f4, f5;
-  mf_load(w, e, f4, f5);
+  if ((fold & MR_FOLD_INIT) && s_begin == 0) mf_init(w, e_t, e_b, f4, f5);
+  else mf_load(w, e, f4, f5);
   for (int s = s_begin; s < s_end; s++) {
     const int kind = kinds.get(s);
     if (kind == 0) {
@@ -304,9 +303,11 @@
     }
     BN_SCHED_FENCE();
     mf_line_fixed(w, lines.get(0, s), e_p0, inf0, f4, f5);
-    mf_line_fixed_k(w, lines.get(1, s), e_p1, inf1, f4, f5);
+    mf_line_fixed(w, lines.get(1, s), e_p1, inf1, f4, f5);
   }
   mf_store(w, e, f4, f5);
+  if ((fold & MR_FOLD_ATE) && s_end == BN_ATE_STEPS) return vm_g2_ate_check(w, e_t, e_b);
+  return true;
 }
 
 template <class W, class LINES, class KINDS>
@@ -317,7 +318,7 @@
     if (kinds.get(s) == 0 && s != 0) mf_sqr(w, f4, f5);
     BN_SCHED_FENCE();
     mf_line_fixed(w, lines.get(0, s), e_p0, inf0, f4, f5);
-    mf_line_fixed_k(w, lines.get(1, s), e_p1, inf1, f4, f5);
+    mf_line_fixed(w, lines.get(1, s), e_p1, inf1, f4, f5);
   }
   mf_store(w, e, f4, f5);
 }
@@ -333,11 +334,27 @@
 
 template <class W> BN_HD Fp6 vld_half(W& w, int e, int h) { Fp6 r; r.c0 = vld2(w, e + 2 * h); r.c1 = vld2(w, e + 4 + 2 * h); r.c2 = vld2(w, e + 8 + 2 * h); return r; }
 template <class W> BN_HD void vst_half(W& w, int e, int h, const Fp6& a) { vst2(w, e + 2 * h, a.c0); vst2(w, e + 4 + 2 * h, a.c1); vst2(w, e + 8 + 2 * h, a.c2); }
-template <class W>
-BN_HD void vm_f12_mul(W& w, int e_dst, int e_a, int e_b, bool conj_b = false) {
+BN_HD Fp vm_const_fp(const int32_t* target, int k) {
+  Fp t;
+#pragma unroll
+  for (int l = 0; l < BN_NL; l++) t.v[l] = target[k * BN_NL + l];
+  BN_SETB(t, 1.0, 0.5);
+  return t;
+}
+BN_HD bool vm_half_eq_const(const Fp6& c, int h, const int32_t* target) {
+  bool ok = fp_eq(c.c0.c0, vm_const_fp(target, 2 * h)) & fp_eq(c.c0.c1, vm_const_fp(target, 2 * h + 1));
+  ok &= fp_eq(c.c1.c0, vm_const_fp(target, 4 + 2 * h)) & fp_eq(c.c1.c1, vm_const_fp(target, 5 + 2 * h));
+  ok &= fp_eq(c.c2.c0, vm_const_fp(target, 8 + 2 * h)) & fp_eq(c.c2.c1, vm_const_fp(target, 9 + 2 * h));
+  return ok;
+}
+template <bool CMP, class W>
+BN_HD bool vm_f12_mul_impl(W& w, int e_dst, int e_a_flagged, int e_b, bool conj_b, const int32_t* target) {
+  const bool conj_a = ve_conj(e_a_flagged);
+  const int e_a = ve_elem(e_a_flagged);
   { Fp6 v0 = fp6_mul(vld_half(w, e_a, 0), vld_half(w, e_b, 0)); w.park(0, v0.c0); w.park(1, v0.c1); w.park(2, v0.c2); }
   BN_SCHED_FENCE();
   Fp6 a1 = vld_half(w, e_a, 1), b1 = vld_half(w, e_b, 1);
+  if (conj_a) a1 = fp6_neg(a1);
   if (conj_b) b1 = fp6_neg(b1);
   Fp6 c0;
   {
@@ -351,23 +368,35 @@
   a1 = fp6_add(vld_half(w, e_a, 0), a1);
   b1 = fp6_add(vld_half(w, e_b, 0), b1);
   vst_half(w, e_dst, 0, c0);
+  bool eq = true;
+  if constexpr (CMP) eq = vm_half_eq_const(c0, 0, target);
   BN_SCHED_FENCE();
   const Fp6 s = fp6_mul(a1, b1);
   BN_SCHED_FENCE();
   Fp6 c1;
   c1.c0 = fp2_sub(s.c0, w.unpark(0)); c1.c1 = fp2_sub(s.c1, w.unpark(1)); c1.c2 = fp2_sub(s.c2, w.unpark(2));
   vst_half(w, e_dst, 1, c1);
-}
-template <class W>
-BN_HD void vm_f12_cyclo_sqr(W& w, int e_dst, int e_src) {
+  if constexpr (CMP) eq &= vm_half_eq_const(c1, 1, target);
+  return eq;
+}
+template <class W>
+BN_HD void vm_f12_mul(W& w, int e_dst, int e_a, int e_b, bool conj_b = false) { vm_f12_mul_impl<false>(w, e_dst, e_a, e_b, conj_b, nullptr); }
+template <class W>
+BN_HD bool vm_f12_mul_eq_const(W& w, int e_dst, int e_a, int e_b, const int32_t* target) { return vm_f12_mul_impl<true>(w, e_dst, e_a, e_b, false, target); }
+template <class W>
+BN_HD void vm_f12_cyclo_sqr(W& w, int e_dst, int e_src_flagged) {
+  const bool cj = ve_conj(e_src_flagged);
+  const int e_src = ve_elem(e_src_flagged);
   {
     Fp2 k0 = vld2(w, e_src), k3 = vld2(w, e_src + 6);
+    if (cj) k3 = fp2_neg(k3);
     Fp2 za, zb;
     gs_pair(za, zb, k0, k3, k0, k3, false);
     vst2(w, e_dst, za); vst2(w, e_dst + 6, zb);
   }
   {
     Fp2 k1 = vld2(w, e_src + 2), k2 = vld2(w, e_src + 4), k4 = vld2(w, e_src + 8), k5 = vld2(w, e_src + 10);
+    if (cj) { k1 = fp2_neg(k1); k5 = fp2_neg(k5); }
     Fp2 z2, z5, z4, z1;
     gs_pair(z2, z5, k1, k4, k2, k5, false);
     gs_pair(z4, z1, k2, k5, k4, k1, true);
@@ -375,8 +404,11 @@
   }
 }
 template <class W>
-BN_HD void vm_f12_cyclo_sqr_n(W& w, int e_dst, int e_src, int count) {
+BN_HD void vm_f12_cyclo_sqr_n(W& w, int e_dst, int e_src_flagged, int count) {
+  const bool cj = ve_conj(e_src_flagged);
+  const int e_src = ve_elem(e_src_flagged);
   Fp2 k0 = vld2(w, e_src), k1 = vld2(w, e_src + 2), k2 = vld2(w, e_src + 4), k3 = vld2(w, e_src + 6), k4 = vld2(w, e_src + 8), k5 = vld2(w, e_src + 10);
+  if (cj) { k1 = fp2_neg(k1); k3 = fp2_neg(k3); k5 = fp2_neg(k5); }
   for (int it = 0; it < count; it++) {
     Fp2 n0, n3, n2, n5, n4, n1;
     gs_pair(n0, n3, k0, k3, k0, k3, false);
@@ -475,29 +507,31 @@
   }
 }
 template <class OPS>
-BN_HD void vm_final_exp_program(OPS& ops) {
+BN_HD void vm_final_exp_program_head(OPS& ops) {
   ops.f12_inv(VE_S0, VE_F);
-  ops.f12_conj(VE_S1, VE_F);
-  ops.f12_mul(VE_S0, VE_S1, VE_S0, false);
+  ops.f12_mul(VE_S0, VE_F | VE_CONJ, VE_S0, false);
   ops.f12_frob(VE_S1, VE_S0, 2);
   ops.f12_mul(VE_F, VE_S1, VE_S0);
-  vm_exp_u(ops, VE_S0, VE_F); ops.f12_conj(VE_S0, VE_S0);
-  ops.f12_cyclo_sqr(VE_S0, VE_S0);
+  vm_exp_u(ops, VE_S0, VE_F);
+  ops.f12_cyclo_sqr(VE_S0, VE_S0 | VE_CONJ);
   ops.f12_cyclo_sqr(VE_S1, VE_S0);
   ops.f12_mul(VE_S1, VE_S0, VE_S1);
-  vm_exp_u(ops, VE_S2, VE_S1); ops.f12_conj(VE_S2, VE_S2);
-  ops.f12_conj(VE_S3, VE_S1);
-  ops.f12_mul(VE_S1, VE_S2, VE_S3);
-  ops.f12_cyclo_sqr(VE_S3, VE_S2);
+  vm_exp_u(ops, VE_S2, VE_S1);
+  ops.f12_mul(VE_S1, VE_S2 | VE_CONJ, VE_S1, true);
+  ops.f12_cyclo_sqr(VE_S3, VE_S2 | VE_CONJ);
   vm_exp_u(ops, VE_S4, VE_S3);
   ops.f12_mul(VE_S4, VE_S1, VE_S4);
   ops.f12_mul(VE_S3, VE_S0, VE_S4);
-  ops.f12_mul(VE_S0, VE_S2, VE_S4);
+  ops.f12_mul(VE_S0, VE_S2 | VE_CONJ, VE_S4);
   ops.f12_mul(VE_S0, VE_F, VE_S0);
   ops.f12_frob(VE_S2, VE_S3, 1); ops.f12_mul(VE_S0, VE_S2, VE_S0);
   ops.f12_frob(VE_S2, VE_S4, 2); ops.f12_mul(VE_S0, VE_S2, VE_S0);
-  ops.f12_conj(VE_S2, VE_F); ops.f12_mul(VE_S2, VE_S2, VE_S3);
+  ops.f12_mul(VE_S2, VE_F | VE_CONJ, VE_S3);
   ops.f12_frob(VE_S2, VE_S2, 3);
+}
+template <class OPS>
+BN_HD void vm_final_exp_program(OPS& ops) {
+  vm_final_exp_program_head(ops);
   ops.f12_mul(VE_S0, VE_S2, VE_S0);
 }
 
```

New measurement: 6.016 million (median of 6 runs). +1.5%, better.
